# 54rt1n/shardmerge

Hardware: AMD Instinct MI355X
Metric: merged-weight GB/s per GPU + % HBM roofline, Llama-3-70B 3-way FFT merge (higher is better)
Workload: dtype f32; 1 GPU; Llama-3-70B block tensors, this rank's 1/8 slice (9 per block x 10 blocks), K=3 finetunes, bf16 in/out, resident in HBM; workload_id=llama3-70b-slice, k=3, parallelism=tensor-partition x1 (no data-path collective), streams_per_gpu=8

## Files before the change

shardmerge_amd/csrc/sm_capi.inc:

```

struct smhip_ctx {
    smhip::Pipeline<SM_BACKEND> pipe;
    explicit smhip_ctx(int device) : pipe(device) {}
};

#define SM_GUARD(ctx)                      \
    if (!(ctx)) return SMHIP_ERR_ARG;      \
    (ctx)->pipe.err.clear();
#define SM_FINISH(ctx, rc)                                                        \
    do {                                                                          \
        int rc__ = (rc);                                                          \
        if (rc__ == SMHIP_OK && !(ctx)->pipe.be.ok()) {                           \
            (ctx)->pipe.err = (ctx)->pipe.be.error();                             \
            rc__ = SMHIP_ERR_HIP;                                                 \
        }                                                                         \
        return rc__;                                                              \
    } while (0)

extern "C" {

const char* smhip_version(void) { return SM_VERSION_STRING; }

int smhip_create(int device, smhip_ctx** out) {
    if (!out) return SMHIP_ERR_ARG;
    *out = nullptr;
    smhip_ctx* c = new smhip_ctx(device);
    if (!c->pipe.be.ok()) {
        fprintf(stderr, "smhip_create: %s\n", c->pipe.be.error().c_str());
        delete c;
        return SMHIP_ERR_HIP;
    }
    *out = c;
    return SMHIP_OK;
}

void smhip_destroy(smhip_ctx* ctx) { delete ctx; }

const char* smhip_last_error(smhip_ctx* ctx) { return ctx ? ctx->pipe.err.c_str() : "null context"; }

int smhip_reserve(smhip_ctx* ctx, int rows, int cols) {
    SM_GUARD(ctx);
    if (rows < 1 || cols < 1) return ctx->pipe.fail(SMHIP_ERR_ARG, "bad shape");
    SM_FINISH(ctx, ctx->pipe.reserve(rows, cols));
}

size_t smhip_workspace_bytes(smhip_ctx* ctx) { return ctx ? ctx->pipe.workspace_bytes() : 0; }

int smhip_length_supported(int n) {
    int T;
    std::vector<int> rad;
    return smhip::plan_shape(n, T, rad) ? SMHIP_OK : SMHIP_ERR_SHAPE;
}

int smhip_shape_supported(int rows, int cols) {
    return smhip::shape_support(rows, cols) ? SMHIP_OK : SMHIP_ERR_SHAPE;
}

int smhip_fft_transform(smhip_ctx* ctx, const float* x, int rows, int cols, float* spectrum, void* stream) {
    SM_GUARD(ctx);
    if (!x || !spectrum || rows < 1 || cols < 1) return ctx->pipe.fail(SMHIP_ERR_ARG, "bad argument");
    ctx->pipe.stream = stream;
    SM_FINISH(ctx, ctx->pipe.fft_transform(x, rows, cols, spectrum));
}

int smhip_ifft_transform(smhip_ctx* ctx, const float* spectrum, int rows, int cols, float* real_out, void* stream) {
    SM_GUARD(ctx);
    if (!real_out || !spectrum || rows < 1 || cols < 1) return ctx->pipe.fail(SMHIP_ERR_ARG, "bad argument");
    ctx->pipe.stream = stream;
    SM_FINISH(ctx, ctx->pipe.ifft_transform(spectrum, rows, cols, real_out));
}

int smhip_interpolate_fft_components(smhip_ctx* ctx, const float* f0, const float* f1, int rows, int cols, double t,
                                     double t_sum, double cutoff_pct, double cull_pct, int interp_imag,
                                     float* out_spectrum, smhip_blend_info* info, void* stream) {
    SM_GUARD(ctx);
    if (!f0 || !f1 || !out_spectrum || rows < 1 || cols < 1) return ctx->pipe.fail(SMHIP_ERR_ARG, "bad argument");
    ctx->pipe.stream = stream;
    SM_FINISH(ctx, ctx->pipe.blend_full(f0, f1, rows, cols, smhip::BLEND_SLERP, t, t_sum, cutoff_pct, cull_pct, 1,
                                        interp_imag, out_spectrum, info));
}

int smhip_arithmetic_fft_components(smhip_ctx* ctx, const float* f0, const float* f1, int rows, int cols, double t,
                                    int agreement, int do_imag, float* out_spectrum, void* stream) {
    SM_GUARD(ctx);
    if (!f0 || !f1 || !out_spectrum || rows < 1 || cols < 1) return ctx->pipe.fail(SMHIP_ERR_ARG, "bad argument");
    ctx->pipe.stream = stream;
    SM_FINISH(ctx, ctx->pipe.blend_full(f0, f1, rows, cols, smhip::BLEND_ARITH, t, 1.0, 0, 0, agreement, do_imag,
                                        out_spectrum, nullptr));
}

int smhip_merge_tensors_fft2_slerp(smhip_ctx* ctx, const float* v0, const float* v1, int rows, int cols, double t,
                                   double b, double t_sum, double cutoff_pct, double cull_pct, float* out,
                                   double* norm0, double* norm1, int* branch, smhip_blend_info* info, void* stream) {
    SM_GUARD(ctx);
    if (!v0 || !v1 || !out || rows < 1 || cols < 1) return ctx->pipe.fail(SMHIP_ERR_ARG, "bad argument");
    ctx->pipe.stream = stream;
    SM_FINISH(ctx, ctx->pipe.merge_pair_slerp(v0, v1, rows, cols, t, b, t_sum, cutoff_pct, cull_pct, out, norm0, norm1,
                                              branch, info));
}

int smhip_task_arithmetic_fft2(smhip_ctx* ctx, const float* v0, const float* v1, int rows, int cols, double t,
                               int agreement, float* out, void* stream) {
    SM_GUARD(ctx);
    if (!v0 || !v1 || !out || rows < 1 || cols < 1) return ctx->pipe.fail(SMHIP_ERR_ARG, "bad argument");
    ctx->pipe.stream = stream;
    smhip::SigDesc a{v0, nullptr, smhip::DT_F32, 1.f}, bb{v1, nullptr, smhip::DT_F32, 1.f};
    smhip::PairOut po;
    po.out = out; po.out_mode = smhip::OUT_F32; po.post = 1.f;
    const int rc0 = ctx->pipe.reserve(rows, cols);
    if (rc0) SM_FINISH(ctx, rc0);
    ctx->pipe.clear_flags();
    po.ifft_policy = 0;
    SM_FINISH(ctx, ctx->pipe.pair_arith(a, bb, rows, cols, 1.f, 1.f, t, agreement, po, -1, -1));
}

int smhip_merge_layer(smhip_ctx* ctx, const smhip_layer_desc* desc, void* out_bf16, float* delta_out,
                      smhip_layer_report* report, void* stream) {
    SM_GUARD(ctx);
    if (!desc || !out_bf16) return ctx->pipe.fail(SMHIP_ERR_ARG, "bad argument");
    for (int i = 0; i < desc->k && i < SMHIP_MAX_MODELS; ++i)
        if (!desc->finetune[i] || !desc->base[i]) return ctx->pipe.fail(SMHIP_ERR_ARG, "null model tensor");
    if (!desc->base_out) return ctx->pipe.fail(SMHIP_ERR_ARG, "null base_out");
    ctx->pipe.stream = stream;
    SM_FINISH(ctx, ctx->pipe.merge_layer(*desc, out_bf16, delta_out, report));
}

int smhip_addition_merge(smhip_ctx* ctx, int k, const void* const* finetunes, const void* base, int dtype, size_t n,
                         int sign_agreement, void* out, void* stream) {
    SM_GUARD(ctx);
    if (!finetunes || !base || !out || n < 1) return ctx->pipe.fail(SMHIP_ERR_ARG, "bad argument");
    if (dtype < SMHIP_BF16 || dtype > SMHIP_F32) return ctx->pipe.fail(SMHIP_ERR_ARG, "bad dtype");
    for (int i = 0; i < k && i < SMHIP_MAX_MODELS; ++i)
        if (!finetunes[i]) return ctx->pipe.fail(SMHIP_ERR_ARG, "null model tensor");
    ctx->pipe.stream = stream;
    SM_FINISH(ctx, ctx->pipe.addition_merge(k, finetunes, base, dtype, n, sign_agreement ? 1 : 0, out));
}

int smhip_slerp(smhip_ctx* ctx, const float* v0, const float* v1, size_t rows, size_t cols, float t, float* out, void* stream) {
    SM_GUARD(ctx);
    if (rows * cols > 0 && (!v0 || !v1 || !out)) return ctx->pipe.fail(SMHIP_ERR_ARG, "bad argument");
    ctx->pipe.stream = stream;
    SM_FINISH(ctx, ctx->pipe.fn_slerp(v0, v1, rows, cols, t, out));
}

int smhip_div_scalar(smhip_ctx* ctx, const void* x, int dtype, size_t n, float s, void* out, void* stream) {
    SM_GUARD(ctx);
    if (n > 0 && (!x || !out)) return ctx->pipe.fail(SMHIP_ERR_ARG, "bad argument");
    if (dtype < SMHIP_BF16 || dtype > SMHIP_F32) return ctx->pipe.fail(SMHIP_ERR_ARG, "bad dtype");
    ctx->pipe.stream = stream;
    SM_FINISH(ctx, ctx->pipe.fn_div_scalar(x, dtype, n, s, out));
}

int smhip_lora_apply(smhip_ctx* ctx, const void* base, int dtype, int rows, int cols, const void* lora_a,
                     const void* lora_b, int factor_dtype, int rank, float scale, void* out, void* stream) {
    SM_GUARD(ctx);
    if (!base || !lora_a || !lora_b || !out || rows < 1 || cols < 1) return ctx->pipe.fail(SMHIP_ERR_ARG, "bad argument");
    if (dtype < SMHIP_BF16 || dtype > SMHIP_F32 || factor_dtype < SMHIP_BF16 || factor_dtype > SMHIP_F32)
        return ctx->pipe.fail(SMHIP_ERR_ARG, "bad dtype");
    if (rank < 1 || rank > smhip::LORA_MAX_RANK) return ctx->pipe.fail(SMHIP_ERR_ARG, "rank out of range (1..512)");
    const size_t bes = dtype == SMHIP_F32 ? 4 : 2, fes = factor_dtype == SMHIP_F32 ? 4 : 2;
    const uintptr_t o0 = (uintptr_t)out, o1 = o0 + (size_t)rows * cols * bes;
    auto overlaps = [&](const void* p, size_t bytes) { return (uintptr_t)p < o1 && o0 < (uintptr_t)p + bytes; };
    if (overlaps(base, (size_t)rows * cols * bes) || overlaps(lora_a, (size_t)rank * cols * fes) ||
        overlaps(lora_b, (size_t)rows * rank * fes))
        return ctx->pipe.fail(SMHIP_ERR_ARG, "lora_apply: out overlaps an input");
    ctx->pipe.stream = stream;
    SM_FINISH(ctx, ctx->pipe.lora_apply(base, dtype, rows, cols, lora_a, lora_b, factor_dtype, rank, scale, out));
}

int smhip_adapter_apply(smhip_ctx* ctx, const smhip_adapter_desc* d, void* stream) {
    SM_GUARD(ctx);
    if (!d || !d->base || !d->lora_a || !d->lora_b || !d->out || d->rows < 1 || d->cols < 1)
        return ctx->pipe.fail(SMHIP_ERR_ARG, "bad argument");
    if (d->dtype < SMHIP_BF16 || d->dtype > SMHIP_F32 || d->factor_dtype < SMHIP_BF16 || d->factor_dtype > SMHIP_F32 ||
        (d->magnitude && (d->magnitude_dtype < SMHIP_BF16 || d->magnitude_dtype > SMHIP_F32)))
        return ctx->pipe.fail(SMHIP_ERR_ARG, "bad dtype");
    if (d->layout != SMHIP_ADAPTER_LINEAR && d->layout != SMHIP_ADAPTER_EMBEDDING)
        return ctx->pipe.fail(SMHIP_ERR_ARG, "adapter_apply: bad layout");
    if (d->magnitude && d->layout != SMHIP_ADAPTER_LINEAR)
        return ctx->pipe.fail(SMHIP_ERR_ARG, "adapter_apply: DoRA (a magnitude) needs the LINEAR layout");
    if (d->rank < 1 || d->rank > smhip::LORA_MAX_RANK) return ctx->pipe.fail(SMHIP_ERR_ARG, "rank out of range (1..512)");
    const size_t bes = d->dtype == SMHIP_F32 ? 4 : 2, fes = d->factor_dtype == SMHIP_F32 ? 4 : 2;
    const size_t mes = d->magnitude_dtype == SMHIP_F32 ? 4 : 2;
    const bool emb = d->layout == SMHIP_ADAPTER_EMBEDDING;
    const uintptr_t o0 = (uintptr_t)d->out, o1 = o0 + (size_t)d->rows * d->cols * bes;
    auto overlaps = [&](const void* p, size_t bytes) { return (uintptr_t)p < o1 && o0 < (uintptr_t)p + bytes; };
    if (overlaps(d->base, (size_t)d->rows * d->cols * bes) ||
        overlaps(d->lora_a, (size_t)d->rank * (emb ? d->rows : d->cols) * fes) ||
        overlaps(d->lora_b, (size_t)(emb ? d->cols : d->rows) * d->rank * fes) ||
        (d->magnitude && overlaps(d->magnitude, (size_t)d->rows * mes)))
        return ctx->pipe.fail(SMHIP_ERR_ARG, "adapter_apply: out overlaps an input");
    ctx->pipe.stream = stream;
    SM_FINISH(ctx, ctx->pipe.adapter_apply(d->base, d->dtype, d->rows, d->cols, d->lora_a, d->lora_b, d->factor_dtype,
                                           d->rank, d->scale, emb ? 1 : 0, d->magnitude, d->magnitude_dtype, d->out));
}

int smhip_exact_norm(smhip_ctx* ctx, const void* x, int dtype, size_t n, double* norm_out, void* stream) {
    SM_GUARD(ctx);
    if (!norm_out || (n > 0 && !x)) return ctx->pipe.fail(SMHIP_ERR_ARG, "bad argument");
    if (dtype < SMHIP_BF16 || dtype > SMHIP_F32) return ctx->pipe.fail(SMHIP_ERR_ARG, "bad dtype");
    ctx->pipe.stream = stream;
    SM_FINISH(ctx, ctx->pipe.fn_exact_norm(x, dtype, n, norm_out));
}

int smhip_correlate_pairs(smhip_ctx* ctx, int k, const void* const* tensors, int dtype, size_t rows, size_t cols,
                          float* matrix_out, void* stream) {
    SM_GUARD(ctx);
    if (!tensors || !matrix_out || rows < 1 || cols < 1) return ctx->pipe.fail(SMHIP_ERR_ARG, "bad argument");
    if (dtype < SMHIP_BF16 || dtype > SMHIP_F32) return ctx->pipe.fail(SMHIP_ERR_ARG, "bad dtype");
    for (int i = 0; i < k && i < 8; ++i)
        if (!tensors[i]) return ctx->pipe.fail(SMHIP_ERR_ARG, "null tensor");
    ctx->pipe.stream = stream;
    SM_FINISH(ctx, ctx->pipe.correlate_pairs(k, tensors, dtype, rows, cols, matrix_out));
}

int smhip_reference_cpu_norm(smhip_ctx* ctx, const void* x, const void* base, int dtype, size_t n, float* norm_out,
                             void* stream) {
    SM_GUARD(ctx);
    if (!x || !norm_out) return ctx->pipe.fail(SMHIP_ERR_ARG, "bad argument");
    if (dtype < SMHIP_BF16 || dtype > SMHIP_F32) return ctx->pipe.fail(SMHIP_ERR_ARG, "bad dtype");
    ctx->pipe.stream = stream;
    const int rc0 = ctx->pipe.reserve(1, 1);
    if (rc0) SM_FINISH(ctx, rc0);
    smhip::SigDesc sg{x, base, dtype, 1.f};
    double out = 0;
    if (!ctx->pipe.run_serial_norms(&sg, 1, n, &out))
        return ctx->pipe.fail(SMHIP_ERR_ARG, "reference_cpu norm: inputs must be 16-byte aligned");
    *norm_out = (float)out;
    SM_FINISH(ctx, SMHIP_OK);
}

int smhip_debug_option(smhip_ctx* ctx, const char* key, long value) {
    SM_GUARD(ctx);
    if (key && std::string(key) == "aten_overlap") { ctx->pipe.aten_overlap = value != 0; return SMHIP_OK; }
    if (key && std::string(key) == "emf_max_sample") { ctx->pipe.emf_max_sample = value >= 1 && value <= 4096 ? (int)value : smhip::EMF_MAX_SAMPLE; return SMHIP_OK; }
    if (key && std::string(key) == "aten_serial") { ctx->pipe.aten_serial = value != 0; return SMHIP_OK; }
    if (key && std::string(key) == "class_norms") { ctx->pipe.class_norms_mode = value >= 0 && value <= 2 ? (int)value : 1; return SMHIP_OK; }
    if (key && std::string(key) == "cand_cap") { ctx->pipe.debug_cand_cap = value > 0 ? (uint32_t)value : 0u; return SMHIP_OK; }
    if (key && std::string(key) == "sel_chunks") { ctx->pipe.debug_sel_chunks = value > 0 ? (uint32_t)value : 0u; return SMHIP_OK; }
    if (key && std::string(key) == "sel_flush_always") { ctx->pipe.debug_flush_always = value != 0; return SMHIP_OK; }
    if (key && std::string(key) == "fuse_norms") { ctx->pipe.fuse_norms = value != 0; return SMHIP_OK; }
    if (key && std::string(key) == "noise_seed") { ctx->pipe.noise_seed_base = (uint32_t)value; return SMHIP_OK; }
    if (key && std::string(key) == "spectral_intermediates") { ctx->pipe.spectral_inter = value != 0; return SMHIP_OK; }
    if (key && std::string(key) == "fuse_spec_norm") { ctx->pipe.fuse_spec_norm = value != 0; return SMHIP_OK; }
    if (key && std::string(key) == "sel_wgs_per_cu") { ctx->pipe.sel_wgs_per_cu = value > 0 ? (int)value : 5; return SMHIP_OK; }
    if (key && std::string(key) == "pair1d") { ctx->pipe.pair1d_enabled = value != 0; return SMHIP_OK; }
    if (key && std::string(key) == "spec_cull") { ctx->pipe.spec_cull = value != 0; return SMHIP_OK; }
    if (key && std::string(key) == "spec_min_bins") { ctx->pipe.spec_min_bins = value >= 0 ? (size_t)value : (size_t)1 << 20; return SMHIP_OK; }
    if (key && std::string(key) == "dftp_pairs") { ctx->pipe.dftp_pairs_enabled = value != 0; return SMHIP_OK; }
    if (key && std::string(key) == "f2s_pair") { ctx->pipe.f2s_pair = value != 0; return SMHIP_OK; }
    if (key && std::string(key) == "f1_multi") { ctx->pipe.f1_multi = value != 0; return SMHIP_OK; }
    if (key && std::string(key) == "force_bluestein") { ctx->pipe.debug_force_bluestein = value != 0; return SMHIP_OK; }
    if (key && std::string(key) == "force_split") { ctx->pipe.debug_force_split = value > 1 && value <= smhip::DFTP_MAX_P ? (int)value : 0; return SMHIP_OK; }
    if (key && std::string(key) == "fold_columns") { ctx->pipe.fold_enabled = value != 0; return SMHIP_OK; }
    if (key && std::string(key) == "fold_min_rows") { ctx->pipe.fold_min_rows = value > 0 ? (int)value : SM_FOLD_MIN_ROWS; return SMHIP_OK; }
    return ctx->pipe.fail(SMHIP_ERR_ARG, "unknown debug option");
}

int smhip_debug_query(smhip_ctx* ctx, const char* key, long* value) {
    SM_GUARD(ctx);
    if (!key || !value) return SMHIP_ERR_ARG;
    if (std::string(key) == "spec_hit") { *value = ctx->pipe.last_spec_verdict(); SM_FINISH(ctx, SMHIP_OK); }
    if (std::string(key) == "spec_checked" || std::string(key) == "spec_hits") {
        unsigned long long c = 0, h = 0;
        ctx->pipe.spec_totals(&c, &h);
        *value = (long)(std::string(key) == "spec_hits" ? h : c);
        SM_FINISH(ctx, SMHIP_OK);
    }
    if (std::string(key) == "aten_fast" || std::string(key) == "aten_group" || std::string(key) == "aten_slow") {
        unsigned long long v3[3];
        ctx->pipe.aten_stats(1, v3);
        *value = (long)v3[std::string(key) == "aten_fast" ? 0 : std::string(key) == "aten_group" ? 1 : 2];
        SM_FINISH(ctx, SMHIP_OK);
    }
    return ctx->pipe.fail(SMHIP_ERR_ARG, "unknown debug query");
}

int smhip_profile_enable(smhip_ctx* ctx, int on) { SM_GUARD(ctx); ctx->pipe.be.profile_enable(on != 0); return SMHIP_OK; }
int smhip_profile_reset(smhip_ctx* ctx) { SM_GUARD(ctx); ctx->pipe.be.profile_reset(); return SMHIP_OK; }
int smhip_profile_count(smhip_ctx* ctx) { return ctx ? ctx->pipe.be.profile_count() : 0; }
int smhip_profile_get(smhip_ctx* ctx, int i, const char** name, uint64_t* launches, double* total_ms) {
    SM_GUARD(ctx);
    return ctx->pipe.be.profile_get(i, name, launches, total_ms) ? SMHIP_OK : SMHIP_ERR_ARG;
}

}
```

shardmerge_amd/csrc/sm_kernels.hpp:

```cpp
#pragma once
#include <cmath>
#include <cstring>

#include "fft_engine.hpp"
#include "sm_aten_core.hpp"

namespace smhip {

struct cf4 { float x, y, z, w; };
struct u32x4 { uint32_t x, y, z, w; };

enum { DT_BF16 = 0, DT_F16 = 1, DT_F32 = 2 };

struct SigDesc {
    const void* x;
    const void* base;
    int dtype;
    float prescale;
};

SM_HD uint32_t umax(uint32_t a, uint32_t b) { return a > b ? a : b; }
SM_HD float u2f(uint32_t u) { float f; memcpy(&f, &u, 4); return f; }
SM_HD uint32_t f2u(float f) { uint32_t u; memcpy(&u, &f, 4); return u; }
SM_HD float bf16_to_f(uint32_t h) { return u2f(h << 16); }
// ... 173 lines not shown

struct F1Params {
    FftPlanDev plan;
    SigDesc a, b;
    int R, C, Cb;
    int pitch4;
    int ilv;
    int nb;
    size_t row_stride;
    int vec;
    cf4* t1;
    double* partials;
    int R2;
    int rowpair;
    int Rcol;
    size_t slab_elems;
    const cf2* twR;
    F1Sigs sigs;
    AtenFuse fuse;
    int fuse_rowpair;
};

template <class P> constexpr bool f1_full_batch() {
    if constexpr (P::is_static) return P::T <= 256; else return false;
}
#ifndef SM_ROW_PACK_MAX_T
#define SM_ROW_PACK_MAX_T 256
#endif
template <class P> constexpr bool f1_opaque() {
    if constexpr (P::is_static) return P::T >= 512; else return false;
}
#ifndef SM_ROW_PACK_BIG
#define SM_ROW_PACK_BIG 0
#endif
template <class P> constexpr int f1_pack() {
    if constexpr (P::is_static) return P::T <= SM_ROW_PACK_MAX_T ? 1 : SM_ROW_PACK_BIG; else return 1;
}

template <class P, class Ex>
SM_HD void k_f1(Ex& ex, const F1Params& p) {
    typename Ex::template State<FftState> st;
    ex.init(st);
    float* lds = ex.lds() + LDS_SCRATCH_FLOATS;
    const FftPlanDev& pl = p.plan;
    const int T = plan_T<P>(pl), C = plan_N<P>(pl);
    const int LF = plan_lds<P>(pl);
    int sig_;
    const int bid = f1_pick_signal(p.sigs, ex.bid(), (p.ilv > p.nb) ? p.ilv / p.nb : 1, sig_);
    const int pbid = p.sigs.n > 1 ? bid : ex.bid();
    SigDesc sgA = p.a, sgB = p.b;
    cf4* t1_ = p.t1;
    double* partials_ = p.partials;
    if (p.sigs.n > 1) {
        sgA.x = p.sigs.x[sig_]; sgA.base = p.sigs.base[sig_];
        sgB.x = (const char*)sgA.x + p.sigs.b_off; sgB.base = sgA.base ? (const char*)sgA.base + p.sigs.b_off : nullptr;
        t1_ = p.sigs.t1[sig_]; partials_ = p.sigs.partials[sig_];
    }
    const bool vec = P::is_static ? true : (p.vec != 0);
    auto fuse_where = [&](int comp) {
        return [&, comp](int g, int& sig, long long& mrow) {
            const int row = bid * p.nb + g;
            if (row >= p.R) return false;
            if (p.fuse_rowpair) { sig = sig_; mrow = 2LL * row + comp; }
            else { sig = comp; mrow = row; if (comp == 1 && !sgB.x) return false; }
            return true;
        };
    };
    if constexpr (P::is_static) {
        if constexpr (aten_fusable(P::N, P::T)) {
            if (p.fuse.prefix) ex.each(st, [&](int tid, FftState& s) {
                s.fep[0] = aten_fused_ep<P::N, P::T>(p.fuse, tid, fuse_where(0));
                s.fep[1] = aten_fused_ep<P::N, P::T>(p.fuse, tid, fuse_where(1));
            });
        }
    }

    ex.each(st, [&](int tid, FftState& s) {
        const int g = tid / T, t = tid % T;
        const int row = bid * p.nb + g;
        const bool valid = row < p.R;
        double sa = 0.0, sb = 0.0;
        if (vec && sgA.dtype != DT_F32 && sgB.dtype != DT_F32) {
            constexpr int NQ = EMAX / 8;
            u32x4 ra[NQ], rab[NQ], rb[NQ], rbb[NQ];
            bool ok[NQ];
            size_t off[NQ];
#pragma unroll
            for (int q = 0; q < NQ; ++q) {
                const int n0 = 8 * (t + q * T);
                ok[q] = valid && n0 < C;
                off[q] = ok[q] ? ((size_t)row * p.row_stride + n0) / 8 : 0;
            }
            const bool has_ab = sgA.base != nullptr, has_b = sgB.x != nullptr, has_bb = has_b && sgB.base != nullptr;
            const u32x4* pa = (const u32x4*)sgA.x;
            const u32x4* pab = has_ab ? (const u32x4*)sgA.base : pa;
            const u32x4* pb = has_b ? (const u32x4*)sgB.x : pa;
            const u32x4* pbb = has_bb ? (const u32x4*)sgB.base : pa;
            constexpr int QB = f1_full_batch<P>() ? NQ : NQ / 2;
            bool all_ok = true;
#pragma unroll
            for (int q = 0; q < NQ; ++q) all_ok = all_ok && ok[q];
            static_for<0, NQ / QB>([&](auto h_c) {
            constexpr int Q0 = decltype(h_c)::value * QB, Q1 = Q0 + QB;
#pragma unroll
            for (int q = Q0; q < Q1; ++q) ra[q] = pa[off[q]];
#pragma unroll
            for (int q = Q0; q < Q1; ++q) rab[q] = pab[off[q]];
#pragma unroll
            for (int q = Q0; q < Q1; ++q) rb[q] = pb[off[q]];
#pragma unroll
            for (int q = Q0; q < Q1; ++q) rbb[q] = pbb[off[q]];
            auto decode = [&](auto masked_c) {
                constexpr bool MASKED = decltype(masked_c)::value;
#pragma unroll
                for (int q = Q0; q < Q1; ++q) {
                    float va[8], vb[8], ba[8], bb[8];
                    decode16x8(ra[q], sgA.dtype, va);
                    decode16x8(rab[q], sgA.dtype, ba);
                    decode16x8(rb[q], sgB.dtype, vb);
                    decode16x8(rbb[q], sgB.dtype, bb);
#pragma unroll
                    for (int c = 0; c < 8; ++c) {
                        if (!has_ab) ba[c] = 0.f;
                        if (!has_b) vb[c] = 0.f;
                        if (!has_bb) bb[c] = 0.f;
                    }
                    float pa = 0.f, pb = 0.f;
#pragma unroll
                    for (int c = 0; c < 8; ++c) {
                        float xa = (va[c] - ba[c]) * sgA.prescale;
                        float xb = (vb[c] - bb[c]) * sgB.prescale;
                        if (MASKED && !ok[q]) { xa = 0.f; xb = 0.f; }
                        s.xr[q * 8 + c] = xa; s.xi[q * 8 + c] = xb;
                        pa += xa * xa; pb += xb * xb;
                    }
                    sa += pa; sb += pb;
                }
            };
            if (all_ok) decode(std::false_type{});
            else decode(std::true_type{});
            });

        } else if (vec) {
            constexpr int NQ = EMAX / 8;
            bool ok[NQ];
            size_t off[NQ];
#pragma unroll
            for (int q = 0; q < NQ; ++q) {
                const int n0 = 8 * (t + q * T);
                ok[q] = valid && n0 < C;
                off[q] = ok[q] ? (size_t)row * p.row_stride + n0 : 0;
            }
            auto load_signal = [&](const SigDesc& sg, float* dst, double& ss) {
                if (!sg.x) {
#pragma unroll
                    for (int i = 0; i < 8 * NQ; ++i) dst[i] = 0.f;
                    return;
                }
                const bool has_base = sg.base != nullptr;
                float v[NQ][8], bv[NQ][8];
                if (sg.dtype == DT_F32) {
                    const cf4* px = (const cf4*)sg.x;
                    const cf4* pb = has_base ? (const cf4*)sg.base : px;
                    cf4 r[NQ][2], rb[NQ][2];
#pragma unroll
                    for (int q = 0; q < NQ; ++q) { r[q][0] = px[off[q] / 4]; r[q][1] = px[off[q] / 4 + 1]; }
#pragma unroll
                    for (int q = 0; q < NQ; ++q) { rb[q][0] = pb[off[q] / 4]; rb[q][1] = pb[off[q] / 4 + 1]; }
#pragma unroll
                    for (int q = 0; q < NQ; ++q) {
                        const cf4 x0 = r[q][0], x1 = r[q][1], b0 = rb[q][0], b1 = rb[q][1];
                        const float xs[8] = {x0.x, x0.y, x0.z, x0.w, x1.x, x1.y, x1.z, x1.w};
                        const float bs[8] = {b0.x, b0.y, b0.z, b0.w, b1.x, b1.y, b1.z, b1.w};
#pragma unroll
                        for (int c = 0; c < 8; ++c) { v[q][c] = xs[c]; bv[q][c] = bs[c]; }
                    }
                } else {
                    const u32x4* px = (const u32x4*)sg.x;
                    const u32x4* pb = has_base ? (const u32x4*)sg.base : px;
                    u32x4 r[NQ], rb[NQ];
#pragma unroll
                    for (int q = 0; q < NQ; ++q) r[q] = px[off[q] / 8];
#pragma unroll
                    for (int q = 0; q < NQ; ++q) rb[q] = pb[off[q] / 8];
#pragma unroll
                    for (int q = 0; q < NQ; ++q) { decode16x8(r[q], sg.dtype, v[q]); decode16x8(rb[q], sg.dtype, bv[q]); }
                }
#pragma unroll
                for (int q = 0; q < NQ; ++q) {
                    float ps = 0.f;
#pragma unroll
                    for (int c = 0; c < 8; ++c) {
                        float x = (v[q][c] - (has_base ? bv[q][c] : 0.f)) * sg.prescale;
                        if (!ok[q]) x = 0.f;
                        dst[q * 8 + c] = x;
                        ps += x * x;
                    }
                    ss += ps;
                }
            };
            load_signal(sgA, s.xr, sa);
            load_signal(sgB, s.xi, sb);
        } else {
#pragma unroll
            for (int q = 0; q < EMAX; ++q) {
                const int n = t + q * T;
                float va = 0.f, vb = 0.f;
                if (valid && n < C) {
                    const size_t off = (size_t)row * p.row_stride + n;
                    va = load_sig1(sgA, off);
                    vb = load_sig1(sgB, off);
                }
                s.xr[q] = va; s.xi[q] = vb;
                sa += (double)va * va; sb += (double)vb * vb;
            }
        }
        s.red[0] = sa; s.red[1] = sb;
    });
    ex.template block_sum<2>(st, [&](const double* tot) {
        partials_[2 * (size_t)pbid] = tot[0];
        partials_[2 * (size_t)pbid + 1] = tot[1];
    });

    wg_fft<P, f1_pack<P>(), 1>(ex, st, pl, lds,
        [&](int tid, FftState& s, auto comp_c) {
            constexpr int comp = decltype(comp_c)::value;
            const int g = tid / T, t = tid % T;
            float* l = lds + g * LF;
            const float* x = comp_of<comp>(s);
            if (vec) {
#pragma unroll
                for (int q = 0; q < EMAX / 8; ++q) {
                    const int n0 = 8 * (t + q * T);
                    if (n0 < C) {
#pragma unroll
                        for (int c = 0; c < 8; ++c) l[lpad(n0 + c)] = x[q * 8 + c];
                    }
                }
            } else {
#pragma unroll
                for (int q = 0; q < EMAX; ++q) {
                    const int n = t + q * T;
                    if (n < C) l[lpad(n)] = x[q];
                }
            }
        },
        [&](int tid, FftState& s, auto comp_c) {
            constexpr int comp = decltype(comp_c)::value;
            int tid_ = tid;
            if constexpr (f1_opaque<P>()) SM_OPAQUE(tid_);
            const int g = tid_ / T, t = tid_ % T;
            const float* l = lds + g * LF;
            float* o = comp_of<comp>(s);
#pragma unroll
            for (int u = 0; u < EMAX / 2 + 1; ++u) {
                const int k = t + u * T;
                if (k < p.Cb) {
                    const int k2 = (k == 0) ? 0 : C - k;
                    const float v1 = l[lpad(k)], v2 = l[lpad(k2)];
                    if (comp == 0) { o[2 * u] = 0.5f * (v1 + v2); o[2 * u + 1] = 0.5f * (v2 - v1); }
                    else           { o[2 * u] = 0.5f * (v1 - v2); o[2 * u + 1] = 0.5f * (v1 + v2); }
                    if (!sgB.x) o[2 * u + 1] = 0.f;
                }
            }
        },
        [&](auto comp_c) {
            constexpr int comp = decltype(comp_c)::value;
            if constexpr (P::is_static) {
                if constexpr (aten_fusable(P::N, P::T)) {
                    if (p.fuse.prefix)
                        aten_fused_rows<P::N, P::T>(ex, st, p.fuse, lds, LF, fuse_where(comp), [](FftState& s) { return s.fep[comp]; });
                }
            }
        });

    ex.each(st, [&](int tid, FftState& s) {
        int tid_ = tid;
        if constexpr (f1_opaque<P>()) SM_OPAQUE(tid_);
        const int g = tid_ / T, t = tid_ % T;
        const int row = bid * p.nb + g;
        if (row >= p.R) return;
        cf4* dst = t1_ + (size_t)(row / p.ilv) * p.pitch4 * p.ilv + (row % p.ilv);
#pragma unroll
        for (int u = 0; u < EMAX / 2 + 1; ++u) {
            const int k = t + u * T;
            if (k < p.Cb) {
                cf4 v;
                v.x = s.xr[2 * u]; v.y = s.xi[2 * u]; v.z = s.xi[2 * u + 1]; v.w = s.xr[2 * u + 1];
                dst[(size_t)k * p.ilv] = v;
            }
        }
    });
}

#ifndef SM_F1Q_QB
#define SM_F1Q_QB 1
#endif
#ifndef SM_F1Q_PREFETCH_B
#define SM_F1Q_PREFETCH_B 1
#endif
#ifndef SM_F1Q_PACK
#define SM_F1Q_PACK 1
#endif
template <class P> constexpr bool f1q_eligible() {
    if constexpr (P::is_static) return 4 * P::T <= 1024 && (P::N / P::T) % 2 == 0 && P::N % 8 == 0; else return false;
}

struct F1QState {
    float xr[EREG];
    float xi[EREG];
    double red[4];
    u32x4 rb[EMAX / 8], rbb[EMAX / 8];
};

template <class P, class Ex>
SM_HD void k_f1q(Ex& ex, const F1Params& p) {
    if constexpr (!f1q_eligible<P>()) { return; } else {
    typename Ex::template State<F1QState> st;
    ex.init(st);
    float* lds = ex.lds() + LDS_SCRATCH_FLOATS;
    const FftPlanDev& pl = p.plan;
    constexpr int T = P::T, C = P::N, LF = P::lds_floats;
    constexpr int E2 = C / T / 2;
    constexpr int NJ = (E2 + 3) / 4;
    constexpr int NQ = EMAX / 8;
    static_assert(NJ * 8 + 4 <= EREG, "register slots");
    int sig_;
    const int bid = f1_pick_signal(p.sigs, ex.bid(), p.ilv > 1 ? p.ilv : 1, sig_);
    const int pbid = p.sigs.n > 1 ? bid : ex.bid();
    SigDesc sa = p.a, sb = p.b;
    cf4* t1_ = p.t1;
    double* partials_ = p.partials;
    if (p.sigs.n > 1) {
        sa.x = p.sigs.x[sig_]; sa.base = p.sigs.base[sig_];
        sb.x = (const char*)sa.x + p.sigs.b_off; sb.base = sa.base ? (const char*)sa.base + p.sigs.b_off : nullptr;
        t1_ = p.sigs.t1[sig_]; partials_ = p.sigs.partials[sig_];
    }
    const int unit = bid;
    const bool live = unit < p.R2;
    const bool bits16 = sa.dtype != DT_F32 && sb.dtype != DT_F32;
    const bool has_ab = sa.base != nullptr, has_b = sb.x != nullptr, has_bb = has_b && sb.base != nullptr;
    const int n2A = p.rowpair ? 2 * unit : unit, n2B = p.rowpair ? 2 * unit + 1 : unit;
    cf4* const rowp = t1_ + (size_t)(unit / p.ilv) * p.pitch4 * p.ilv + (unit % p.ilv);
    const size_t slabstride = p.slab_elems;

    ex.each(st, [&](int, F1QState& s) { s.red[0] = 0.0; s.red[1] = 0.0; });

    wg_fft<P, SM_F1Q_PACK, 1>(ex, st, pl, lds,
        [&](int tid, F1QState& s, auto comp_c) {
            constexpr int comp = decltype(comp_c)::value;
            int tid_ = tid;
            SM_OPAQUE(tid_);
            const int g = tid_ / T, t = tid_ % T;
            float* l = lds + g * LF;
            const size_t rowoff = (size_t)(unit + g * p.R2) * p.row_stride;
            auto okq = [&](int q) { return live && 8 * (t + q * T) < C; };
            auto offq = [&](int q) { return okq(q) ? rowoff + 8 * (t + q * T) : (size_t)0; };
            double ss = 0.0;
            if (bits16) {
                const u32x4* pa = (const u32x4*)sa.x;
                if (comp == 0) {
                    const u32x4* pab = has_ab ? (const u32x4*)sa.base : pa;
                    u32x4 ra[NQ], rab[NQ];
#pragma unroll
                    for (int q = 0; q < NQ; ++q) ra[q] = pa[offq(q) / 8];
#pragma unroll
                    for (int q = 0; q < NQ; ++q) rab[q] = pab[offq(q) / 8];
#if SM_F1Q_PREFETCH_B
                    const u32x4* pb = has_b ? (const u32x4*)sb.x : pa;
                    const u32x4* pbb = has_bb ? (const u32x4*)sb.base : pa;
#pragma unroll
                    for (int q = 0; q < NQ; ++q) s.rb[q] = pb[offq(q) / 8];
#pragma unroll
                    for (int q = 0; q < NQ; ++q) s.rbb[q] = pbb[offq(q) / 8];
#endif
#pragma unroll
                    for (int q = 0; q < NQ; ++q) {
                        float va[8], ba[8];
                        decode16x8(ra[q], sa.dtype, va);
                        decode16x8(rab[q], sa.dtype, ba);
                        const int n0 = 8 * (t + q * T);
                        float qa = 0.f;
#pragma unroll
                        for (int c = 0; c < 8; ++c) {
                            float xa = (va[c] - (has_ab ? ba[c] : 0.f)) * sa.prescale;
                            if (!okq(q)) xa = 0.f;
                            if (n0 < C) l[lpad(n0 + c)] = xa;
                            qa += xa * xa;
                        }
                        ss += qa;
                    }
                } else {
#if !SM_F1Q_PREFETCH_B
                    const u32x4* pb = has_b ? (const u32x4*)sb.x : pa;
                    const u32x4* pbb = has_bb ? (const u32x4*)sb.base : pa;
#pragma unroll
                    for (int q = 0; q < NQ; ++q) s.rb[q] = pb[offq(q) / 8];
#pragma unroll
                    for (int q = 0; q < NQ; ++q) s.rbb[q] = pbb[offq(q) / 8];
#endif
#pragma unroll
                    for (int q = 0; q < NQ; ++q) {
                        float vb[8], bb[8];
                        decode16x8(s.rb[q], sb.dtype, vb);
                        decode16x8(s.rbb[q], sb.dtype, bb);
                        const int n0 = 8 * (t + q * T);
                        float qb = 0.f;
#pragma unroll
                        for (int c = 0; c < 8; ++c) {
                            float xb = has_b ? (vb[c] - (has_bb ? bb[c] : 0.f)) * sb.prescale : 0.f;
                            if (!okq(q)) xb = 0.f;
                            if (n0 < C) l[lpad(n0 + c)] = xb;
                            qb += xb * xb;
                        }
                        ss += qb;
                    }
                }
            } else {
                const SigDesc& sg = comp == 0 ? sa : sb;
#pragma unroll
                for (int q = 0; q < NQ; ++q) {
                    float v[8];
                    if (sg.x) load_sig8(sg, offq(q), v);
                    else { for (int c = 0; c < 8; ++c) v[c] = 0.f; }
                    const int n0 = 8 * (t + q * T);
                    float ps = 0.f;
#pragma unroll
                    for (int c = 0; c < 8; ++c) {
                        const float x = okq(q) ? v[c] : 0.f;
                        if (n0 < C) l[lpad(n0 + c)] = x;
                        ps += x * x;
                    }
                    ss += ps;
                }
            }
            s.red[comp] += ss;
        },
        [&](int tid, F1QState& s, auto comp_c) {
            constexpr int comp = decltype(comp_c)::value;
            int tid_ = tid;
            SM_OPAQUE(tid_);
            const int g = tid_ / T, t = tid_ % T;
            auto emit = [&](int k, const float* are, const float* aim, const float* bre, const float* bim) {
                SM_SCHED_FENCE();
                float ar[4], ai[4], br[4], bi[4];
#pragma unroll
                for (int q = 0; q < 4; ++q) { ar[q] = are[q]; ai[q] = aim[q]; br[q] = has_b ? bre[q] : 0.f; bi[q] = has_b ? bim[q] : 0.f; }
                Dft<4>::run(ar, ai);
                Dft<4>::run(br, bi);
#pragma unroll
                for (int k1 = 0; k1 < 4; ++k1) {
                    if (k1) {
                        const cf2 wa = p.twR[(size_t)n2A * k1], wb = p.twR[(size_t)n2B * k1];
                        cmul(ar[k1], ai[k1], wa.x, wa.y); cmul(br[k1], bi[k1], wb.x, wb.y);
                    }
                    cf4 v = {ar[k1], ai[k1], br[k1], bi[k1]};
                    if (live) rowp[(size_t)k * p.ilv + k1 * slabstride] = v;
                }
                SM_SCHED_FENCE();
            };
#pragma unroll
            for (int jj = 0; jj < NJ; ++jj) {
                const int u = 4 * jj + g;
                if (u < E2) {
                    const int k = t + u * T;
                    const int k2 = (k == 0) ? 0 : C - k;
                    float aim[4], bre[4];
#pragma unroll
                    for (int gp = 0; gp < 4; ++gp) {
                        const float* l = lds + gp * LF;
                        const float v1 = l[lpad(k)], v2 = l[lpad(k2)];
                        const int sl = (jj * 4 + gp) * 2;
                        if (comp == 0) { s.xr[sl] = 0.5f * (v1 + v2); s.xr[sl + 1] = 0.5f * (v2 - v1); }
                        else           { aim[gp] = 0.5f * (v1 - v2); bre[gp] = 0.5f * (v1 + v2); }
                    }
                    if (comp == 1) {
                        float are[4], bim[4];
#pragma unroll
                        for (int gp = 0; gp < 4; ++gp) { are[gp] = s.xr[(jj * 4 + gp) * 2]; bim[gp] = s.xr[(jj * 4 + gp) * 2 + 1]; }
                        emit(k, are, aim, bre, bim);
                    }
                }
            }
            if (tid == 0) {
                if (comp == 0) {
#pragma unroll
                    for (int gp = 0; gp < 4; ++gp) s.xr[NJ * 8 + gp] = lds[gp * LF + lpad(C / 2)];
                } else {
                    float are[4], aim[4] = {0.f, 0.f, 0.f, 0.f}, bre[4], bim[4] = {0.f, 0.f, 0.f, 0.f};
#pragma unroll
                    for (int gp = 0; gp < 4; ++gp) { are[gp] = s.xr[NJ * 8 + gp]; bre[gp] = lds[gp * LF + lpad(C / 2)]; }
                    emit(C / 2, are, aim, bre, bim);
                }
            }
        });

    ex.template block_sum<2>(st, [&](const double* tot) {
        partials_[2 * (size_t)pbid] = tot[0];
        partials_[2 * (size_t)pbid + 1] = tot[1];
    });
    }
}

struct SliceGrid { int wgs = 0; size_t t1_stride = 0, plane_stride = 0; };
template <class Ex> SM_HD int slice_of(Ex& ex, const SliceGrid& sl, int& bid) {
    bid = ex.bid();
    if (sl.wgs <= 0) return 0;
    const int s = bid / sl.wgs;
    bid -= s * sl.wgs;
    return s;
}

struct F2Params {
    FftPlanDev plan;
    const cf4* t1;
    int pitch4;
    int ilv;
    int R, C, Cb;
    int nsig;
    int swap;
    float scale[2];
    float* reA; float* imA; float* reB;
    unsigned long long* hist;
    int slab;
    int Cb_real;
    int Rfull;
    size_t slab_elems;
    SliceGrid sl;
};
SM_HD int fold_bin(int v, int slab, int Cb_real, int R2, int Rfull, size_t& off) {
    const int k1 = v / slab, k = v % slab;
    off = (size_t)k * Rfull + (size_t)k1 * R2;
    return k < Cb_real ? k : -1;
}

#ifndef SM_T1_ILV
#define SM_T1_ILV 2
#endif
#ifndef SM_T1_ILV_MIN_ROWS
#define SM_T1_ILV_MIN_ROWS 8192
#endif
#ifndef SM_F2_MAX_THREADS
#define SM_F2_MAX_THREADS 512
#endif
SM_HD constexpr int t1_interleave_rows(int R) { return R >= SM_T1_ILV_MIN_ROWS ? SM_T1_ILV : 1; }
SM_HD constexpr int f2_nsig_for(int T) { return (2 * T <= SM_F2_MAX_THREADS) ? 2 : 1; }

constexpr int FOLD_ILV = 2;
template <class P> constexpr bool fold_col_plan() {
    if constexpr (P::is_static) return f2_nsig_for(P::T) == 2 && (P::N == 2048 || P::N == 3584 || P::N == 4096 || P::N == 7168);
    else return false;
}
template <class P, int BINS, bool FOLD = false, class Ex>
SM_HD void k_f2(Ex& ex, const F2Params& p) {
    if constexpr (FOLD && !fold_col_plan<P>()) { return; } else {
    typename Ex::template State<FftState> st;
    ex.init(st);
    float* lds = ex.lds() + LDS_SCRATCH_FLOATS;
    const FftPlanDev& pl = p.plan;
    const int T = plan_T<P>(pl), R = plan_N<P>(pl);
    const int LF = plan_lds<P>(pl);
    const int ng = P::is_static ? f2_nsig_for(T) : p.nsig;
    const int ilv = FOLD ? FOLD_ILV : (P::is_static ? t1_interleave_rows(R) : p.ilv);
    int bid;
    const int slice = slice_of(ex, p.sl, bid);
    const cf4* const t1 = p.t1 + slice * p.sl.t1_stride;
    const size_t pl_off = slice * p.sl.plane_stride;
    const int lbid = (ng == 2) ? xcd_remap(bid, 8 / BINS) : xcd_remap(bid, 16);
    const int kbase = (ng == 2) ? lbid * BINS : lbid / 2;
    const int slot0 = (ng == 2) ? 0 : lbid % 2;
    if (kbase >= p.Cb) return;
    const int ngroups = (ng == 2) ? 2 * BINS : 1;
    const int nthreads = ngroups * T;
    uint32_t* lhist = (uint32_t*)(lds + ngroups * LF);

    ex.each(st, [&](int tid, FftState& s) {
        if (ng == 2) {
            const int b = tid % BINS, lane = tid / BINS;
            const int k2 = kbase + b;
            auto load_rows = [&](auto ilv_c) {
                constexpr int ILV = decltype(ilv_c)::value;
#pragma unroll
                for (int q = 0; q < EMAX / 2; ++q) {
                    const int m = lane + (q / ILV) * 2 * T;
                    const int n = m * ILV + q % ILV;
                    const bool live = n < R && k2 < p.Cb;
                    const int kc = k2 < p.Cb ? k2 : p.Cb - 1;
                    const int mcl = n < R ? m : (R - 1 - q % ILV) / ILV;
                    cf4 v;
                    if constexpr (FOLD) {
                        v = t1[(size_t)(kc / p.slab) * p.slab_elems + ((size_t)mcl * p.slab + (kc % p.slab)) * ILV + q % ILV];
                    } else {
                        v = t1[((size_t)mcl * p.pitch4 + kc) * ILV + q % ILV];
                    }
                    s.xr[2 * q] = live ? v.x : 0.f; s.xi[2 * q] = live ? v.y : 0.f; s.xr[2 * q + 1] = live ? v.z : 0.f; s.xi[2 * q + 1] = live ? v.w : 0.f;
                }
            };
            if (ilv == 2) load_rows(std::integral_constant<int, 2>{});
            else load_rows(std::integral_constant<int, 1>{});
        } else {
#pragma unroll
            for (int q = 0; q < EMAX; ++q) {
                const int n = tid + q * T;
                float re = 0.f, im = 0.f;
                if (n < R) {
                    const cf2* src = (const cf2*)(t1 + ((size_t)(n / ilv) * p.pitch4 + kbase) * ilv + n % ilv) + slot0;
                    re = src->x; im = src->y;
                }
                s.xr[q] = re; s.xi[q] = im;
            }
        }
        if (p.hist) for (int h = tid; h < HIST1_BINS; h += nthreads) lhist[h] = 0;
    });

#ifndef SM_F2_PACK
#define SM_F2_PACK 1
#endif
    wg_fft<P, SM_F2_PACK, 2>(ex, st, pl, lds,
        [&](int tid, FftState& s, auto comp_c) {
            constexpr int comp = decltype(comp_c)::value;
            const float* x = comp_of<comp>(s);
            if (ng == 2) {
                const int b = tid % BINS, lane = tid / BINS;
                float* la = lds + (2 * b) * LF;
                auto scatter_rows = [&](auto ilv_c) {
                    constexpr int ILV = decltype(ilv_c)::value;
#pragma unroll
                    for (int q = 0; q < EMAX / 2; ++q) {
                        const int n = (lane + (q / ILV) * 2 * T) * ILV + q % ILV;
                        if (n < R) { la[lpad(n)] = x[2 * q]; la[LF + lpad(n)] = x[2 * q + 1]; }
                    }
                };
                if (ilv == 2) scatter_rows(std::integral_constant<int, 2>{});
                else scatter_rows(std::integral_constant<int, 1>{});
            } else {
#pragma unroll
                for (int q = 0; q < EMAX; ++q) {
                    const int n = tid + q * T;
                    if (n < R) lds[lpad(n)] = x[q];
                }
            }
        },
        [&](int tid, FftState& s, auto comp_c) {
            constexpr int comp = decltype(comp_c)::value;
            const int g = tid / T, t = tid % T;
            const float* l = lds + g * LF;
            float* o = comp_of<comp>(s);
#pragma unroll
            for (int u = 0; u < EMAX / 4; ++u) {
#pragma unroll
                for (int c = 0; c < 4; ++c) {
                    const int k1 = 4 * (t + u * T) + c;
                    if (k1 < R) o[4 * u + c] = l[lpad(k1)];
                }
            }
        });

    ex.each(st, [&](int tid, FftState& s) {
        const int g = tid / T, t = tid % T;
        const int slot = (ng == 2) ? (g & 1) : slot0;
        const int k2 = kbase + ((ng == 2) ? (g >> 1) : 0);
        if (k2 >= p.Cb) return;
        const bool role_a = (slot ^ p.swap) == 0;
        const float sc = p.scale[slot];
        size_t poff = (size_t)k2 * R;
        int kreal = k2;
        if constexpr (FOLD) { kreal = fold_bin(k2, p.slab, p.Cb_real, R, p.Rfull, poff); if (kreal < 0) return; }
        const uint32_t w = (uint32_t)bin_weight(kreal, p.C);
        float* dre = (role_a ? p.reA : p.reB) + pl_off + poff;
        float* dim = p.imA + pl_off + poff;
#pragma unroll
        for (int u = 0; u < EMAX / 4; ++u) {
            const int k0 = 4 * (t + u * T);
            if (k0 + 3 < R && (R & 3) == 0) {
                cf4 vr = {s.xr[4 * u] * sc, s.xr[4 * u + 1] * sc, s.xr[4 * u + 2] * sc, s.xr[4 * u + 3] * sc};
                *(cf4*)(dre + k0) = vr;
                if (role_a) {
                    cf4 vi = {s.xi[4 * u] * sc, s.xi[4 * u + 1] * sc, s.xi[4 * u + 2] * sc, s.xi[4 * u + 3] * sc};
                    *(cf4*)(dim + k0) = vi;
                }
            } else {
#pragma unroll
                for (int c = 0; c < 4; ++c) {
                    if (k0 + c < R) {
                        dre[k0 + c] = s.xr[4 * u + c] * sc;
                        if (role_a) dim[k0 + c] = s.xi[4 * u + c] * sc;
                    }
                }
            }
            if (p.hist) {
#pragma unroll
                for (int c = 0; c < 4; ++c) {
                    if (k0 + c < R) {
                        const uint32_t key = f2u(s.xr[4 * u + c] * sc) & 0x7fffffffu;
                        ex.lds_atomic_add(&lhist[key >> 20], w);
                    }
                }
            }
        }
    });
    if (p.hist) {
        ex.sync();
        ex.each(st, [&](int tid, FftState&) {
            for (int h = tid; h < HIST1_BINS; h += nthreads) {
                const uint32_t v = lhist[h];
                if (v) ex.global_atomic_add(&p.hist[h], (unsigned long long)v);
            }
        });
    }
    }
}

#ifndef SM_COL_THREADS
#define SM_COL_THREADS 512
#endif
constexpr int f2_bins_for(int T, int N = 1 << 30) {
    if (T == 64 && N <= 256) return 8;
    return (SM_COL_THREADS / (2 * T)) > 1 ? (SM_COL_THREADS / (2 * T) > 8 ? 8 : SM_COL_THREADS / (2 * T)) : 1;
}
#ifndef SM_I1_THREADS
constexpr int i1_bins_for(int T) { return 2; }
#else
constexpr int i1_bins_for(int T) { return (SM_I1_THREADS / T) > 2 ? ((SM_I1_THREADS / T) > 16 ? 16 : (SM_I1_THREADS / T)) : 2; }
#endif
template <class P> constexpr int f2_bins() { if constexpr (P::is_static) return f2_bins_for(P::T, P::N); else return 1; }
template <class P> constexpr int i1_bins() { if constexpr (P::is_static) return i1_bins_for(P::T); else return 2; }

struct F2SParams {
    FftPlanDev plan;
    const cf4* t1;
    int pitch4;
    int R, C, Cb;
    int role_a;
    float scale;
    float* re; float* im;
    unsigned long long* hist;
    int slab, Cb_real, Rfull;
    size_t slab_elems;
    double* im_partials;
    SliceGrid sl;
    int two;
    const cf4* t1_2; int role_a_2; float scale_2; float* re_2;
};
template <class P> constexpr int f2s_groups() {
    if constexpr (P::is_static) return f2_nsig_for(P::T) == 2 ? 2 * f2_bins_for(P::T, P::N) : 1; else return 1;
}

#ifndef SM_F2S_ILV
#define SM_F2S_ILV 1
#endif
constexpr int F2S_ILV = SM_F2S_ILV;
#ifndef SM_F2S_DIRECT
#define SM_F2S_DIRECT 0
#endif
template <class P, int G> constexpr int f2s_direct() {
    if constexpr (!P::is_static) return 0;
    else {
        constexpr int R0 = P::radix(0);
        constexpr bool ok = F2S_ILV == 1 && (G == 1 || G == 2) && P::npass >= 2 && P::T % 2 == 0 && R0 % 2 == 0 &&
                            (P::N / R0) % 2 == 0 && (EMAX / R0) * R0 * P::T >= P::N;
        return ok ? (SM_F2S_DIRECT & 3) : 0;
    }
}
template <class P, int G, bool FOLD = false, class Ex>
SM_HD void k_f2s(Ex& ex, const F2SParams& p) {
    if constexpr (FOLD && !fold_col_plan<P>()) { return; } else {
    typename Ex::template State<FftState> st;
    ex.init(st);
    float* lds = ex.lds() + LDS_SCRATCH_FLOATS;
    const FftPlanDev& pl = p.plan;
    const int T = plan_T<P>(pl), R = plan_N<P>(pl);
    const int LF = plan_lds<P>(pl);
    constexpr int XG = G >= 8 ? 1 : 8 / G;
    int bid_in_slice;
    const int slice = slice_of(ex, p.sl, bid_in_slice);
    int sig2 = 0;
    const int lbid = p.two ? pick_signal(2, bid_in_slice, XG, sig2) : xcd_remap(bid_in_slice, XG);
    const cf4* const t1 = (sig2 ? p.t1_2 : p.t1) + slice * p.sl.t1_stride;
    const size_t pl_off = slice * p.sl.plane_stride;
    const int role_a_ = sig2 ? p.role_a_2 : p.role_a;
    const float scale_ = sig2 ? p.scale_2 : p.scale;
    float* const re_ = sig2 ? p.re_2 : p.re;
    const int kbase = lbid * G;
    if (kbase >= p.Cb) {
        if (p.im_partials) ex.each(st, [&](int tid, FftState&) { if (tid == 0) p.im_partials[ex.bid()] = 0.0; });
        return;
    }
    const int nthreads = G * T;
    const int half = R / 2;
    uint32_t* lhist = (uint32_t*)(lds + G * LF);

    constexpr int DIRECT = f2s_direct<P, G>();
    if constexpr ((DIRECT & 1) != 0) {
        constexpr int R0 = P::radix(0), MB0 = EMAX / R0, nb0 = P::N / R0;
        ex.each(st, [&](int tid, FftState& s) {
            const int g = tid / T, t = tid % T;
            const int k2 = kbase + g;
            const int kc = k2 < p.Cb ? k2 : p.Cb - 1;
            const int par = t & 1;
            static_for<0, MB0>([&](auto m_c) {
                constexpr int m = decltype(m_c)::value;
                const bool live = (t + m * T) < nb0 && k2 < p.Cb;
                static_for<0, R0 / 2>([&](auto q_c) {
                    constexpr int q = decltype(q_c)::value;
                    const int pm = live ? (t >> 1) + m * (T / 2) + q * nb0 + par * (nb0 / 2) : 0;
                    cf4 v;
#if defined(SM_DIAG_NOMEM)
                    v = cf4{(float)q, (float)t, 1.f, (float)kc};
#else
                    if constexpr (FOLD) v = t1[(size_t)(kc / p.slab) * p.slab_elems + (size_t)pm * p.slab + (kc % p.slab)];
                    else v = t1[(size_t)pm * p.pitch4 + kc];
#endif
                    s.xr[m * R0 + 2 * q] = live ? v.x : 0.f; s.xi[m * R0 + 2 * q] = live ? v.y : 0.f;
                    s.xr[m * R0 + 2 * q + 1] = live ? v.z : 0.f; s.xi[m * R0 + 2 * q + 1] = live ? v.w : 0.f;
                });
            });
            if (p.hist) for (int h = tid; h < HIST1_BINS; h += nthreads) lhist[h] = 0;
        });
        ex.template lane_pair_trade<MB0 * (R0 / 2) * 2>(st, [](FftState& s, auto k_c) {
            constexpr int k = decltype(k_c)::value;
            constexpr int idx = k / 2, m = idx / (R0 / 2), q = idx % (R0 / 2);
            float* arr = (k % 2) ? s.xi : s.xr;
            return FloatPairRef{arr[m * R0 + 2 * q], arr[m * R0 + 2 * q + 1]};
        });
    } else
    ex.each(st, [&](int tid, FftState& s) {
        const int b = tid % G, lane = tid / G;
        const int k2 = kbase + b;
#pragma unroll
        for (int q = 0; q < EMAX / 2; ++q) {
            const int m = F2S_ILV * (lane + (q / F2S_ILV) * T) + q % F2S_ILV;
            const bool live = m < half && k2 < p.Cb;
            const int mc = m < half ? m : half - 1, kc = k2 < p.Cb ? k2 : p.Cb - 1;
            cf4 v;
#if defined(SM_DIAG_NOMEM)
            v = cf4{(float)q, (float)lane, 1.f, (float)kc};
#else
            if constexpr (FOLD) {
                v = t1[(size_t)(kc / p.slab) * p.slab_elems + ((size_t)(mc / F2S_ILV) * p.slab + (kc % p.slab)) * F2S_ILV + mc % F2S_ILV];
            } else {
                v = t1[((size_t)(mc / F2S_ILV) * p.pitch4 + kc) * F2S_ILV + mc % F2S_ILV];
            }
#endif
            s.xr[2 * q] = live ? v.x : 0.f; s.xi[2 * q] = live ? v.y : 0.f; s.xr[2 * q + 1] = live ? v.z : 0.f; s.xi[2 * q + 1] = live ? v.w : 0.f;
        }
        if (p.hist) for (int h = tid; h < HIST1_BINS; h += nthreads) lhist[h] = 0;
    });

#ifndef SM_F2S_PACK
#define SM_F2S_PACK 1
#endif
    wg_fft<P, SM_F2S_PACK, 4, DIRECT>(ex, st, pl, lds,
        [&](int tid, FftState& s, auto comp_c) {
            constexpr int comp = decltype(comp_c)::value;
            const float* x = comp_of<comp>(s);
            const int b = tid % G, lane = tid / G;
            float* la = lds + b * LF;
#pragma unroll
            for (int q = 0; q < EMAX / 2; ++q) {
                const int m = F2S_ILV * (lane + (q / F2S_ILV) * T) + q % F2S_ILV;
                if (m < half) { la[lpad(2 * m)] = x[2 * q]; la[lpad(2 * m + 1)] = x[2 * q + 1]; }
            }
        },
        [&](int tid, FftState& s, auto comp_c) {
            constexpr int comp = decltype(comp_c)::value;
            const int g = tid / T, t = tid % T;
            const float* l = lds + g * LF;
            float* o = comp_of<comp>(s);
#pragma unroll
            for (int u = 0; u < EMAX / 4; ++u) {
#pragma unroll
                for (int c = 0; c < 4; ++c) {
                    const int k1 = 4 * (t + u * T) + c;
                    if (k1 < R) o[4 * u + c] = l[lpad(k1)];
                }
            }
        });

    ex.each(st, [&](int tid, FftState& s) {
        const int g = tid / T, t = tid % T;
        const int k2 = kbase + g;
        s.red[0] = 0.0;
        if (k2 >= p.Cb) return;
        const float sc = scale_;
        size_t poff = (size_t)k2 * R;
        int kreal = k2;
        if constexpr (FOLD) { kreal = fold_bin(k2, p.slab, p.Cb_real, R, p.Rfull, poff); if (kreal < 0) return; }
        const uint32_t w = (uint32_t)bin_weight(kreal, p.C);
        float* dre = re_ + pl_off + poff;
        float* dim = p.im + pl_off + poff;
        float imsq = 0.f;
        if constexpr ((DIRECT & 2) != 0) {
            constexpr int RL = P::radix(P::npass - 1), MBL = EMAX / RL, NsL = P::N / RL;
            static_for<0, MBL>([&](auto m_c) {
                constexpr int m = decltype(m_c)::value;
                const int j = t + m * T;
                if (j < NsL) {
                    static_for<0, RL>([&](auto i_c) {
                        constexpr int i = decltype(i_c)::value, e = m * RL + i;
                        const float vr = s.xr[e] * sc;
#if defined(SM_DIAG_NOMEM)
                        if (vr == 12345.678f)
#endif
                        dre[j + i * NsL] = vr;
                        if (role_a_) {
                            const float vi = s.xi[e] * sc;
#if defined(SM_DIAG_NOMEM)
                            if (vi == 12345.678f)
#endif
                            dim[j + i * NsL] = vi;
                            imsq += vi * vi;
                        }
                        if (p.hist) ex.lds_atomic_add(&lhist[(f2u(vr) & 0x7fffffffu) >> 20], w);
                    });
                }
            });
        } else
#pragma unroll
        for (int u = 0; u < EMAX / 4; ++u) {
            const int k0 = 4 * (t + u * T);
            if (k0 + 3 < R && (R & 3) == 0) {
                cf4 vr = {s.xr[4 * u] * sc, s.xr[4 * u + 1] * sc, s.xr[4 * u + 2] * sc, s.xr[4 * u + 3] * sc};
#if defined(SM_DIAG_NOMEM)
                if (vr.x == 12345.678f)
#endif
                *(cf4*)(dre + k0) = vr;
                if (role_a_) {
                    cf4 vi = {s.xi[4 * u] * sc, s.xi[4 * u + 1] * sc, s.xi[4 * u + 2] * sc, s.xi[4 * u + 3] * sc};
#if defined(SM_DIAG_NOMEM)
                    if (vi.x == 12345.678f)
#endif
                    *(cf4*)(dim + k0) = vi;
                    imsq += vi.x * vi.x + vi.y * vi.y + vi.z * vi.z + vi.w * vi.w;
                }
            } else {
#pragma unroll
                for (int c = 0; c < 4; ++c) {
                    if (k0 + c < R) {
                        dre[k0 + c] = s.xr[4 * u + c] * sc;
                        if (role_a_) { const float vi = s.xi[4 * u + c] * sc; dim[k0 + c] = vi; imsq += vi * vi; }
                    }
                }
            }
            if (p.hist) {
#pragma unroll
                for (int c = 0; c < 4; ++c) {
                    if (k0 + c < R) {
                        const uint32_t key = f2u(s.xr[4 * u + c] * sc) & 0x7fffffffu;
                        ex.lds_atomic_add(&lhist[key >> 20], w);
                    }
                }
            }
        }
        s.red[0] = (double)imsq * (double)w;
    });
    if (p.hist) {
        ex.sync();
        ex.each(st, [&](int tid, FftState&) {
            for (int h = tid; h < HIST1_BINS; h += nthreads) {
                const uint32_t v = lhist[h];
                if (v) ex.global_atomic_add(&p.hist[h], (unsigned long long)v);
            }
        });
    }
    if (p.im_partials) {
        ex.sync();
        ex.template block_sum<1>(st, [&](const double* tot) { p.im_partials[ex.bid()] = tot[0]; });
    }
    }
}

template <class Ex>
SM_HD void k_f2_r1(Ex& ex, const F2Params& p) {
    typename Ex::template State<EmptyStateF> st;
    ex.init(st);
    uint32_t* lhist = (uint32_t*)(ex.lds() + LDS_SCRATCH_FLOATS);
    const int nt = ex.nthreads();
    if (p.hist) {
        ex.each(st, [&](int tid, EmptyStateF&) { for (int h = tid; h < HIST1_BINS; h += nt) lhist[h] = 0; });
        ex.sync();
    }
    ex.each(st, [&](int tid, EmptyStateF&) {
        for (int k2 = ex.bid() * nt + tid; k2 < p.Cb; k2 += ex.nblocks() * nt) {
            const cf4 v = p.t1[k2];
            const float in[2][2] = {{v.x, v.y}, {v.z, v.w}};
            const uint32_t w = (uint32_t)bin_weight(k2, p.C);
#pragma unroll
            for (int slot = 0; slot < 2; ++slot) {
                const bool role_a = (slot ^ p.swap) == 0;
                const float re = in[slot][0] * p.scale[slot], im = in[slot][1] * p.scale[slot];
                if (role_a) { p.reA[k2] = re; p.imA[k2] = im; } else { p.reB[k2] = re; }
                if (p.hist) ex.lds_atomic_add(&lhist[(f2u(re) & 0x7fffffffu) >> 20], w);
            }
        }
    });
    if (p.hist) {
        ex.sync();
        ex.each(st, [&](int tid, EmptyStateF&) {
            for (int h = tid; h < HIST1_BINS; h += nt) {
                const uint32_t v = lhist[h];
                if (v) ex.global_atomic_add(&p.hist[h], (unsigned long long)v);
            }
        });
    }
}

struct I1Params {
    FftPlanDev plan;
    const float* reR;
    const float* imA;
    const float* cull_thr;
    float cull_val;
    int R, Cb;
    int s;
    cf2* G;
    int pitchG;
    SliceGrid sl;
};

template <class P> constexpr bool fold_full_plan() {
    if constexpr (P::is_static) return P::N == 8192 || P::N == 14336 || P::N == 16384 || P::N == 28672; else return false;
}
template <class P, int S, bool FOLD = false, class Ex>
SM_HD void k_i1(Ex& ex, const I1Params& p) {
    if constexpr (FOLD && !fold_full_plan<P>()) { return; } else {
    typename Ex::template State<FftState> st;
    ex.init(st);
    float* lds = ex.lds() + LDS_SCRATCH_FLOATS;
    const FftPlanDev& pl = p.plan;
    const int T = plan_T<P>(pl), R = plan_N<P>(pl);
    const int LF = plan_lds<P>(pl);
    int bid_in_slice;
    const int slice = slice_of(ex, p.sl, bid_in_slice);
    const size_t pl_off = slice * p.sl.plane_stride;
    cf2* const Gs = p.G + slice * p.sl.t1_stride;
    const int bid = xcd_remap(bid_in_slice, 16 / S);
    if (bid * S >= p.Cb) return;
    const float thr = p.cull_thr ? *p.cull_thr : p.cull_val;

    ex.each(st, [&](int tid, FftState& s) {
        const int g = tid / T, t = tid % T;
        const int k2 = bid * S + g;
        const bool valid = k2 < p.Cb;
        const float* sre = p.reR + pl_off + (size_t)k2 * R;
        const float* sim = p.imA + pl_off + (size_t)k2 * R;
#pragma unroll
        for (int u = 0; u < EMAX / 4; ++u) {
            const int k0 = 4 * (t + u * T);
            float re[4] = {0.f, 0.f, 0.f, 0.f}, im[4] = {0.f, 0.f, 0.f, 0.f};
            if (valid) {
                if (k0 + 3 < R && (R & 3) == 0) {
                    const cf4 a = *(const cf4*)(sre + k0), b = *(const cf4*)(sim + k0);
                    re[0] = a.x; re[1] = a.y; re[2] = a.z; re[3] = a.w;
                    im[0] = b.x; im[1] = b.y; im[2] = b.z; im[3] = b.w;
                } else {
#pragma unroll
                    for (int c = 0; c < 4; ++c)
                        if (k0 + c < R) { re[c] = sre[k0 + c]; im[c] = sim[k0 + c]; }
                }
            }
#pragma unroll
            for (int c = 0; c < 4; ++c) {
                if (fabsf(re[c]) < thr) re[c] = 0.f;
                s.xr[4 * u + c] = im[c];
                s.xi[4 * u + c] = re[c];
            }
        }
    });

#ifndef SM_I1_PACK
#define SM_I1_PACK 0
#endif
    wg_fft<P, SM_I1_PACK, 8>(ex, st, pl, lds,
        [&](int tid, FftState& s, auto comp_c) {
            constexpr int comp = decltype(comp_c)::value;
            const int g = tid / T, t = tid % T;
            float* l = lds + g * LF;
            const float* x = comp_of<comp>(s);
#pragma unroll
            for (int u = 0; u < EMAX / 4; ++u) {
#pragma unroll
                for (int c = 0; c < 4; ++c) {
                    const int k1 = 4 * (t + u * T) + c;
                    if (k1 < R) {
                        if constexpr (FOLD) {
                            const int R2 = R / 4;
                            l[lpad((k1 / R2) + 4 * (k1 % R2))] = x[4 * u + c];
                        } else {
                            l[lpad(k1)] = x[4 * u + c];
                        }
                    }
                }
            }
        },
        [&](int tid, FftState& s, auto comp_c) {
            constexpr int comp = decltype(comp_c)::value;
            float* o = comp_of<comp>(s);
#pragma unroll
            for (int j = 0; j < EMAX / (2 * S); ++j) {
                const int m = tid + j * S * T;
#pragma unroll
                for (int par = 0; par < 2; ++par) {
                    const int r = 2 * m + par;
                    if (r < R) {
#pragma unroll
                        for (int g = 0; g < S; ++g) o[(2 * j + par) * S + g] = lds[g * LF + lpad(r)];
                    }
                }
            }
        });

    ex.each(st, [&](int tid, FftState& s) {
#pragma unroll
        for (int j = 0; j < EMAX / (2 * S); ++j) {
            const int m = tid + j * S * T;
            if (2 * m < R) {
                cf4* dst = (cf4*)Gs + (size_t)m * p.pitchG + (size_t)bid * S;
                const bool odd = 2 * m + 1 < R;
#pragma unroll
                for (int g = 0; g < S; ++g) {
                    if (bid * S + g < p.pitchG) {
                        const int e0 = (2 * j) * S + g, e1 = (2 * j + 1) * S + g;
                        cf4 v = {s.xi[e0], s.xr[e0], odd ? s.xi[e1] : 0.f, odd ? s.xr[e1] : 0.f};
                        dst[g] = v;
                    }
                }
            }
        }
    });
    }
}

template <class Ex>
SM_HD void k_i1_r1(Ex& ex, const I1Params& p) {
    typename Ex::template State<EmptyStateF> st;
    ex.init(st);
    const int nt = ex.nthreads();
    const float thr = p.cull_thr ? *p.cull_thr : p.cull_val;
    ex.each(st, [&](int tid, EmptyStateF&) {
        for (int k2 = ex.bid() * nt + tid; k2 < p.Cb; k2 += ex.nblocks() * nt) {
            float re = p.reR[k2];
            if (fabsf(re) < thr) re = 0.f;
            cf4 v = {re, p.imA[k2], 0.f, 0.f};
            ((cf4*)p.G)[k2] = v;
        }
    });
}

enum { OUT_BF16 = 0, OUT_F32 = 1 };
struct I2Params {
    FftPlanDev plan;
    const cf2* G;
    int pitchG;
    int R, C, Cb;
    int nb;
    int vec;
    float inv_n;
    float post;
    int ifft_policy;
    const void* base; int base_dtype;
    void* out; int out_mode;
    uint32_t* flags;
    double* norm_partials;
};

SM_HD void i2_finish(const I2Params& p, float v, size_t off, uint32_t& nan1, uint32_t& inf1, uint32_t& nan2, uint32_t& inf2, float& outv) {
    v *= p.inv_n;
    if (p.ifft_policy) {
        if (is_nan(v)) { v = 0.f; nan1++; }
        if (is_inf(v)) inf1 = 1;
    }
    v *= p.post;
    if (p.base) {
        v += load_elem(p.base, p.base_dtype, off);
        if (is_nan(v)) { v = 0.f; nan2++; }
        if (is_inf(v)) inf2 = 1;
    }
    outv = v;
}

template <class P, class Ex>
SM_HD void k_i2(Ex& ex, const I2Params& p) {
    typename Ex::template State<FftState> st;
    ex.init(st);
    float* lds = ex.lds() + LDS_SCRATCH_FLOATS;
    const FftPlanDev& pl = p.plan;
    const int T = plan_T<P>(pl), C = plan_N<P>(pl);
    const int LF = plan_lds<P>(pl);
    const int bid = ex.bid();
    const bool vec = P::is_static ? true : (p.vec != 0);

    ex.each(st, [&](int tid, FftState& s) {
        const int g = tid / T, t = tid % T;
        const int r0 = 2 * (bid * p.nb + g), r1 = r0 + 1;
        const bool v0 = r0 < p.R, v1 = r1 < p.R;
        const cf4* GP = (const cf4*)p.G + (size_t)(v0 ? r0 / 2 : 0) * p.pitchG;
        constexpr int NU = EMAX / 2 + 1, HU = (NU + 1) / 2;
        static_for<0, 2>([&](auto half_c) {
            constexpr int u0 = decltype(half_c)::value * HU;
            constexpr int u1 = (u0 + HU < NU) ? u0 + HU : NU;
            cf4 ap[HU];
#pragma unroll
            for (int u = u0; u < u1; ++u) {
                const int k = t + u * T;
                ap[u - u0] = GP[k < p.Cb ? k : 0];
            }
#pragma unroll
            for (int u = u0; u < u1; ++u) {
                const int k = t + u * T;
                if (k < p.Cb) {
                    cf2 g0 = {ap[u - u0].x, ap[u - u0].y}, g1 = {ap[u - u0].z, ap[u - u0].w};
                    if (!v0) { g0.x = 0.f; g0.y = 0.f; }
                    if (!v1) { g1.x = 0.f; g1.y = 0.f; }
                    if (k == 0 || 2 * k == C) { g0.y = 0.f; g1.y = 0.f; }
                    const float ykr = g0.x - g1.y, yki = g0.y + g1.x;
                    const float ymr = g0.x + g1.y, ymi = g1.x - g0.y;
                    s.xr[2 * u] = yki; s.xi[2 * u] = ykr;
                    s.xr[2 * u + 1] = ymi; s.xi[2 * u + 1] = ymr;
                }
            }
        });
    });

    wg_fft<P, f1_pack<P>(), 16>(ex, st, pl, lds,
        [&](int tid, FftState& s, auto comp_c) {
            constexpr int comp = decltype(comp_c)::value;
            const int g = tid / T, t = tid % T;
            float* l = lds + g * LF;
            const float* x = comp_of<comp>(s);
#pragma unroll
            for (int u = 0; u < EMAX / 2 + 1; ++u) {
                const int k = t + u * T;
                if (k < p.Cb) {
                    l[lpad(k)] = x[2 * u];
                    if (k != 0 && 2 * k != C) l[lpad(C - k)] = x[2 * u + 1];
                }
            }
        },
        [&](int tid, FftState& s, auto comp_c) {
            constexpr int comp = decltype(comp_c)::value;
            const int g = tid / T, t = tid % T;
            const float* l = lds + g * LF;
            float* o = comp_of<comp>(s);
            if (vec) {
#pragma unroll
                for (int q = 0; q < EMAX / 8; ++q) {
                    const int n0 = 8 * (t + q * T);
                    if (n0 < C) {
#pragma unroll
                        for (int c = 0; c < 8; ++c) o[q * 8 + c] = l[lpad(n0 + c)];
// ... 2470 lines not shown
```

shardmerge_amd/csrc/sm_pipeline.hpp:

```cpp
#pragma once
#include <algorithm>
#include <cmath>
#include <cstdio>
#include <map>
#include <string>
#include <vector>

#include "../../include/shardmerge_hip.h"
#include "sm_kernels.hpp"
#include "sm_aten_norm.hpp"
#include "sm_bluestein.hpp"
#include "sm_lora.hpp"

namespace smhip {

#define SM_KERNEL_TAG(Tag, ParamsT, NAME, CALL)                                      \
    struct Tag {                                                                     \
        using Params = ParamsT;                                                      \
        static constexpr int waves = 4;                                              \
        static constexpr int max_threads = 1024;                                     \
        static const char* name() { return NAME; }                                   \
        template <class Ex> static SM_HD void run(Ex& ex, const Params& p) { CALL; } \
    };
#define SM_KERNEL_TAG_LB(Tag, ParamsT, NAME, CALL, MAXT, WAVES)                      \
    struct Tag {                                                                     \
        using Params = ParamsT;                                                      \
        static constexpr int waves = WAVES;                                          \
        static constexpr int max_threads = MAXT;                                     \
        static const char* name() { return NAME; }                                   \
        template <class Ex> static SM_HD void run(Ex& ex, const Params& p) { CALL; } \
    };
template <class P, int GROUPS> constexpr int fft_max_threads() {
    if constexpr (P::is_static) return (GROUPS * P::T < 256) ? 256 : (GROUPS * P::T > 1024 ? 1024 : GROUPS * P::T);
    else return 1024;
}
#ifndef SM_W3_MAX_THREADS
#define SM_W3_MAX_THREADS 256
#endif
#define SM_FFT_KERNEL_TAG(Tag, ParamsT, NAME, CALL, GROUPS, WAVES)                   \
    template <class P> struct Tag {                                                  \
        using Params = ParamsT;                                                      \
        static constexpr int waves = (WAVES < 4 && P::is_static && fft_max_threads<P, GROUPS>() <= SM_W3_MAX_THREADS) ? WAVES : 4; \
        static constexpr int max_threads = waves < 4 ? fft_max_threads<P, GROUPS>() : 1024; \
        static const char* name() { return NAME; }                                   \
        template <class Ex> static SM_HD void run(Ex& ex, const Params& p) { CALL; } \
    };
SM_FFT_KERNEL_TAG(KF1, F1Params, "f1_rows_fwd", k_f1<P>(ex, p), 1, 3)
SM_FFT_KERNEL_TAG(KF2, F2Params, "f2_cols_fwd", (k_f2<P, f2_bins<P>()>(ex, p)), 2 * f2_bins<P>(), 4)
SM_FFT_KERNEL_TAG(KI1x1, I1Params, "i1_cols_inv", (k_i1<P, 1>(ex, p)), 1, 4)
SM_FFT_KERNEL_TAG(KI1x2, I1Params, "i1_cols_inv", (k_i1<P, i1_bins<P>()>(ex, p)), i1_bins<P>(), 4)
SM_FFT_KERNEL_TAG(KI2, I2Params, "i2_rows_inv", k_i2<P>(ex, p), 1, 4)
SM_FFT_KERNEL_TAG(KF2S, F2SParams, "f2s_cols_fwd1", (k_f2s<P, f2s_groups<P>()>(ex, p)), f2s_groups<P>(), 4)
SM_FFT_KERNEL_TAG(KF1Q, F1Params, "f1_rows_fwd", k_f1q<P>(ex, p), 4, 4)
SM_FFT_KERNEL_TAG(KF2Q, F2Params, "f2_cols_fwd", (k_f2<P, f2_bins<P>(), true>(ex, p)), 2 * f2_bins<P>(), 4)
SM_FFT_KERNEL_TAG(KF2SQ, F2SParams, "f2s_cols_fwd1", (k_f2s<P, f2s_groups<P>(), true>(ex, p)), f2s_groups<P>(), 4)
SM_FFT_KERNEL_TAG(KI1x1Q, I1Params, "i1_cols_inv", (k_i1<P, 1, true>(ex, p)), 1, 4)
SM_FFT_KERNEL_TAG(KI1x2Q, I1Params, "i1_cols_inv", (k_i1<P, i1_bins<P>(), true>(ex, p)), i1_bins<P>(), 4)
#define SM_BLUE_KERNEL_TAG(Tag, ParamsT, NAME, CALL)                                 \
    template <class P> struct Tag {                                                  \
        using Params = ParamsT;                                                      \
        static constexpr int max_threads = fft_max_threads<P, 1>();                  \
        static constexpr int waves = max_threads > 512 ? 4 : 2;                      \
        static const char* name() { return NAME; }                                   \
        template <class Ex> static SM_HD void run(Ex& ex, const Params& p) { CALL; } \
    };
SM_BLUE_KERNEL_TAG(KF1B, F1BParams, "f1_rows_fwd", k_f1b<P>(ex, p))
SM_BLUE_KERNEL_TAG(KI2B, I2BParams, "i2_rows_inv", k_i2b<P>(ex, p))
SM_FFT_KERNEL_TAG(KPair1d, Pair1dParams, "pair_1d", k_pair1d<P>(ex, p), 1, 1)

#ifndef SM_COLS_MAX_THREADS
#define SM_COLS_MAX_THREADS 1024
#endif
#ifndef SM_F2_MAX_THREADS
#define SM_F2_MAX_THREADS 512
#endif
#ifndef SM_R14336
#define SM_R14336 16, 16, 8, 7
#endif
#ifndef SM_R7168
#define SM_R7168 32, 32, 7
#endif
#ifndef SM_T8192
#define SM_T8192 256
#define SM_W8192 4
#define SM_R8192 32, 16, 16
#endif
#define SM_STATIC_PLANS(X)                 \
    X(SPlan<1024, 64, false, 4, 32, 32>)       \
    X(SPlan<2048, 64, false, 4, 16, 16, 8>)    \
    X(SPlan<4096, 128, false, 4, 16, 16, 16>)  \
    X(SPlan<8192, SM_T8192, false, SM_W8192, SM_R8192>)  \
    X(SPlan<16384, 512, false, 4, 32, 32, 16>)\
    X(SPlan<14336, 512, false, 4, SM_R14336>) \
    X(SPlan<28672, 1024, false, 4, 16, 16, 16, 7>) \
    X(SPlan<3072, 128, false, 4, 16, 16, 4, 3>)    \
    X(SPlan<3584, 128, false, 4, 16, 32, 7>)       \
    X(SPlan<5120, 256, false, 4, 16, 16, 4, 5>)    \
    X(SPlan<6144, 256, false, 4, 16, 16, 8, 3>)    \
    X(SPlan<7168, 256, false, 4, SM_R7168>)    \
    X(SPlan<12288, 512, false, 4, 16, 16, 16, 3>)  \
    X(SPlan<13824, 512, false, 4, 32, 16, 3, 3, 3>) \
    X(SPlan<27648, 1024, false, 4, 32, 32, 3, 3, 3>) \
    X(SPlan<2304, 128, false, 4, 16, 16, 3, 3>) \
    X(SPlan<256, 64, false, 4, 8, 8, 4>)            \
    X(SPlan<512, 64, false, 4, 32, 16>)             \
    X(SPlan<64, 64, false, 4, 8, 8>)                \
    X(SPlan<128, 64, false, 4, 16, 8>)

inline bool plan_uses_cx(int N) { (void)N; return false; }

template <class PL> inline void plan_from_static(int N, int& T, std::vector<int>& radices, bool& found) {
    if (!found && PL::N == N) {
        T = PL::T; radices.clear();
        for (int i = 0; i < PL::npass; ++i) radices.push_back(PL::radix(i));
        found = true;
    }
}
inline bool plan_shape_static(int N, int& T, std::vector<int>& radices) {
    bool found = false;
#define SM_PLAN_FROM(...) plan_from_static<__VA_ARGS__>(N, T, radices, found);
    SM_STATIC_PLANS(SM_PLAN_FROM)
#undef SM_PLAN_FROM
    return found;
}

template <class PL>
inline bool plan_matches(const FftPlanDev& pl) {
    if (pl.N != PL::N || pl.T != PL::T || pl.npass != PL::npass || pl.lds_floats != PL::lds_floats || (pl.cx != 0) != PL::cx) return false;
    for (int i = 0; i < PL::npass; ++i)
        if (pl.radix[i] != PL::radix(i)) return false;
    return true;
}
SM_KERNEL_TAG(KF2R1, F2Params, "f2_cols_fwd", k_f2_r1(ex, p))
SM_KERNEL_TAG(KI1R1, I1Params, "i1_cols_inv", k_i1_r1(ex, p))
SM_KERNEL_TAG(KPublish, PublishParams, "publish", k_publish(ex, p))
SM_KERNEL_TAG(KHist, HistParams, "select_hist", k_hist(ex, p))
SM_KERNEL_TAG(KScan, ScanParams, "select_scan", k_scan(ex, p))
SM_KERNEL_TAG(KSelect2, Select2Params, "select_lvl2", k_select2<false>(ex, p))
SM_KERNEL_TAG(KSelect2Cull, Select2Params, "select_lvl2_cull", k_select2<false>(ex, p))
SM_KERNEL_TAG(KBlendSel, Select2Params, "blend", k_select2<true>(ex, p))
SM_KERNEL_TAG(KSpecCheck, SpecCheckParams, "select_spec_check", k_spec_check(ex, p))
SM_KERNEL_TAG(KSelect3, Select3Params, "select_lvl3_cand", k_select3(ex, p))
SM_KERNEL_TAG(KReduceCand, ReduceCandParams, "slerp_reduce_cand", k_reduce_cand(ex, p))
SM_KERNEL_TAG(KReduce, ReduceParams, "slerp_reduce", k_reduce(ex, p))
SM_KERNEL_TAG(KSlerpConsts, SlerpConstParams, "slerp_consts", k_slerp_consts(ex, p))
SM_KERNEL_TAG_LB(KClassEmf, ClassEmfParams, "class_norm_stats", k_class_emf(ex, p), 256, 2)
SM_KERNEL_TAG(KSumPartials, SumPartialsParams, "sum_partials", k_sum_partials(ex, p))
SM_KERNEL_TAG(KDeltaNorms, DeltaNormsParams, "delta_norms", k_delta_norms(ex, p))
SM_KERNEL_TAG(KSumPartialsN, SumNParams, "sum_partials", k_sum_partials_n(ex, p))
SM_KERNEL_TAG(KBlend, BlendParams, "blend", k_blend(ex, p))
SM_KERNEL_TAG(KCombine, CombineParams, "combine", k_combine(ex, p))
SM_KERNEL_TAG(KExpand, ExpandParams, "expand_full", k_expand(ex, p))
SM_KERNEL_TAG(KPack, PackParams, "pack_planes", k_pack(ex, p))
SM_KERNEL_TAG(KSplit, SplitParams, "split_complex", k_split(ex, p))
SM_KERNEL_TAG(KJoin, JoinParams, "join_complex", k_join(ex, p))
SM_KERNEL_TAG(KCull, CullParams, "cull_inplace", k_cull(ex, p))
SM_KERNEL_TAG(KAddition, AdditionParams, "addition_merge", k_addition(ex, p))
SM_KERNEL_TAG(KFnSums, FnSumsParams, "fn_slerp_sums", k_fn_sums(ex, p))
SM_KERNEL_TAG(KFnSlerpFin, FnSlerpFinParams, "fn_slerp_consts", k_fn_slerp_fin(ex, p))
SM_KERNEL_TAG(KFnSlerpRows0, FnSlerpRowsParams, "fn_slerp_relnorm", k_fn_slerp_rows<0>(ex, p))
SM_KERNEL_TAG(KFnSlerpRows1, FnSlerpRowsParams, "fn_slerp_out", k_fn_slerp_rows<1>(ex, p))
SM_KERNEL_TAG(KFnSlerpDen, FnSlerpDenParams, "fn_slerp_den", k_fn_slerp_den(ex, p))
SM_KERNEL_TAG(KSumsqAny, SumsqAnyParams, "fn_sumsq", k_sumsq_any(ex, p))
SM_KERNEL_TAG(KDivScalar, DivScalarParams, "fn_div_scalar", k_div_scalar(ex, p))
SM_KERNEL_TAG(KCorrPartial, CorrPartialParams, "correlate_pairs", k_corr_partial(ex, p))
SM_KERNEL_TAG(KCorrFinish, CorrFinishParams, "correlate_finish", k_corr_finish(ex, p))
SM_KERNEL_TAG(KSerialNorm, SerialNormParams, "serial_norm", k_serial_norm(ex, p))
SM_KERNEL_TAG(KSpecNorm, SpecNormParams, "spec_norm", k_spec_norm(ex, p))
SM_KERNEL_TAG(KSumsqCand, SumsqCandParams, "spec_norm_cand", k_sumsq_cand(ex, p))
SM_KERNEL_TAG(KSumSpec, SumSpecParams, "spec_norm_sum", k_sum_spec(ex, p))
SM_KERNEL_TAG(KSpecRescale, SpecRescaleParams, "spec_rescale", k_spec_rescale(ex, p))
SM_KERNEL_TAG(KDftp, DftpParams, "dft_across_slices", k_dftp(ex, p))
SM_KERNEL_TAG(KDftpPairs, DftpParams, "dft_across_slices", k_dftp_pairs(ex, p))
SM_KERNEL_TAG(KTranspose, TransposeParams, "transpose", k_transpose(ex, p))
SM_KERNEL_TAG_LB(KLoraPack, LoraPackParams, "lora_pack", k_lora_pack(ex, p), 256, 4)
SM_KERNEL_TAG_LB(KLoraBf16, LoraApplyParams, "lora_apply", k_lora_apply<DT_BF16>(ex, p), 256, 2)
SM_KERNEL_TAG_LB(KLoraF16, LoraApplyParams, "lora_apply", k_lora_apply<DT_F16>(ex, p), 256, 2)
SM_KERNEL_TAG_LB(KLoraF32, LoraApplyParams, "lora_apply", k_lora_apply<DT_F32>(ex, p), 256, 2)
SM_KERNEL_TAG_LB(KDoraNormBf16, LoraApplyParams, "dora_norm", k_dora_norm<DT_BF16>(ex, p), 256, 2)
SM_KERNEL_TAG_LB(KDoraNormF16, LoraApplyParams, "dora_norm", k_dora_norm<DT_F16>(ex, p), 256, 2)
SM_KERNEL_TAG_LB(KDoraNormF32, LoraApplyParams, "dora_norm", k_dora_norm<DT_F32>(ex, p), 256, 2)
SM_KERNEL_TAG_LB(KDoraScale, DoraScaleParams, "dora_scale", k_dora_scale(ex, p), DORA_SCALE_THREADS, 4)
SM_KERNEL_TAG_LB(KDoraApplyBf16, LoraApplyParams, "dora_apply", k_dora_apply<DT_BF16>(ex, p), 256, 2)
SM_KERNEL_TAG_LB(KDoraApplyF16, LoraApplyParams, "dora_apply", k_dora_apply<DT_F16>(ex, p), 256, 2)
SM_KERNEL_TAG_LB(KDoraApplyF32, LoraApplyParams, "dora_apply", k_dora_apply<DT_F32>(ex, p), 256, 2)
SM_KERNEL_TAG_LB(KAtenPre, AtenPreParams, "aten_norm_pre", k_aten_pre<0>(ex, p), 256, 4)
SM_KERNEL_TAG_LB(KAtenPreC, AtenPreParams, "aten_norm_pre", k_aten_pre<1>(ex, p), 256, 4)
SM_KERNEL_TAG_LB(KAtenScan, AtenScanParams, "aten_norm_scan", k_aten_scan(ex, p), 256, 4)
SM_KERNEL_TAG_LB(KAtenRec, AtenRecParams, "aten_norm_rec", k_aten_rec(ex, p), 256, 4)
#ifndef SM_ATEN_PART_WAVES
#define SM_ATEN_PART_WAVES 3
#endif
SM_KERNEL_TAG_LB(KAtenPart16, AtenPartParams, "aten_norm_part", k_aten_part<ATEN_PART_RAW16>(ex, p), 256, SM_ATEN_PART_WAVES)
SM_KERNEL_TAG_LB(KAtenPart32, AtenPartParams, "aten_norm_part", k_aten_part<ATEN_PART_RAW32>(ex, p), 256, SM_ATEN_PART_WAVES)
SM_KERNEL_TAG_LB(KAtenPart, AtenPartParams, "aten_norm_part", k_aten_part<ATEN_PART_SIGNAL>(ex, p), 256, 2)
SM_KERNEL_TAG_LB(KAtenPartC, AtenPartParams, "aten_norm_part", k_aten_part<ATEN_PART_CLASS>(ex, p), 256, 2)
SM_KERNEL_TAG_LB(KAtenWalk, AtenWalkParams, "aten_norm_walk", k_aten_walk<0>(ex, p), 256, 4)
SM_KERNEL_TAG_LB(KAtenWalkC, AtenWalkParams, "aten_norm_walk", k_aten_walk<1>(ex, p), 256, 4)
SM_KERNEL_TAG_LB(KAtenFinish, AtenFinishParams, "aten_norm_finish", k_aten_finish(ex, p), 256, 4)
#define SM_SIDE_KERNELS_0(X) X(KAtenPre) X(KAtenPreC) X(KAtenScan) X(KAtenRec) X(KAtenPart16) X(KAtenPart32) X(KAtenPart) X(KAtenPartC) X(KAtenWalk) X(KAtenWalkC) X(KAtenFinish)
#define SM_SIDE_KERNELS_1(X) X(KF2R1) X(KI1R1) X(KPublish) X(KHist) X(KScan) X(KSelect2) X(KSelect2Cull) X(KBlendSel) \
    X(KSpecCheck) X(KSelect3) X(KReduceCand) X(KReduce) X(KSlerpConsts) X(KSumPartials) X(KClassEmf)
#define SM_SIDE_KERNELS_2(X) X(KDeltaNorms) X(KSumPartialsN) X(KBlend) X(KCombine) X(KExpand) X(KPack) X(KSplit) X(KJoin) \
    X(KCull) X(KAddition) X(KFnSums) X(KFnSlerpFin) X(KFnSlerpRows0) X(KFnSlerpRows1) X(KFnSlerpDen) X(KSumsqAny) X(KDivScalar) X(KCorrPartial) X(KCorrFinish) X(KSerialNorm) X(KSpecNorm) X(KSumsqCand) X(KSumSpec)       \
    X(KSpecRescale) X(KDftp) X(KDftpPairs) X(KTranspose) X(KLoraPack) X(KLoraBf16) X(KLoraF16) X(KLoraF32) \
    X(KDoraNormBf16) X(KDoraNormF16) X(KDoraNormF32) X(KDoraScale) X(KDoraApplyBf16) X(KDoraApplyF16) X(KDoraApplyF32)
#define SM_SIDE_GROUPS 7

struct HostPlan {
    FftPlanDev dev;
    bool ok = false;
};

inline bool plan_radices(int N, int T, std::vector<int>& out) {
    out.clear();
    if (N == 1) { out.push_back(1); return true; }
    int rest = N, a = 0;
    while (rest % 2 == 0) { rest /= 2; ++a; }
    std::vector<int> odd;
    for (int p : {3, 5, 7, 11, 13})
        while (rest % p == 0) { rest /= p; odd.push_back(p); }
    if (rest != 1) return false;
    if (a > 0) {
        const int np = (a + 4) / 5;
        const int base = a / np, extra = a % np;
        for (int i = 0; i < np; ++i) out.push_back(1 << (base + (i < extra ? 1 : 0)));
    }
    for (int p : odd) out.push_back(p);
    if ((int)out.size() > MAX_PASSES) return false;
    for (int r : out) {
        const int nb = N / r;
        const int per = (nb + T - 1) / T;
        if (per * r > EMAX) return false;
    }
    return true;
}


inline bool plan_shape(int N, int& T, std::vector<int>& radices) {
    if (N < 1 || N > EMAX * 1024) return false;
    if (plan_shape_static(N, T, radices)) return true;
    int t0 = ((N + EMAX - 1) / EMAX + 63) / 64 * 64;
    if (t0 < 64) t0 = 64;
    for (T = t0; T <= 1024; T += 64)
        if (plan_radices(N, T, radices)) return true;
    return false;
}

inline bool rough_split(int N, int& p, int& M) {
    int T;
    std::vector<int> rad;
    if (plan_shape(N, T, rad)) { p = 1; M = N; return true; }
    for (p = 2; p <= DFTP_MAX_P; ++p) {
        if (N % p) continue;
        M = N / p;
        if (M % 2 == 0 && plan_shape(M, T, rad)) return true;
    }
    return false;
}
inline int bluestein_len(int C) {
    if (C < 2) return 0;
    for (int L = 256; L <= EMAX * 1024; L *= 2)
        if (L >= 2 * C - 1) return L;
    return 0;
}
inline int shape_support(int rows, int cols, bool* transposed = nullptr) {
    int T, p, M;
    std::vector<int> rad;
    if (transposed) *transposed = false;
    if (rows < 1 || cols < 1) return 0;
    if (plan_shape(cols, T, rad) && rough_split(rows, p, M)) return 1;
    if (plan_shape(rows, T, rad) && rough_split(cols, p, M)) { if (transposed) *transposed = true; return 1; }
    if (bluestein_len(cols) && rough_split(rows, p, M)) return 1;
    if (bluestein_len(rows) && rough_split(cols, p, M)) { if (transposed) *transposed = true; return 1; }
    return 0;
}

struct Buffer {
    void* p = nullptr;
    size_t cap = 0;
};

struct ProfEntry { std::string name; uint64_t launches = 0; double ms = 0; };

inline size_t round_up(size_t v, size_t m) { return (v + m - 1) / m * m; }

struct PairOut {
    void* out = nullptr; int out_mode = OUT_F32;
    const void* base = nullptr; int base_dtype = DT_BF16;
    float post = 1.f;
    int ifft_policy = 1;
};

template <class B>
class Pipeline {
  public:
    B be;
    std::string err;
    void* stream = nullptr;
    uint32_t debug_cand_cap = 0;
    uint32_t debug_sel_chunks = 0;
    bool debug_flush_always = false;
    bool spec_cull = true;
    size_t spec_min_bins = 1 << 20;
    bool dftp_pairs_enabled = true;
    int debug_force_split = 0;
    int sel_wgs_per_cu = 5;
    bool safe_select = false;
    uint32_t noise_seed_base = 0;
    bool spectral_inter = true;
    bool f2s_pair = true;
    size_t f2s_pair_max_bins = (size_t)64 << 20;
    bool f1_multi = true;
    bool fuse_spec_norm = true;
    float noise_sigma = 1.2e-7f;

    explicit Pipeline(int device) : be(device) {}
    ~Pipeline() {
        for (auto& kv : plans_) if (kv.second.dev.tw) be.free((void*)kv.second.dev.tw);
        for (Buffer* b : {&cand_, &t1_, &small_, &tmpA_, &tmpB_, &tmpC_, &fullS_, &saveR_, &saveI_, &aten_, &emf_, &lora_, &dora_}) if (b->p) be.free(b->p);
        for (Buffer& b : pool_) if (b.p) be.free(b.p);
        if (mail_) be.free_host(mail_);
        for (Buffer& b : inter_) if (b.p) be.free(b.p);
        for (Buffer& b : rowspec_) if (b.p) be.free(b.p);
        for (Buffer& b : tr_) if (b.p) be.free(b.p);
        for (auto& kv : rough_tw_) if (kv.second) be.free(kv.second);
        for (auto& kv : blue_) { if (kv.second.chirp) be.free(kv.second.chirp); if (kv.second.filt) be.free(kv.second.filt); }
    }

    int fail(int code, const std::string& msg) { err = msg; return code; }

    int get_plan(int N, FftPlanDev& out) {
        auto it = plans_.find(N);
        if (it == plans_.end()) {
            HostPlan hp;
            int T;
            std::vector<int> rad;
            if (plan_shape(N, T, rad)) {
                hp.ok = true;
                hp.dev.N = N; hp.dev.T = T; hp.dev.npass = (int)rad.size();
                for (int i = 0; i < MAX_PASSES; ++i) hp.dev.radix[i] = i < (int)rad.size() ? rad[i] : 1;
                hp.dev.cx = plan_uses_cx(N) ? 1 : 0;
                hp.dev.lds_floats = hp.dev.cx ? (int)round_up((size_t)2 * (N + (N >> 4) + 1), 32)
                                              : (int)round_up((size_t)lpad(N) + 1, 32);
                std::vector<cf2> tw(N);
                for (int j = 0; j < N; ++j) {
                    const double ang = -2.0 * M_PI * (double)j / (double)N;
                    tw[j].x = (float)cos(ang); tw[j].y = (float)sin(ang);
                }
                void* d = be.alloc(sizeof(cf2) * N);
                if (!d) return fail(SMHIP_ERR_NOMEM, "twiddle alloc failed");
                be.h2d(d, tw.data(), sizeof(cf2) * N, stream);
                hp.dev.tw = (const cf2*)d;
            } else {
                hp.dev.tw = nullptr;
            }
            it = plans_.emplace(N, hp).first;
        }
        if (!it->second.ok) {
            char buf[256];
            snprintf(buf, sizeof buf, "unsupported transform length %d (a row length needs factors in {2,3,5,7,11,13} and <= %d; the layer merge "
                                       "also takes p * M column lengths, p <= %d)", N, EMAX * 1024, DFTP_MAX_P);
            return fail(SMHIP_ERR_SHAPE, buf);
        }
        out = it->second.dev;
        return SMHIP_OK;
    }

    int ensure(Buffer& b, size_t bytes) {
        if (b.cap >= bytes) return SMHIP_OK;
        if (b.p) { be.sync(stream); be.free(b.p); b.p = nullptr; b.cap = 0; }
        b.p = be.alloc(bytes);
        if (!b.p) return fail(SMHIP_ERR_NOMEM, "workspace allocation failed");
        b.cap = bytes;
        return SMHIP_OK;
    }
    size_t workspace_bytes() const {
        size_t t = cand_.cap + t1_.cap + small_.cap + tmpA_.cap + tmpB_.cap + tmpC_.cap + fullS_.cap + saveR_.cap + saveI_.cap + aten_.cap + emf_.cap + lora_.cap + dora_.cap;
        for (const Buffer& b : inter_) t += b.cap;
        for (const Buffer& b : rowspec_) t += b.cap;
        for (const Buffer& b : pool_) t += b.cap;
        for (const Buffer& b : tr_) t += b.cap;
        return t;
    }

    struct Geo {
        int R, C, Cb, pitch4, pitchG, ilv;
        size_t plane_floats;
        bool full;
        int Cw;
        int fold;
        int batch;
        size_t t1_slice;
        int rough;
    };
#ifndef SM_FOLD_MIN_ROWS
#define SM_FOLD_MIN_ROWS 14336
#endif
    int fold_min_rows = SM_FOLD_MIN_ROWS;
    bool fold_shape(int R, int C) const {
        if (R < fold_min_rows || !(R == 8192 || R == 14336 || R == 16384 || R == 28672)) return false;
        int T; std::vector<int> rad;
        if (!plan_shape_static(C, T, rad)) return false;
        return 4 * T <= 1024 && (C / T) % 2 == 0 && C % 8 == 0;
    }
    bool fold_enabled = true;
    Geo geo(int R, int C, bool full = false, bool allow_fold = false, int batch = 1) const {
        Geo g;
        g.R = R; g.C = C; g.full = full;
        g.batch = batch < 1 ? 1 : batch;
        g.fold = (allow_fold && fold_enabled && !full && g.batch == 1 && fold_shape(R, C) && !row_bluestein(C)) ? 4 : 1;
        g.Cb = full ? C : (C / 2 + 1) * g.batch;
        g.pitch4 = (int)round_up((size_t)(C / 2 + 1), 8);
        g.t1_slice = round_up((size_t)R, 8) * (size_t)g.pitch4;
        g.pitchG = g.pitch4;
        g.ilv = t1_interleave(R);
        g.plane_floats = round_up((size_t)g.Cb * R, 64);
        g.Cw = full ? -1 : C;
        g.rough = 1;
        return g;
    }
#ifndef SM_T1_ILV
#define SM_T1_ILV 2
#endif
#ifndef SM_T1_ILV_MIN_ROWS
#define SM_T1_ILV_MIN_ROWS 8192
#endif
    static int t1_interleave(int R) { return t1_interleave_rows(R); }
    static constexpr int MAXGRID_PART = 1 << 20;
    int reserve(int R, int C, bool full = false, int batch = 1) {
        const Geo g = geo(R, C, full, false, batch);
        int rc;
        if ((rc = ensure(t1_, g.t1_slice * g.batch * sizeof(cf4)))) return rc;
        for (int i = 0; i < 4; ++i)
            if ((rc = ensure(pool_[pidx_[i]], g.plane_floats * sizeof(float)))) return rc;
        {
            const size_t ck = std::max<size_t>(1 << 16, g.plane_floats / 4), cp = std::max<size_t>(1 << 15, g.plane_floats / 16);
            if ((rc = ensure(cand_, ck * 4 + cp * 16))) return rc;
            cap_keys_ = (uint32_t)std::min<size_t>(ck, 0xffffffffu); cap_pairs_ = (uint32_t)std::min<size_t>(cp, 0xffffffffu);
        }
        if (!small_.p) {
            if ((rc = ensure(small_, SMALL_BYTES))) return rc;
            be.memset(small_.p, 0, SMALL_BYTES, stream);
            if (!mail_) mail_ = (Mailbox*)be.alloc_host(sizeof(Mailbox));
            if (!mail_) return fail(SMHIP_ERR_NOMEM, "host mailbox");
        }
        return SMHIP_OK;
    }
    static constexpr size_t OFF_HIST = 0;
    static constexpr size_t OFF_SEL = OFF_HIST + 8 * (HIST1_BINS + 2 * HIST_LO_BINS);
    static constexpr size_t OFF_CONSTS = OFF_SEL + 2 * sizeof(SelState);
    static constexpr size_t OFF_THR = OFF_CONSTS + 256;
    static constexpr size_t OFF_FLAGS = OFF_THR + 64;
    static constexpr size_t OFF_CANDCTR = OFF_FLAGS + 32;
    static constexpr size_t OFF_NORM2 = OFF_FLAGS + 64;
    static constexpr size_t OFF_PART = OFF_NORM2 + 64;
    static constexpr size_t PART_DOUBLES = 4 * 65536 + 2 * 40000;
    static constexpr size_t OFF_PART_IM = OFF_PART + PART_DOUBLES * 8;
    static constexpr size_t PART_IM_DOUBLES = 131072;
    static constexpr size_t OFF_SPEC = OFF_PART_IM + PART_IM_DOUBLES * 8;
    static constexpr size_t SMALL_BYTES = OFF_SPEC + 64;
    unsigned long long* d_hist() { return (unsigned long long*)((char*)small_.p + OFF_HIST); }
    unsigned long long* d_hist2() { return d_hist() + HIST1_BINS; }
    unsigned long long* d_hist3() { return d_hist2() + HIST_LO_BINS; }
    SelState* d_sel(int i) { return (SelState*)((char*)small_.p + OFF_SEL) + i; }
    BlendConsts* d_consts() { return (BlendConsts*)((char*)small_.p + OFF_CONSTS); }
    float* d_thr(int i) { return (float*)((char*)small_.p + OFF_THR) + i; }
    uint32_t* d_flags() { return (uint32_t*)((char*)small_.p + OFF_FLAGS); }
    uint32_t* d_candctr() { return (uint32_t*)((char*)small_.p + OFF_CANDCTR); }
    CandLists cand_lists() {
        CandLists c;
        c.keys = (uint32_t*)cand_.p; c.pairs = (cf4*)((char*)cand_.p + (size_t)cap_keys_ * 4);
        c.cap_keys = cap_keys_; c.cap_pairs = cap_pairs_; c.counters = d_candctr();
        if (debug_cand_cap) { c.cap_keys = std::min(c.cap_keys, debug_cand_cap); c.cap_pairs = std::min(c.cap_pairs, debug_cand_cap); }
        return c;
    }
    double* d_norm2() { return (double*)((char*)small_.p + OFF_NORM2); }
    double* d_part() { return (double*)((char*)small_.p + OFF_PART); }
    double* d_part_im() { return (double*)((char*)small_.p + OFF_PART_IM); }
    uint32_t* d_spec_guess(int slot) { return (uint32_t*)((char*)small_.p + OFF_SPEC) + (slot < 0 ? 0 : slot > 7 ? 7 : slot); }
    uint32_t* d_spec_flag() { return (uint32_t*)((char*)small_.p + OFF_SPEC) + 8; }
    float* plane(const Geo&, int i) { return (float*)pool_[pidx_[i]].p; }
    enum { P_REA = 0, P_IMA = 1, P_REB = 2, P_RER = 3 };
    int pool_acquire(size_t bytes) {
        int id = -1;
        for (size_t q = 0; q < pool_.size(); ++q) if (!pool_busy_[q]) { id = (int)q; break; }
        if (id < 0) { pool_.emplace_back(); pool_busy_.push_back(0); id = (int)pool_.size() - 1; }
        if (ensure(pool_[id], bytes)) return -1;
        pool_busy_[id] = 1;
        return id;
    }
    void pool_release(int id) { if (id >= 0) pool_busy_[id] = 0; }

    static bool is_static_plan(const FftPlanDev& pl) {
        bool found = false;
#define SM_IS_PLAN(...) if (plan_matches<__VA_ARGS__>(pl)) found = true;
        SM_STATIC_PLANS(SM_IS_PLAN)
#undef SM_IS_PLAN
        return found;
    }
    static int f2_bins_host(const FftPlanDev& pl) { return is_static_plan(pl) ? f2_bins_for(pl.T, pl.N) : 1; }
    static int i1_bins_host(const FftPlanDev& pl) {
        if (2 * pl.T > SM_F2_MAX_THREADS) return 1;
        return is_static_plan(pl) ? i1_bins_for(pl.T) : 2;
    }

    template <template <class> class KT, class Params>
    void launch_fft(const FftPlanDev& pl, int grid, int block, size_t lds, const Params& p, bool allow_static = true) {
        bool done = !allow_static;
#define SM_TRY_PLAN(...)                                                     \
        if (!done && plan_matches<__VA_ARGS__>(pl)) {                        \
            be.template launch<KT<__VA_ARGS__>>(grid, block, lds, p, stream);\
            done = true;                                                     \
        }
        SM_STATIC_PLANS(SM_TRY_PLAN)
#undef SM_TRY_PLAN
        if (!done || !allow_static) be.template launch<KT<DynPlan>>(grid, block, lds, p, stream);
    }

    static int pick_chunks(size_t units, int block, int min_chunks, int wgs_per_cu = 5) {
        const size_t target = (size_t)256 * wgs_per_cu;
        size_t c = (units + (size_t)block * target - 1) / ((size_t)block * target);
        if (c < (size_t)min_chunks) c = min_chunks;
        if (c > 4096) c = 4096;
        return (int)c;
    }
    static int stream_grid(size_t units, int block, int chunks) {
        const size_t per = (size_t)block * chunks;
        size_t g = (units + per - 1) / per;
        return (int)std::max<size_t>(g, 1);
    }
    static bool aligned16(const void* p) { return ((uintptr_t)p & 15) == 0; }
    static int vec4(const Geo& g) { return g.full ? (((size_t)g.R * g.C) % 4 == 0) : (g.R % 4 == 0); }

    bool debug_force_bluestein = false;
    bool row_bluestein(int C) const {
        int T; std::vector<int> rad;
        if (debug_force_bluestein) return bluestein_len(C) > 0;
        return !plan_shape(C, T, rad) && bluestein_len(C) > 0;
    }
    struct BlueHost { void* chirp = nullptr; void* filt = nullptr; int L = 0; };
    int bluestein_tables(int C, BluesteinTab& out, FftPlanDev& plan) {
        const int L = bluestein_len(C);
        if (!L) return fail(SMHIP_ERR_SHAPE, "row length too long for the chirp-z transform");
        int rc = get_plan(L, plan);
        if (rc) return rc;
        auto it = blue_.find(C);
        if (it == blue_.end()) {
            std::vector<double> wr(C), wi(C);
            for (int n = 0; n < C; ++n) {
                const unsigned long long m = ((unsigned long long)n * (unsigned long long)n) % (2ull * (unsigned long long)C);
                const double ang = -M_PI * (double)m / (double)C;
                wr[n] = cos(ang); wi[n] = sin(ang);
            }
            std::vector<double> hr(L, 0.0), hi(L, 0.0);
            for (int m = 0; m < C; ++m) {
                hr[m] = wr[m]; hi[m] = -wi[m];
                if (m) { hr[L - m] = wr[m]; hi[L - m] = -wi[m]; }
            }
            for (int i = 1, j = 0; i < L; ++i) {
                int bit = L >> 1;
                for (; j & bit; bit >>= 1) j ^= bit;
                j ^= bit;
                if (i < j) { std::swap(hr[i], hr[j]); std::swap(hi[i], hi[j]); }
            }
            for (int len = 2; len <= L; len <<= 1) {
                const int half = len / 2;
                for (int k = 0; k < half; ++k) {
                    const double ang = -2.0 * M_PI * (double)k / (double)len;
                    const double cr = cos(ang), ci = sin(ang);
                    for (int i = k; i < L; i += len) {
                        const int j = i + half;
                        const double tr = hr[j] * cr - hi[j] * ci, ti = hr[j] * ci + hi[j] * cr;
                        hr[j] = hr[i] - tr; hi[j] = hi[i] - ti;
                        hr[i] += tr; hi[i] += ti;
                    }
                }
            }
            std::vector<cf2> chirp(C), filt(L);
            for (int n = 0; n < C; ++n) { chirp[n].x = (float)wr[n]; chirp[n].y = (float)wi[n]; }
            for (int k = 0; k < L; ++k) { filt[k].x = (float)(hr[k] / L); filt[k].y = (float)(hi[k] / L); }
            BlueHost bh;
            bh.L = L;
            bh.chirp = be.alloc(sizeof(cf2) * C);
            bh.filt = be.alloc(sizeof(cf2) * L);
            if (!bh.chirp || !bh.filt) return fail(SMHIP_ERR_NOMEM, "chirp table alloc failed");
            be.h2d(bh.chirp, chirp.data(), sizeof(cf2) * C, stream);
            be.h2d(bh.filt, filt.data(), sizeof(cf2) * L, stream);
            be.sync(stream);
            it = blue_.emplace(C, bh).first;
        }
        out.chirp = (const cf2*)it->second.chirp; out.filt = (const cf2*)it->second.filt;
        return SMHIP_OK;
    }
    int get_row_plan(int C, FftPlanDev& plan, bool& blue, BluesteinTab& bt) {
        blue = row_bluestein(C);
        bt.chirp = nullptr; bt.filt = nullptr;
        return blue ? bluestein_tables(C, bt, plan) : get_plan(C, plan);
    }

    int rough_twiddles(int N, const cf2** out) {
        auto it = rough_tw_.find(N);
        if (it == rough_tw_.end()) {
            std::vector<cf2> tw(N);
            for (int j = 0; j < N; ++j) {
                const double ang = -2.0 * M_PI * (double)j / (double)N;
                tw[j].x = (float)cos(ang); tw[j].y = (float)sin(ang);
            }
            void* d = be.alloc(sizeof(cf2) * N);
            if (!d) return fail(SMHIP_ERR_NOMEM, "twiddle alloc failed");
            be.h2d(d, tw.data(), sizeof(cf2) * N, stream);
            be.sync(stream);
            it = rough_tw_.emplace(N, d).first;
        }
        *out = (const cf2*)it->second;
        return SMHIP_OK;
    }
    int run_dftp(const Geo& g, void* buf, bool rowpair, int ilv, int pitch, size_t slice_stride, bool inverse) {
        DftpParams q;
        int rc = rough_twiddles(g.R * g.rough, &q.tw);
        if (rc) return rc;
        q.buf = (cf4*)buf; q.p = g.rough; q.M = g.R; q.units = rowpair ? g.R / 2 : g.R; q.rowpair = rowpair ? 1 : 0;
        q.ilv = ilv; q.pitch = pitch; q.ncols = g.C / 2 + 1; q.slice_stride = slice_stride; q.inverse = inverse ? 1 : 0;
        q.cols = DFTP_COLS;
        if (q.p <= DFTP_PAIR_MAX_P && dftp_pairs_enabled) {
            q.cols = dftp_pairs_cols(q.p);
            const int ntp = (q.ncols + q.cols - 1) / q.cols;
            const size_t ldsp = LDS_SCRATCH_FLOATS * 4 + dftp_pairs_lds_bytes(q.p) + ((size_t)(q.p / 2 + 1) + 64) * sizeof(cf2);
            be.template launch<KDftpPairs>((q.units + DFTP_UNITS - 1) / DFTP_UNITS * ntp, 256, ldsp, q, stream);
            return SMHIP_OK;
        }
        const int ntiles = (q.ncols + DFTP_COLS - 1) / DFTP_COLS;
        const size_t lds = LDS_SCRATCH_FLOATS * 4 + (size_t)q.p * DFTP_COLS * sizeof(cf4) + (size_t)q.p * sizeof(cf2);
        be.template launch<KDftp>(q.units * ntiles, 256, lds, q, stream);
        return SMHIP_OK;
    }

    int run_f1(const Geo& g, const SigDesc& a, const SigDesc& b, int& grid_out) {
        F1Params p;
        bool blue; BluesteinTab bt;
        int rc = get_row_plan(g.C, p.plan, blue, bt);
        if (rc) return rc;
        p.a = a; p.b = b; p.R = g.R; p.C = g.C; p.Cb = g.C / 2 + 1; p.pitch4 = g.pitch4; p.ilv = g.ilv;
        p.sigs.n = 0;
        p.fuse.prefix = nullptr; p.fuse.grp = nullptr; p.fuse.nchunks = 0; p.fuse.sig0 = 0; p.fuse_rowpair = 0;
        p.nb = blue ? 1 : std::max(1, 256 / p.plan.T);
        p.row_stride = (size_t)g.C;
        p.vec = !blue && (g.C % 8 == 0) && aligned16(a.x) && aligned16(a.base) && aligned16(b.x) && aligned16(b.base);
        if (fused_.armed && p.vec && g.batch == 1 && g.rough == 1) { p.fuse = fused_.af; p.fuse_rowpair = 0; fused_.used = true; }
        p.t1 = (cf4*)t1_.p;
        p.partials = d_part();
        p.R2 = 0; p.rowpair = 0; p.Rcol = g.R; p.twR = nullptr; p.slab_elems = fold_slab_elems(g);
        if (g.fold == 4) {
            if (!p.vec) return fail(SMHIP_ERR_ARG, "internal: folded row pass on unaligned input");
            FftPlanDev colp;
            if ((rc = get_plan(g.R, colp))) return rc;
            p.R2 = g.R / 4; p.twR = colp.tw; p.ilv = FOLD_ILV; p.nb = 4;
            const int gridq = (int)round_up((size_t)p.R2, 8 * p.ilv);
            if ((size_t)gridq * 2 > PART_DOUBLES) return fail(SMHIP_ERR_SHAPE, "too many rows");
            launch_fft<KF1Q>(p.plan, gridq, 4 * p.plan.T, (LDS_SCRATCH_FLOATS + (size_t)4 * p.plan.lds_floats) * 4, p);
            grid_out = gridq;
            return SMHIP_OK;
        }
        const int xg = p.ilv > p.nb ? p.ilv / p.nb : 1;
        const bool joint = joint_rows(g);
        const int nlaunch = joint ? 1 : g.batch;
        if (joint) p.R = g.R * g.rough;
        const int grid = (int)round_up((size_t)(p.R + p.nb - 1) / p.nb, 8 * xg);
        if ((size_t)grid * 2 * nlaunch > PART_DOUBLES) return fail(SMHIP_ERR_SHAPE, "too many rows");
        const size_t lds = (LDS_SCRATCH_FLOATS + (size_t)p.nb * p.plan.lds_floats) * 4;
        for (int bi = 0; bi < nlaunch; ++bi) {
            p.a = sig_at(a, (size_t)bi * g.R * g.C); p.b = sig_at(b, (size_t)bi * g.R * g.C);
            p.t1 = (cf4*)t1_.p + (size_t)bi * g.t1_slice;
            p.partials = d_part() + (size_t)bi * 2 * grid;
            if (blue) { F1BParams q; q.f = p; q.bt = bt; launch_fft<KF1B>(p.plan, grid, p.plan.T, lds, q); }
            else launch_fft<KF1>(p.plan, grid, p.nb * p.plan.T, lds, p, p.vec != 0);
        }
        grid_out = grid * nlaunch;
        if (g.rough > 1) return run_dftp(g, t1_.p, false, p.ilv, g.pitch4, g.t1_slice, false);
        return SMHIP_OK;
    }
    static size_t dt_size(int dt) { return dt == DT_F32 ? 4 : 2; }
    static SigDesc sig_at(const SigDesc& s, size_t elems) {
        SigDesc r = s;
        if (r.x) r.x = (const char*)r.x + elems * dt_size(s.dtype);
        if (r.base) r.base = (const char*)r.base + elems * dt_size(s.dtype);
        return r;
    }
    static size_t fold_slab_elems(const Geo& g, bool rowpair = false) {
        return round_up((size_t)g.R / (rowpair ? 8 : 4), 8) * (size_t)g.pitch4;
    }
    static bool joint_rows(const Geo& g) { return g.rough > 1 && g.R % 16 == 0; }
    int run_f1_rowpairs(const Geo& g, const SigDesc& sig, void* t1buf = nullptr, double* partials = nullptr, int* grid_out = nullptr,
                        F1Sigs* multi = nullptr) {
        F1Params p;
        bool blue; BluesteinTab bt;
        int rc = get_row_plan(g.C, p.plan, blue, bt);
        if (rc) return rc;
        SigDesc a = sig, b = sig;
        b.x = (const char*)sig.x + (size_t)g.C * dt_size(sig.dtype);
        if (sig.base) b.base = (const char*)sig.base + (size_t)g.C * dt_size(sig.dtype);
        p.a = a; p.b = b; p.R = g.R / 2; p.C = g.C; p.Cb = g.C / 2 + 1; p.pitch4 = g.pitch4; p.ilv = F2S_ILV;
        p.sigs.n = 0;
        p.fuse.prefix = nullptr; p.fuse.grp = nullptr; p.fuse.nchunks = 0; p.fuse.sig0 = 0; p.fuse_rowpair = 0;
        const int nm = multi ? multi->n : 1;
        if (multi && (blue || nm < 2 || nm > F1_MAX_SIGS)) return SMHIP_ERR_ARG;
        p.nb = blue ? 1 : std::max(1, 256 / p.plan.T);
        p.row_stride = (size_t)2 * g.C;
        p.vec = !blue && (g.C % 8 == 0) && aligned16(a.x) && aligned16(a.base) && aligned16(b.x) && aligned16(b.base);
        if (fused_.armed && p.vec && g.batch == 1 && g.rough == 1) {
            p.fuse = fused_.af; p.fuse.sig0 = multi ? 0 : fused_.next_sig; p.fuse_rowpair = 1; fused_.used = true;
        }
        p.t1 = (cf4*)(t1buf ? t1buf : t1_.p);
        p.partials = partials ? partials : d_part();
        p.R2 = 0; p.rowpair = 0; p.Rcol = g.R; p.twR = nullptr; p.slab_elems = fold_slab_elems(g, true);
        if (g.fold == 4) {
            if (!p.vec) return fail(SMHIP_ERR_ARG, "internal: folded row pass on unaligned input");
            FftPlanDev colp;
            if ((rc = get_plan(g.R, colp))) return rc;
            p.R2 = g.R / 8; p.rowpair = 1; p.twR = colp.tw; p.ilv = F2S_ILV; p.nb = 4;
            const int gridq = (int)round_up((size_t)p.R2, 8 * p.ilv);
            if (multi) {
                if ((size_t)gridq * 2 * nm > PART_DOUBLES) return SMHIP_ERR_ARG;
                for (int i = 0; i < nm; ++i) multi->partials[i] = p.partials + (size_t)i * 2 * gridq;
                multi->b_off = (long long)((size_t)g.C * dt_size(sig.dtype));
                p.sigs = *multi;
            }
            launch_fft<KF1Q>(p.plan, gridq * nm, 4 * p.plan.T, (LDS_SCRATCH_FLOATS + (size_t)4 * p.plan.lds_floats) * 4, p);
            if (grid_out) *grid_out = gridq;
            return SMHIP_OK;
        }
        const int xgs = p.ilv > p.nb ? p.ilv / p.nb : 1;
        const bool joint = joint_rows(g);
        const int nlaunch = joint ? 1 : g.batch;
        if (joint) p.R = g.R * g.rough / 2;
        const int grid = (int)round_up((size_t)(p.R + p.nb - 1) / p.nb, 8 * xgs);
        if (multi && (nlaunch != 1 || g.rough > 1 || (size_t)grid * 2 * nm > PART_DOUBLES || !p.vec)) return SMHIP_ERR_ARG;
        if ((size_t)grid * 2 * nlaunch > PART_DOUBLES) return fail(SMHIP_ERR_SHAPE, "too many rows");
        const size_t lds = (LDS_SCRATCH_FLOATS + (size_t)p.nb * p.plan.lds_floats) * 4;
        cf4* const t1base = p.t1;
        double* const pbase = p.partials;
        if (multi) {
            for (int i = 0; i < nm; ++i) multi->partials[i] = pbase + (size_t)i * 2 * grid;
            multi->b_off = (long long)((size_t)g.C * dt_size(sig.dtype));
            p.sigs = *multi;
            launch_fft<KF1>(p.plan, grid * nm, p.nb * p.plan.T, lds, p, true);
            if (grid_out) *grid_out = grid;
            return SMHIP_OK;
        }
        for (int bi = 0; bi < nlaunch; ++bi) {
            p.a = sig_at(a, (size_t)bi * g.R * g.C); p.b = sig_at(b, (size_t)bi * g.R * g.C);
            p.t1 = t1base + (size_t)bi * (g.t1_slice / 2);
            p.partials = pbase + (size_t)bi * 2 * grid;
            if (blue) { F1BParams q; q.f = p; q.bt = bt; launch_fft<KF1B>(p.plan, grid, p.plan.T, lds, q); }
            else launch_fft<KF1>(p.plan, grid, p.nb * p.plan.T, lds, p, p.vec != 0);
        }
        if (grid_out) *grid_out = grid * nlaunch;
        if (g.rough > 1) return run_dftp(g, t1base, true, F2S_ILV, g.pitch4, g.t1_slice / 2, false);
        return SMHIP_OK;
    }
    struct F2SSecond { const void* t1; bool role_a; float scale; };
    int run_f2s(const Geo& g, bool role_a, float scale, bool hist, const void* t1buf = nullptr, int* im_parts = nullptr,
                const F2SSecond* second = nullptr) {
        F2SParams p;
        p.two = 0; p.t1_2 = nullptr; p.role_a_2 = 0; p.scale_2 = 0.f; p.re_2 = nullptr;
        if (second) {
            if (g.batch != 1 || second->role_a == role_a) return fail(SMHIP_ERR_ARG, "internal: paired column pass");
            p.two = 1; p.t1_2 = (const cf4*)second->t1; p.role_a_2 = second->role_a ? 1 : 0; p.scale_2 = second->scale;
            p.re_2 = plane(g, second->role_a ? P_REA : P_REB);
        }
        const int nsg = second ? 2 : 1;
        const int Rt = g.R / g.fold;
        int rc = get_plan(Rt, p.plan);
        if (rc) return rc;
        p.t1 = (const cf4*)(t1buf ? t1buf : t1_.p); p.pitch4 = g.pitch4 * g.fold; p.R = Rt; p.C = g.C;
        p.Cb = g.fold == 4 ? 4 * g.pitch4 : g.C / 2 + 1;
        p.slab = g.pitch4; p.Cb_real = g.C / 2 + 1; p.Rfull = g.R; p.slab_elems = fold_slab_elems(g, true);
        p.role_a = role_a ? 1 : 0; p.scale = scale;
        p.re = plane(g, role_a ? P_REA : P_REB); p.im = plane(g, P_IMA);
        p.hist = hist ? d_hist() : nullptr;
        const bool st = is_static_plan(p.plan);
        const int G = st ? (f2_nsig_for(p.plan.T) == 2 ? 2 * f2_bins_for(p.plan.T, p.plan.N) : 1) : 1;
        const int xg = G >= 8 ? 1 : 8 / G;
        const int grid = (int)round_up((size_t)(p.Cb + G - 1) / G, 8 * xg) * nsg;
        const size_t lds = (LDS_SCRATCH_FLOATS + (size_t)G * p.plan.lds_floats + HIST1_BINS) * 4;
        const bool any_a = role_a || (second && second->role_a);
        const bool want_im = im_parts && any_a && (size_t)grid * g.batch <= PART_IM_DOUBLES;
        if (im_parts) *im_parts = want_im ? grid * g.batch : -1;
        p.im_partials = want_im ? d_part_im() : nullptr;
        if (g.fold == 4) { launch_fft<KF2SQ>(p.plan, grid, G * p.plan.T, lds, p); return SMHIP_OK; }
        if (g.batch > 1) { p.sl.wgs = grid; p.sl.t1_stride = g.t1_slice / 2; p.sl.plane_stride = (size_t)(g.C / 2 + 1) * g.R; }
        launch_fft<KF2S>(p.plan, grid * g.batch, G * p.plan.T, lds, p);
        return SMHIP_OK;
    }
    void run_spec_norm(const Geo& g, const float* re, const float* im, const float* thr, double& sre, double& sim) {
        const size_t total = (size_t)g.Cb * g.R;
        SpecNormParams q;
        q.re = re; q.im = im; q.R = g.R; q.C = g.Cw; q.Cb = g.Cb; q.vec4 = vec4(g); q.thr = thr;
        q.chunks = pick_chunks((total + 3) / 4, 256, 8, 8);
        int grid = stream_grid((total + 3) / 4, 256, q.chunks);
        while ((size_t)grid * 2 > PART_DOUBLES) { q.chunks *= 2; grid = stream_grid((total + 3) / 4, 256, q.chunks); }
        q.partials = d_part();
        be.template launch<KSpecNorm>(grid, 256, LDS_SCRATCH_FLOATS * 4, q, stream);
        SumPartialsParams sp;
        sp.partials = d_part(); sp.nparts = grid; sp.out = mail_->norm2;
        be.template launch<KSumPartials>(1, 1024, LDS_SCRATCH_FLOATS * 4, sp, stream);
        PublishParams pp;
        pp.flags = d_flags(); pp.thr = d_thr(0); pp.consts = d_consts(); pp.mail = mail_; pp.zero_flags = nullptr;
        be.template launch<KPublish>(1, 64, LDS_SCRATCH_FLOATS * 4, pp, stream);
        be.sync(stream);
        sre = mail_->norm2[0]; sim = mail_->norm2[1];
    }
    void run_spec_rescale(const Geo& g, const float* re, const float* im, float thr, float scale, bool role_a, bool hist,
                          int* im_parts = nullptr) {
        const size_t total = (size_t)g.Cb * g.R;
        SpecRescaleParams q;
        q.re = re; q.im = role_a ? im : nullptr;
        q.dre = plane(g, role_a ? P_REA : P_REB); q.dim = plane(g, P_IMA);
        q.R = g.R; q.C = g.Cw; q.Cb = g.Cb; q.vec4 = vec4(g);
        q.thr = thr; q.scale = scale; q.sigma = noise_sigma; q.seed = ++noise_seed_;
        q.hist = hist ? d_hist() : nullptr;
        q.chunks = pick_chunks((total + 3) / 4, 256, 8, 8);
        const int grid = stream_grid((total + 3) / 4, 256, q.chunks);
        const bool want_im = im_parts && role_a && (size_t)grid <= PART_IM_DOUBLES;
        if (im_parts) *im_parts = want_im ? grid : -1;
        q.im_partials = want_im ? d_part_im() : nullptr;
        be.template launch<KSpecRescale>(grid, 256, (LDS_SCRATCH_FLOATS + HIST1_BINS) * 4, q, stream);
    }
    void run_spec_norm_fused(int sel_parts, int im_parts, double& sre, double& sim) {
        SumsqCandParams sc;
        sc.cand = cand_lists(); sc.thr = d_thr(1); sc.partials = d_part() + 4 * (size_t)sel_parts;
        be.template launch<KSumsqCand>(CAND_GRID, 256, LDS_SCRATCH_FLOATS * 4, sc, stream);
        SumSpecParams sp;
        sp.part4 = d_part(); sp.n4 = sel_parts + CAND_GRID; sp.part1 = d_part_im(); sp.n1 = im_parts; sp.out = mail_->norm2;
        sp.zero_u32 = d_candctr(); sp.zero_u32_count = 3;
        be.template launch<KSumSpec>(1, 1024, LDS_SCRATCH_FLOATS * 4, sp, stream);
        PublishParams pp;
        pp.flags = d_flags(); pp.thr = d_thr(0); pp.consts = d_consts(); pp.mail = mail_; pp.zero_flags = nullptr;
        be.template launch<KPublish>(1, 64, LDS_SCRATCH_FLOATS * 4, pp, stream);
        be.sync(stream);
        sre = mail_->norm2[0]; sim = mail_->norm2[1];
    }

    void read_norms(int grid, double& na, double& nb) {
        SumPartialsParams sp;
        sp.partials = d_part(); sp.nparts = grid; sp.out = mail_->norm2;
        be.template launch<KSumPartials>(1, 1024, LDS_SCRATCH_FLOATS * 4, sp, stream);
        be.sync(stream);
        na = std::sqrt(mail_->norm2[0]); nb = std::sqrt(mail_->norm2[1]);
    }

    int run_f2(const Geo& g, float scale0, float scale1, int swap, bool hist) {
        F2Params p;
        int rc = get_plan(g.R, p.plan);
        if (rc) return rc;
        if (g.R == 1) {
            p.slab = g.pitch4; p.Cb_real = g.C / 2 + 1; p.Rfull = 1; p.slab_elems = 0;
            p.t1 = (const cf4*)t1_.p; p.pitch4 = g.pitch4; p.ilv = 1; p.R = 1; p.C = g.C; p.Cb = g.C / 2 + 1; p.nsig = 2;
            p.swap = swap; p.scale[0] = scale0; p.scale[1] = scale1;
            p.reA = plane(g, P_REA); p.imA = plane(g, P_IMA); p.reB = plane(g, P_REB);
            p.hist = hist ? d_hist() : nullptr;
            be.template launch<KF2R1>(std::max(1, std::min(64, (p.Cb + 255) / 256)), 256, (LDS_SCRATCH_FLOATS + HIST1_BINS) * 4, p, stream);
            return SMHIP_OK;
        }
        p.slab = g.pitch4; p.Cb_real = g.C / 2 + 1; p.Rfull = g.R; p.slab_elems = fold_slab_elems(g);
        if (g.fold == 4) {
            if ((rc = get_plan(g.R / 4, p.plan))) return rc;
            p.t1 = (const cf4*)t1_.p; p.pitch4 = 4 * g.pitch4; p.ilv = FOLD_ILV; p.R = g.R / 4; p.C = g.C; p.Cb = 4 * g.pitch4;
            p.nsig = 2; p.swap = swap; p.scale[0] = scale0; p.scale[1] = scale1;
            p.reA = plane(g, P_REA); p.imA = plane(g, P_IMA); p.reB = plane(g, P_REB);
            p.hist = hist ? d_hist() : nullptr;
            const int binsq = f2_bins_host(p.plan);
            const int gridq = (int)round_up((size_t)(p.Cb + binsq - 1) / binsq, 64);
            const size_t ldsq = (LDS_SCRATCH_FLOATS + (size_t)2 * binsq * p.plan.lds_floats + HIST1_BINS) * 4;
            launch_fft<KF2Q>(p.plan, gridq, 2 * binsq * p.plan.T, ldsq, p);
            return SMHIP_OK;
        }
        p.t1 = (const cf4*)t1_.p; p.pitch4 = g.pitch4; p.ilv = g.ilv; p.R = g.R; p.C = g.C; p.Cb = g.C / 2 + 1;
        p.nsig = f2_nsig_for(p.plan.T);
        p.swap = swap; p.scale[0] = scale0; p.scale[1] = scale1;
        p.reA = plane(g, P_REA); p.imA = plane(g, P_IMA); p.reB = plane(g, P_REB);
        p.hist = hist ? d_hist() : nullptr;
        const int bins = p.nsig == 2 ? f2_bins_host(p.plan) : 1;
        const int ngroups = p.nsig == 2 ? 2 * bins : 1;
        const int grid = p.nsig == 2 ? (int)round_up((size_t)(p.Cb + bins - 1) / bins, 64) : (int)round_up((size_t)p.Cb * 2, 128);
        const size_t lds = (LDS_SCRATCH_FLOATS + (size_t)ngroups * p.plan.lds_floats + HIST1_BINS) * 4;
        if (g.batch > 1) { p.sl.wgs = grid; p.sl.t1_stride = g.t1_slice; p.sl.plane_stride = (size_t)(g.C / 2 + 1) * g.R; }
        launch_fft<KF2>(p.plan, grid * g.batch, ngroups * p.plan.T, lds, p);
        return SMHIP_OK;
    }

    static constexpr int CAND_GRID = 256;
    void run_select(const Geo& g, const float* X, const float* Y, unsigned long long rank, bool level1_done, float* thr_out,
                    bool fuse_reduce = false, int* nparts_out = nullptr, bool sumsq = false, int spec_slot = -1) {
        const size_t total = (size_t)g.Cb * g.R;
        HistParams h;
        h.X = X; h.Y = Y; h.R = g.R; h.C = g.Cw; h.Cb = g.Cb; h.vec4 = vec4(g); h.sel = d_sel(0);
        h.hist = d_hist(); h.chunks = pick_chunks((total + 3) / 4, 256, 8); h.only_if = nullptr;
        const int hgrid = stream_grid((total + 3) / 4, 256, h.chunks);
        const size_t hlds = (LDS_SCRATCH_FLOATS + HIST1_BINS) * 4;
        const size_t scan_lds = (LDS_SCRATCH_FLOATS + 2 * 256 + 32) * 4;
        ScanParams s;
        s.hist = d_hist(); s.sel = d_sel(0); s.value_out = thr_out; s.zero_also = nullptr; s.zero_count = 0;
        s.zero_u32 = nullptr; s.zero_u32_count = 0;
        if (!level1_done) { h.level = 1; be.template launch<KHist>(hgrid, 256, hlds, h, stream); }
        if (nparts_out) *nparts_out = 0;
        if (safe_select) {
            s.nbins = HIST1_BINS; s.shift = 11; s.final_level = 0; s.init = 1; s.rank_init = rank;
            be.template launch<KScan>(1, 256, scan_lds, s, stream);
            for (int level = 2; level <= 3; ++level) {
                h.level = level;
                be.template launch<KHist>(hgrid, 256, hlds, h, stream);
                s.nbins = HIST_LO_BINS; s.shift = 10; s.final_level = (level == 3); s.init = 0;
                be.template launch<KScan>(1, 256, scan_lds, s, stream);
            }
            return;
        }
        Select2Params q;
        q.X = X; q.Y = Y; q.R = g.R; q.C = g.Cw; q.Cb = g.Cb; q.vec4 = vec4(g); q.sel = d_sel(0);
        q.hist1 = d_hist(); q.rank = rank; q.hist = d_hist2();
        q.cand = cand_lists(); q.fuse_reduce = (fuse_reduce && Y) ? 1 : 0; q.partials = d_part();
        q.sumsq = (sumsq && !Y) ? 1 : 0;
        q.flush_always = debug_flush_always ? 1 : 0;
        q.chunks = debug_sel_chunks ? (int)debug_sel_chunks : pick_chunks((total + 3) / 4, 256, 8, sel_wgs_per_cu);
        int grid2 = stream_grid((total + 3) / 4, 256, q.chunks);
        while ((size_t)(grid2 + CAND_GRID) * 4 > PART_DOUBLES) { q.chunks *= 2; grid2 = stream_grid((total + 3) / 4, 256, q.chunks); }
        const size_t lds2 = (LDS_SCRATCH_FLOATS + HIST_LO_BINS + 8 + STAGE_KEYS) * 4 + (size_t)STAGE_PAIRS * sizeof(cf4);
        q.skip = nullptr; q.blendB = nullptr; q.blendR = nullptr; q.consts = nullptr; q.t_sum = 0.f; q.hist1_out = nullptr; q.guess = nullptr;
        if (spec_slot >= 0) {
            SpecCheckParams sc;
            sc.hist1 = d_hist(); sc.rank = rank; sc.guess = d_spec_guess(spec_slot); sc.flag = d_spec_flag();
            sc.sel = d_sel(0); sc.hist2 = d_hist2(); sc.counters = d_candctr();
            be.template launch<KSpecCheck>(1, 256, LDS_SCRATCH_FLOATS * 4 + (256 + 16) * 8 + 16, sc, stream);
            q.skip = d_spec_flag();
            be.template launch<KSelect2Cull>(grid2, 256, lds2, q, stream);
        } else {
            be.template launch<KSelect2>(grid2, 256, lds2, q, stream);
        }

        Select3Params t3;
        t3.cand = q.cand; t3.sel = d_sel(0); t3.hist2 = d_hist2(); t3.hist = d_hist3();
        be.template launch<KSelect3>(CAND_GRID, 256, (LDS_SCRATCH_FLOATS + HIST_LO_BINS + 8 + 2 * 256 + 32) * 4, t3, stream);

        s.hist = d_hist3(); s.sel = d_sel(1); s.nbins = HIST_LO_BINS; s.shift = 10; s.final_level = 1; s.init = 0;
        s.zero_also = d_hist(); s.zero_count = HIST1_BINS + HIST_LO_BINS;
        if (!q.fuse_reduce && !q.sumsq) { s.zero_u32 = d_candctr(); s.zero_u32_count = 3; }
        be.template launch<KScan>(1, 256, scan_lds, s, stream);

        if (q.sumsq && nparts_out) *nparts_out = grid2;
        if (q.fuse_reduce) {
            ReduceCandParams rc;
            rc.cand = q.cand; rc.thr = thr_out; rc.partials = d_part() + 4 * (size_t)grid2;
            be.template launch<KReduceCand>(CAND_GRID, 256, LDS_SCRATCH_FLOATS * 4, rc, stream);
            if (nparts_out) *nparts_out = grid2 + CAND_GRID;
        }
    }

    void run_blend(const Geo& g, int mode, int agreement, float t, float t_sum, bool hist) {
        const size_t total = (size_t)g.Cb * g.R;
        BlendParams b;
        b.reA = plane(g, P_REA); b.reB = plane(g, P_REB); b.reR = plane(g, P_RER);
        b.R = g.R; b.C = g.Cw; b.Cb = g.Cb; b.vec4 = vec4(g);
        b.mode = mode; b.agreement = agreement; b.t = t; b.t_sum = t_sum;
        b.consts = d_consts(); b.hist = hist ? d_hist() : nullptr; b.chunks = pick_chunks((total + 3) / 4, 256, 8, 8);
        be.template launch<KBlend>(stream_grid((total + 3) / 4, 256, b.chunks), 256, (LDS_SCRATCH_FLOATS + HIST1_BINS) * 4, b, stream);
    }

    void run_blend_spec(const Geo& g, float t_sum, bool sumsq, int spec_slot) {
        const size_t total = (size_t)g.Cb * g.R;
        Select2Params q;
        q.X = plane(g, P_REA); q.Y = nullptr; q.R = g.R; q.C = g.Cw; q.Cb = g.Cb; q.vec4 = vec4(g); q.sel = d_sel(0);
        q.hist1 = nullptr; q.rank = 0; q.hist = d_hist2();
        q.cand = cand_lists(); q.fuse_reduce = 0; q.partials = d_part(); q.sumsq = sumsq ? 1 : 0;
        q.flush_always = debug_flush_always ? 1 : 0;
        q.chunks = cull_select_chunks(total);
        q.skip = nullptr;
        q.blendB = plane(g, P_REB); q.blendR = plane(g, P_RER); q.consts = d_consts(); q.t_sum = t_sum;
        q.hist1_out = d_hist(); q.guess = d_spec_guess(spec_slot);
        const int grid = stream_grid((total + 3) / 4, 256, q.chunks);
        const size_t lds = (LDS_SCRATCH_FLOATS + HIST_LO_BINS + 8 + STAGE_KEYS + HIST1_BINS) * 4;
        be.template launch<KBlendSel>(grid, 256, lds, q, stream);
    }
    long last_spec_verdict() {
        if (!small_.p) return -1;
        uint32_t v = 0;
        be.d2h(&v, d_spec_flag(), sizeof v, stream);
        be.sync(stream);
        return (long)v;
    }
    void spec_totals(unsigned long long* checked, unsigned long long* hits) {
        uint32_t v[3] = {0, 0, 0};
        if (small_.p) { be.d2h(v, d_spec_flag(), sizeof v, stream); be.sync(stream); }
        *checked = v[1]; *hits = v[2];
    }
    int cull_select_chunks(size_t total) const {
        int chunks = debug_sel_chunks ? (int)debug_sel_chunks : pick_chunks((total + 3) / 4, 256, 8, sel_wgs_per_cu);
        int grid2 = stream_grid((total + 3) / 4, 256, chunks);
        while ((size_t)(grid2 + CAND_GRID) * 4 > PART_DOUBLES) { chunks *= 2; grid2 = stream_grid((total + 3) / 4, 256, chunks); }
        return chunks;
    }

    void run_slerp_consts(const Geo& g, bool have_thr, float t, int fused_parts, const float* ref_norms = nullptr,
                          const double* emf_part = nullptr, int emf_nparts = 0, int emf_elo = 0) {
        const size_t total = (size_t)g.Cb * g.R;
        SlerpConstParams c;
        c.ref_norms = ref_norms; c.emf_part = emf_part; c.emf_nparts = emf_nparts; c.emf_elo = emf_elo;
        c.fallback = nullptr; c.nfallback = 0; c.overflow = nullptr;
        c.thr = have_thr ? d_thr(0) : nullptr; c.t = t; c.out = d_consts();
        c.zero_u32 = nullptr; c.zero_u32_count = 0;
        if (fused_parts > 0) {
            c.zero_u32 = d_candctr(); c.zero_u32_count = 3;
            c.partials = d_part(); c.nparts = fused_parts;
        } else {
            ReduceParams r;
            r.reA = plane(g, P_REA); r.reB = plane(g, P_REB); r.R = g.R; r.C = g.Cw; r.Cb = g.Cb; r.vec4 = vec4(g);
            r.thr = c.thr; r.chunks = pick_chunks((total + 3) / 4, 256, 16, 8); r.only_if = nullptr;
            int grid = stream_grid((total + 3) / 4, 256, r.chunks);
            while ((size_t)grid * 4 > PART_DOUBLES) { r.chunks *= 2; grid = stream_grid((total + 3) / 4, 256, r.chunks); }
            r.partials = d_part();
            be.template launch<KReduce>(grid, 256, LDS_SCRATCH_FLOATS * 4, r, stream);
            c.partials = r.partials; c.nparts = grid;
        }
        be.template launch<KSlerpConsts>(1, 256, (2 * LDS_SCRATCH_FLOATS + 4 * EMF_VALS + 8) * 4, c, stream);
    }

    int run_inverse(const Geo& g, const float* reR, const float* imA, const float* cull_thr, const PairOut& o,
                    int* norm_grid = nullptr, float cull_val = 0.f) {
        I1Params a;
        int rc = get_plan(g.R, a.plan);
        if (rc) return rc;
        const int Cb = g.C / 2 + 1;
        a.cull_thr = cull_thr; a.cull_val = cull_val; a.R = g.R; a.Cb = Cb;
        a.G = (cf2*)t1_.p; a.pitchG = g.pitchG;
        a.s = g.R == 1 ? 1 : i1_bins_host(a.plan);
        const size_t lds1 = (LDS_SCRATCH_FLOATS + (size_t)a.s * a.plan.lds_floats) * 4;
        const int grid1 = (int)round_up((size_t)(Cb + a.s - 1) / a.s, 8 * (16 / a.s));

        I2Params b;
        bool blue; BluesteinTab bt;
        if ((rc = get_row_plan(g.C, b.plan, blue, bt))) return rc;
        b.G = (const cf2*)t1_.p; b.pitchG = g.pitchG; b.R = g.R; b.C = g.C; b.Cb = Cb;
        b.nb = blue ? 1 : std::max(1, 256 / b.plan.T);
        b.vec = !blue && (g.C % 8 == 0) && aligned16(o.out) && aligned16(o.base);
        b.inv_n = (float)(1.0 / ((double)g.R * (double)g.rough * (double)g.C));
        b.ifft_policy = o.ifft_policy;
        b.post = o.post; b.base_dtype = o.base_dtype; b.out_mode = o.out_mode;
        b.flags = d_flags();
        const bool joint = joint_rows(g);
        if (joint) b.R = g.R * g.rough;
        const int pairs = (b.R + 1) / 2;
        const int grid2 = (pairs + b.nb - 1) / b.nb;
        const int nrow_launch = joint ? 1 : g.batch;
        const bool want_norm = norm_grid && (size_t)grid2 * 2 * nrow_launch <= PART_DOUBLES;
        if (norm_grid) *norm_grid = want_norm ? grid2 * nrow_launch : -1;
        const size_t lds2 = (LDS_SCRATCH_FLOATS + (size_t)b.nb * b.plan.lds_floats) * 4;
        const size_t pslice = (size_t)Cb * g.R, eslice = (size_t)g.R * g.C;
        const int phases = g.rough > 1 ? 2 : 1;
        for (int phase = 0; phase < phases; ++phase) {
        if (phase == 1 && (rc = run_dftp(g, t1_.p, true, 1, g.pitchG, g.t1_slice / 2, true))) return rc;
        for (int bi = 0; bi < g.batch; ++bi) {
            if (g.rough > 1) { a.G = (cf2*)t1_.p + (size_t)bi * g.t1_slice; b.G = a.G; }
            a.reR = reR + bi * pslice; a.imA = imA + bi * pslice;
            if (phases == 2 && phase == 0 && g.R > 1) {
                if (bi > 0) break;
                a.G = (cf2*)t1_.p;
                a.sl.wgs = grid1; a.sl.t1_stride = g.t1_slice; a.sl.plane_stride = pslice;
                const int gridj = grid1 * g.batch;
                if (a.s >= 2) launch_fft<KI1x2>(a.plan, gridj, a.s * a.plan.T, lds1, a);
                else launch_fft<KI1x1>(a.plan, gridj, a.plan.T, lds1, a);
                continue;
            }
            if (phases == 2 && phase == 1) {
            } else
            if (g.R == 1) {
                be.template launch<KI1R1>(std::max(1, std::min(64, (Cb + 255) / 256)), 256, LDS_SCRATCH_FLOATS * 4, a, stream);
            } else if (g.fold == 4) {
                if (a.s >= 2) launch_fft<KI1x2Q>(a.plan, grid1, a.s * a.plan.T, lds1, a);
                else launch_fft<KI1x1Q>(a.plan, grid1, a.plan.T, lds1, a);
            } else if (a.s >= 2) launch_fft<KI1x2>(a.plan, grid1, a.s * a.plan.T, lds1, a);
            else launch_fft<KI1x1>(a.plan, grid1, a.plan.T, lds1, a);
            if (phases == 2 && phase == 0) continue;
            if (joint) { if (bi > 0) break; b.G = (const cf2*)t1_.p; }
            b.base = o.base ? (const char*)o.base + bi * eslice * dt_size(o.base_dtype) : nullptr;
            b.out = (char*)o.out + bi * eslice * (o.out_mode == OUT_BF16 ? 2 : 4);
            b.norm_partials = want_norm ? d_part() + (size_t)bi * 2 * grid2 : nullptr;
            if (blue) { I2BParams q; q.i = b; q.bt = bt; launch_fft<KI2B>(b.plan, grid2, b.plan.T, lds2, q); }
            else launch_fft<KI2>(b.plan, grid2, b.nb * b.plan.T, lds2, b, b.vec != 0);
        }
        }
        return SMHIP_OK;
    }

    void run_combine(const SigDesc& a, const SigDesc& b, float ca, float cb, size_t n, float* out_f32,
                     const PairOut* fin, bool want_norms, int* grid_out = nullptr) {
        CombineParams c;
        c.a = a; c.b = b; c.ca = ca; c.cb = cb; c.n = n; c.out_f32 = out_f32;
        c.base = fin ? fin->base : nullptr; c.base_dtype = fin ? fin->base_dtype : DT_BF16;
        c.out_final = fin ? fin->out : nullptr; c.out_mode = fin ? fin->out_mode : OUT_F32;
        c.flags = d_flags();
        c.vec8 = (n % 8 == 0) && aligned16(a.x) && aligned16(a.base) && aligned16(b.x) && aligned16(b.base) &&
                 aligned16(out_f32) && aligned16(c.base) && aligned16(c.out_final);
        c.chunks = pick_chunks((n + 7) / 8, 256, 4, 8);
        int grid = stream_grid((n + 7) / 8, 256, c.chunks);
        while ((size_t)grid * 2 > PART_DOUBLES) { c.chunks *= 2; grid = stream_grid((n + 7) / 8, 256, c.chunks); }
        c.partials = want_norms ? d_part() : nullptr;
        be.template launch<KCombine>(grid, 256, LDS_SCRATCH_FLOATS * 4, c, stream);
        if (grid_out) *grid_out = grid;
    }

    void publish(bool zero_flags) {
        PublishParams pp;
        pp.flags = d_flags(); pp.thr = d_thr(0); pp.consts = d_consts(); pp.mail = mail_;
        pp.zero_flags = zero_flags ? d_flags() : nullptr;
        be.template launch<KPublish>(1, 64, LDS_SCRATCH_FLOATS * 4, pp, stream);
        be.sync(stream);
        if (zero_flags) flags_clean_ = true;
    }
    void read_blend_info(smhip_blend_info* info, bool have_cut, bool have_cull, bool have_consts, bool published = false) {
        if (!info) return;
        if (!published) publish(false);
        const BlendConsts c = mail_->consts;
        float thr[4];
        for (int i = 0; i < 4; ++i) thr[i] = mail_->thr[i];
        info->cutoff_threshold = have_cut ? thr[0] : 0.0;
        info->cull_threshold = have_cull ? thr[1] : 0.0;
        info->dot = have_consts ? c.dot : 0.0;
        info->s00 = have_consts ? c.s00 : 0.0; info->s01 = have_consts ? c.s01 : 0.0; info->s11 = have_consts ? c.s11 : 0.0;
        info->n_slerp = have_consts ? c.n_slerp : 0;
        info->t = 0.0; info->cull_pct = 0.0;
    }

    static unsigned long long pct_index(unsigned long long len, double pct) {
        unsigned long long idx = (unsigned long long)((double)len * pct);
        if (idx >= len) idx = len - 1;
        return idx;
    }

    void spectral_blend(const Geo& g, int mode, double t, double t_sum, double cutoff_pct, double cull_pct,
                        int agreement, bool level1_hist_done, bool& have_cull, int* sumsq_parts = nullptr, int spec_slot = 7) {
        const unsigned long long nfull = (unsigned long long)g.R * g.C * (unsigned long long)g.batch;
        have_cull = false;
        if (mode == BLEND_SLERP) {
            const bool have_cut = cutoff_pct > 0;
            int fused = 0;
            if (have_cut)
                run_select(g, plane(g, P_REA), plane(g, P_REB), pct_index(2 * nfull, cutoff_pct), level1_hist_done, d_thr(0),
                           true, &fused);
            const float* class_norms = nullptr;
            const double* emf_part = nullptr;
            int emf_nparts = 0, emf_elo = 0;
            if (ref_mode_ && class_norms_mode == 2 && !g.full) {
                AtenSrc cs[2];
                for (int w = 0; w < 2; ++w) {
                    memset(&cs[w], 0, sizeof(AtenSrc));
                    cs[w].kind = 1; cs[w].reA = plane(g, P_REA); cs[w].reB = plane(g, P_REB);
                    cs[w].thr = have_cut ? d_thr(0) : nullptr; cs[w].which = w;
                    cs[w].R = g.R; cs[w].C = g.Cw; cs[w].Cb = g.Cb; cs[w].n = (size_t)g.Cb * g.R;
                }
                if (run_aten_norms(cs, 2, false)) class_norms = d_aten_out();
            } else if (ref_mode_ && class_norms_mode == 1) {
                ClassEmfParams q;
                q.reA = plane(g, P_REA); q.reB = plane(g, P_REB); q.thr = have_cut ? d_thr(0) : nullptr;
                q.R = g.R; q.C = g.Cw; q.Cb = g.Cb; q.n = (size_t)g.Cb * g.R;
                q.elo = (int)std::floor(std::log2(0.03 * (double)nfull + 1.0)) - 11;
                q.sample = 1;
                while (q.sample < emf_max_sample && q.n / (2 * (size_t)q.sample) >= EMF_MIN_SAMPLED) q.sample *= 2;
                const size_t rows = (q.n + 7) / 8, npieces = (rows + 8 * (size_t)q.sample - 1) / (8 * (size_t)q.sample);
                q.iters = (int)std::max<size_t>(1, std::min<size_t>(64, (npieces + (size_t)32 * 384 - 1) / ((size_t)32 * 384)));
                const int grid = (int)std::max<size_t>(1, (npieces + (size_t)32 * q.iters - 1) / ((size_t)32 * q.iters));
                if (!ensure(emf_, (size_t)grid * 2 * EMF_VALS * sizeof(double))) {
                    q.partials = (double*)emf_.p;
                    be.template launch<KClassEmf>(grid, 256, LDS_SCRATCH_FLOATS * 4 * 2, q, stream);
                    emf_part = q.partials; emf_nparts = grid; emf_elo = q.elo;
                }
            }
            run_slerp_consts(g, have_cut, (float)t, fused, class_norms, emf_part, emf_nparts, emf_elo);
            const bool spec = cull_pct > 0 && spec_cull && !safe_select && !g.full && (size_t)g.Cb * g.R >= spec_min_bins;
            if (spec) run_blend_spec(g, (float)t_sum, sumsq_parts != nullptr, spec_slot);
            else run_blend(g, BLEND_SLERP, 1, (float)t, (float)t_sum, cull_pct > 0);
            if (sumsq_parts) *sumsq_parts = 0;
            if (cull_pct > 0) {
                run_select(g, plane(g, P_RER), nullptr, pct_index(nfull, cull_pct), true, d_thr(1), false, sumsq_parts,
                           sumsq_parts != nullptr, spec ? spec_slot : -1);
                have_cull = true;
            }
        } else {
            run_blend(g, BLEND_ARITH, agreement, (float)t, 1.f, false);
        }
    }

    bool pair1d_enabled = true;
    bool pair1d_ok(const Geo& g) const {
        return pair1d_enabled && g.R == 1 && g.batch == 1 && !g.full && g.C >= 2 && g.C <= PAIR1D_MAX_C && !row_bluestein(g.C);
    }
    int run_pair1d(const Geo& g, const SigDesc& A, const SigDesc& Bs, double na, double nb, double t, double t_sum,
                   double cutoff_pct, double cull_pct, const PairOut& o, int* norm_parts) {
        Pair1dParams q;
        int rc = get_plan(g.C, q.plan);
        if (rc) return rc;
        q.a = A; q.b = Bs; q.C = g.C;
        q.sa = (float)(1.0 / na); q.sb = (float)(1.0 / nb);
        q.t = (float)t; q.t_sum = (float)t_sum;
        const unsigned long long nfull = (unsigned long long)g.C;
        q.have_cut = cutoff_pct > 0; q.rank_cut = pct_index(2 * nfull, cutoff_pct);
        q.have_cull = cull_pct > 0; q.rank_cull = pct_index(nfull, cull_pct);
        memset(&q.fin, 0, sizeof q.fin);
        q.fin.R = 1; q.fin.C = g.C; q.fin.Cb = g.C / 2 + 1;
        q.fin.inv_n = (float)(1.0 / (double)g.C);
        q.fin.ifft_policy = o.ifft_policy; q.fin.post = o.post;
        q.fin.base = o.base; q.fin.base_dtype = o.base_dtype; q.fin.out = o.out; q.fin.out_mode = o.out_mode;
        q.fin.flags = d_flags();
        q.fin.norm_partials = norm_parts ? d_part() : nullptr;
        if (norm_parts) *norm_parts = 1;
        q.thr = d_thr(0); q.consts = d_consts();
        const size_t lds = (LDS_SCRATCH_FLOATS + (size_t)q.plan.lds_floats + 2 * (size_t)g.C + HIST1_BINS + 1024 + 64 + 16) * 4;
        launch_fft<KPair1d>(q.plan, 1, q.plan.T, lds, q);
        return SMHIP_OK;
    }

    int merge_pair_slerp(const float* v0, const float* v1, int R, int C, double t, double bthr, double t_sum,
                         double cutoff_pct, double cull_pct, float* out, double* n0o, double* n1o, int* branch,
                         smhip_blend_info* info) {
        return with_select_retry([&] {
            return merge_pair_slerp_once(v0, v1, R, C, t, bthr, t_sum, cutoff_pct, cull_pct, out, n0o, n1o, branch, info);
        });
    }
    int merge_pair_slerp_once(const float* v0, const float* v1, int R, int C, double t, double bthr, double t_sum,
                              double cutoff_pct, double cull_pct, float* out, double* n0o, double* n1o, int* branch,
                              smhip_blend_info* info) {
        const Geo g = geo(R, C, false, aligned16(v0) && aligned16(v1) && aligned16(out));
        int rc = reserve(R, C);
        if (rc) return rc;
        clear_flags();
        SigDesc a{v0, nullptr, DT_F32, 1.f}, b{v1, nullptr, DT_F32, 1.f};
        int grid;
        if ((rc = run_f1(g, a, b, grid))) return rc;
        double n0, n1;
        read_norms(grid, n0, n1);
        n0 = (double)(float)n0; n1 = (double)(float)n1;
        if (n0o) *n0o = n0;
        if (n1o) *n1o = n1;
        const size_t n = (size_t)R * C;
        if (n1 < 1e-4 || n0 < 1e-4) {
            if (branch) *branch = SMHIP_BRANCH_EARLY_V0;
            SigDesc none{nullptr, nullptr, DT_F32, 1.f};
            run_combine(a, none, n0 != 0 ? (float)(1.0 / n0) : 1.f, 0.f, n, out, nullptr, false);
            read_blend_info(info, false, false, false);
            return SMHIP_OK;
        }
        const double ratio = n1 / (n0 + 1e-10);
        PairOut po;
        po.out = out; po.out_mode = OUT_F32; po.post = 1.f;
        if (ratio < bthr) {
            if (branch) *branch = SMHIP_BRANCH_LINEAR;
            if ((rc = run_f2_linear(g, (float)(1.0 / n0), (float)(1.0 / n1), (float)t))) return rc;
            if ((rc = run_inverse(g, plane(g, P_RER), plane(g, P_IMA), nullptr, po))) return rc;
            read_blend_info(info, false, false, false);
            return check_flags(true, false);
        }
        if (branch) *branch = SMHIP_BRANCH_SLERP;
        if ((rc = run_f2(g, (float)(1.0 / n0), (float)(1.0 / n1), 0, cutoff_pct > 0))) return rc;
        bool have_cull;
        spectral_blend(g, BLEND_SLERP, t, t_sum, cutoff_pct, cull_pct, 1, true, have_cull);
        if ((rc = run_inverse(g, plane(g, P_RER), plane(g, P_IMA), have_cull ? d_thr(1) : nullptr, po))) return rc;
        read_blend_info(info, cutoff_pct > 0, have_cull, true);
        if (info) { info->t = t; info->cull_pct = cull_pct; }
        return check_flags(true, false);
    }

    int run_f2_linear(const Geo& g, float s0, float s1, float t) {
        int rc = run_f2(g, s0, s1, 0, false);
        if (rc) return rc;
        const size_t total = (size_t)g.Cb * g.R;
        run_blend(g, BLEND_ARITH, 0, t, 1.f, false);
        if ((rc = ensure(tmpC_, g.plane_floats * sizeof(float)))) return rc;
        SigDesc ia{plane(g, P_IMA), nullptr, DT_F32, 1.f}, none{nullptr, nullptr, DT_F32, 1.f};
        run_combine(ia, none, 1.f, 0.f, total, (float*)tmpC_.p, nullptr, false);
        if ((rc = run_f2(g, s0, s1, 1, false))) return rc;
        SigDesc ib{plane(g, P_IMA), nullptr, DT_F32, 1.f}, ia2{tmpC_.p, nullptr, DT_F32, 1.f};
        run_combine(ia2, ib, 1.f, t, total, plane(g, P_IMA), nullptr, false);
        return SMHIP_OK;
    }

    void clear_flags() {
        if (!small_.p && reserve(1, 1)) return;
        if (!flags_clean_) be.memset(d_flags(), 0, 48, stream);
        flags_clean_ = false;
        overflow_seen_ = false;
    }
    bool select_overflowed() {
        uint32_t v = 0;
        publish(false);
        v = mail_->flags[11];
        return v != 0;
    }
    template <class F>
    int with_select_retry(F&& body) {
        int rc = body();
        if (!safe_select && overflow_seen_) {
            safe_select = true;
            rc = body();
            safe_select = false;
        }
        return rc;
    }

    int check_flags(bool ifft_stage, bool final_stage, uint32_t* nan_ifft = nullptr, uint32_t* nan_final = nullptr) {
        uint32_t f[12];
        publish(true);
        for (int i = 0; i < 12; ++i) f[i] = mail_->flags[i];
        if (f[11] && !safe_select) { overflow_seen_ = true; return SMHIP_OK; }
        if (nan_ifft) *nan_ifft = f[0];
        if (nan_final) *nan_final = f[2];
        if (ifft_stage && f[1]) return fail(SMHIP_ERR_INF_IFFT, "Inf in ifft output");
        if (final_stage && f[3]) return fail(SMHIP_ERR_INF_MERGED, "Inf in merged tensor");
        return SMHIP_OK;
    }

    int pair_arith(const SigDesc& a_in, const SigDesc& b_in, int R, int C, float sa, float sb, double t, int agreement,
                   const PairOut& po, double na_hint, double nb_hint, const Geo* layer_geo = nullptr) {
        const Geo g = layer_geo ? *layer_geo
                                : geo(R, C, false, aligned16(a_in.x) && aligned16(a_in.base) && aligned16(b_in.x) && aligned16(b_in.base) &&
                                                   aligned16(po.out) && aligned16(po.base));
        int rc = reserve(g.R, g.C, false, g.batch);
        if (rc) return rc;
        SigDesc a = a_in, b = b_in;
        int grid;
        double na = na_hint, nb = nb_hint;
        if (na < 0 || nb < 0) {
            if ((rc = run_f1(g, a, b, grid))) return rc;
            read_norms(grid, na, nb);
            na *= std::fabs(sa); nb *= std::fabs(sb);
        } else {
            na *= std::fabs(sa); nb *= std::fabs(sb);
            grid = -1;
        }
        float pre = 1.f;
        if (nb == 0) { b.x = nullptr; b.base = nullptr; }
        if (nb > 0 && na > 0 && (nb < na * 0.25 || nb > na * 4.0)) {
            int e;
            std::frexp(na / nb, &e);
            pre = std::ldexp(1.f, e - 1);
        }
        if (pre != 1.f || grid < 0 || nb == 0) {
            b.prescale = b_in.prescale * pre;
            if ((rc = run_f1(g, a, b, grid))) return rc;
        }
        if ((rc = run_f2(g, sa, sb / pre, 0, false))) return rc;
        bool have_cull;
        spectral_blend(g, BLEND_ARITH, t, 1.0, 0, 0, agreement, false, have_cull);
        return run_inverse(g, plane(g, P_RER), plane(g, P_IMA), nullptr, po);
    }

    static void correlated_pairs_least(const std::vector<float>& norms, int m, std::vector<std::pair<int, int>>& out) {
        out.clear();
        std::vector<char> used(m, 0);
        std::vector<float> corr((size_t)m * m, 0.f);
        for (int i = 0; i < m; ++i)
            for (int j = i + 1; j < m; ++j) corr[(size_t)i * m + j] = norms[i] * norms[j];
        for (;;) {
            float best = INFINITY;
            bool any = false;
            for (int i = 0; i < m; ++i)
                for (int j = i + 1; j < m; ++j)
                    if (!used[i] && !used[j]) { any = true; best = std::min(best, std::fabs(corr[(size_t)i * m + j])); }
            if (!any) break;
            int bx = -1, by = -1;
            for (int i = 0; i < m && bx < 0; ++i)
                for (int j = i + 1; j < m; ++j)
                    if (!used[i] && !used[j] && std::fabs(corr[(size_t)i * m + j]) == best) { bx = i; by = j; break; }
            if (bx < 0) break;
            out.emplace_back(bx, by);
            used[bx] = used[by] = 1;
        }
        for (int i = 0; i < m; ++i)
            if (!used[i]) out.emplace_back(i, -1);
    }

    struct Slot {
// ... 995 lines not shown
```

shardmerge_amd/csrc/smhip_device.hpp:

```cpp
#pragma once
#include <hip/hip_runtime.h>

#include "sm_pipeline.hpp"

namespace smhip {

struct DeviceExec {
    template <class S> struct State { using value_type = S; S s; };
    __device__ __forceinline__ int bid() const { return blockIdx.x; }
    __device__ __forceinline__ int nthreads() const { return blockDim.x; }
    __device__ __forceinline__ int nblocks() const { return gridDim.x; }
    __device__ __forceinline__ float* lds() {
        extern __shared__ __attribute__((aligned(16))) float sm_dyn_lds[];
        return sm_dyn_lds;
    }
    template <class S> __device__ __forceinline__ void init(State<S>&) {}
    template <class S, class F> __device__ __forceinline__ void each(State<S>& st, F&& f) { f((int)threadIdx.x, st.s); }
    __device__ __forceinline__ void sync() { __syncthreads(); }
    __device__ __forceinline__ void lds_atomic_add(uint32_t* p, uint32_t v) { atomicAdd(p, v); }
    __device__ __forceinline__ uint32_t lds_atomic_add_ret(uint32_t* p, uint32_t v) { return atomicAdd(p, v); }
    __device__ __forceinline__ uint32_t global_atomic_add_ret_u32(uint32_t* p, uint32_t v) { return atomicAdd(p, v); }
    __device__ __forceinline__ void global_atomic_add(unsigned long long* p, unsigned long long v) { atomicAdd(p, v); }
    __device__ __forceinline__ void global_atomic_add_u32(uint32_t* p, uint32_t v) { atomicAdd(p, v); }
    __device__ __forceinline__ void global_atomic_or_u32(uint32_t* p, uint32_t v) { atomicOr(p, v); }

    template <int DELTA, int N, class S, class Src, class Dst>
    __device__ __forceinline__ void wave_shift_down(State<S>& st, Src src, Dst dst) {
        const uint32_t* a = src(st.s);
        uint32_t* b = dst(st.s);
#pragma unroll
        for (int i = 0; i < N; ++i) b[i] = (uint32_t)__shfl_down((int)a[i], DELTA, 64);
    }
    template <int NP, class S, class Get>
    __device__ __forceinline__ void lane_pair_trade(State<S>& st, Get get) {
        const bool odd = (threadIdx.x & 1u) != 0;
        static_for<0, NP>([&](auto k_c) {
            auto pr = get(st.s, k_c);
            const float give = odd ? pr.a : pr.b;
            const float got = __builtin_bit_cast(float, __builtin_amdgcn_mov_dpp(__builtin_bit_cast(int, give), 0xB1, 0xF, 0xF, true));
            pr.a = odd ? got : pr.a;
            pr.b = odd ? pr.b : got;
        });
    }
    template <int NV, class S, class F>
    __device__ __forceinline__ void block_sum(State<S>& st, F&& f) {
        double v[NV];
#pragma unroll
        for (int q = 0; q < NV; ++q) v[q] = st.s.red[q];
#pragma unroll
        for (int off = 32; off > 0; off >>= 1) {
#pragma unroll
            for (int q = 0; q < NV; ++q) v[q] += __shfl_down(v[q], off, 64);
        }
        double* scratch = (double*)lds();
        const int wave = threadIdx.x >> 6, lane = threadIdx.x & 63;
        const int nw = (blockDim.x + 63) >> 6;
        if (lane == 0) {
#pragma unroll
            for (int q = 0; q < NV; ++q) scratch[wave * NV + q] = v[q];
        }
        __syncthreads();
        if (threadIdx.x == 0) {
            double tot[NV];
#pragma unroll
            for (int q = 0; q < NV; ++q) tot[q] = 0.0;
            for (int w = 0; w < nw; ++w) {
#pragma unroll
                for (int q = 0; q < NV; ++q) tot[q] += scratch[w * NV + q];
            }
            f((const double*)tot);
        }
        __syncthreads();
    }
};

template <class K>
__global__ void __launch_bounds__(K::max_threads, K::waves) sm_kernel(const typename K::Params p) {
    DeviceExec ex;
    K::run(ex, p);
}

#define SM_FFT_KERNELS_OF(X, ...)                      \
    X(KF1<__VA_ARGS__>) X(KF2<__VA_ARGS__>) X(KI1x1<__VA_ARGS__>) X(KI1x2<__VA_ARGS__>) X(KI2<__VA_ARGS__>) X(KF2S<__VA_ARGS__>) \
    X(KF1Q<__VA_ARGS__>) X(KF2Q<__VA_ARGS__>) X(KF2SQ<__VA_ARGS__>) X(KI1x1Q<__VA_ARGS__>) X(KI1x2Q<__VA_ARGS__>) \
    X(KPair1d<__VA_ARGS__>) X(KF1B<__VA_ARGS__>) X(KI2B<__VA_ARGS__>)

}
```

shardmerge_amd/csrc/smhip_side.hip:

```cpp
#include "smhip_device.hpp"

namespace smhip {
#define SM_INST(...) template __global__ void sm_kernel<__VA_ARGS__>(const typename __VA_ARGS__::Params);
#if SM_SIDE_GROUP == 0
SM_SIDE_KERNELS_0(SM_INST)
#elif SM_SIDE_GROUP == 1
SM_SIDE_KERNELS_1(SM_INST)
#elif SM_SIDE_GROUP == 2
SM_SIDE_KERNELS_2(SM_INST)
#elif SM_SIDE_GROUP == 3
SM_INST(KF1<DynPlan>) SM_INST(KF1Q<DynPlan>) SM_INST(KI2<DynPlan>) SM_INST(KPair1d<DynPlan>)
#elif SM_SIDE_GROUP == 4
SM_INST(KF2<DynPlan>) SM_INST(KF2Q<DynPlan>) SM_INST(KF2S<DynPlan>) SM_INST(KF2SQ<DynPlan>)
#elif SM_SIDE_GROUP == 5
SM_INST(KI1x1<DynPlan>) SM_INST(KI1x2<DynPlan>) SM_INST(KI1x1Q<DynPlan>) SM_INST(KI1x2Q<DynPlan>)
#elif SM_SIDE_GROUP == 6
SM_INST(KF1B<DynPlan>) SM_INST(KI2B<DynPlan>)
#else
#error "SM_SIDE_GROUP must be 0..6"
#endif
}
```

Baseline: 84.90 GB/s.

## Add fold-by-2 column FFT path for tall tensors alongside fold-by-4

Generalizes the folded 2D FFT (rows split into sub-columns whose first DFT stage is fused into the row pass) from a fixed factor of 4 to a selectable factor of 2 or 4. New kernel instantiations (F1Q2, F2Q2, F2SQ2) handle factor 2, using a gather that writes interleaved halves, and slab offsets and plan sizes are reworked to depend on the fold factor. Tensors with at least 28672 rows default to factor 2, so the column FFTs become length R/2 instead of R/4 at the cost of fewer folded rows per workgroup. It also changes fold_bin's offset formula, which risks bugs in the inverse path, and adds a debug knob to force either factor.

```diff
diff --git a/shardmerge_amd/csrc/sm_capi.inc b/shardmerge_amd/csrc/sm_capi.inc
--- a/shardmerge_amd/csrc/sm_capi.inc
+++ b/shardmerge_amd/csrc/sm_capi.inc
@@ -253,6 +253,10 @@
     if (key && std::string(key) == "force_bluestein") { ctx->pipe.debug_force_bluestein = value != 0; return SMHIP_OK; }
     if (key && std::string(key) == "force_split") { ctx->pipe.debug_force_split = value > 1 && value <= smhip::DFTP_MAX_P ? (int)value : 0; return SMHIP_OK; }
     if (key && std::string(key) == "fold_columns") { ctx->pipe.fold_enabled = value != 0; return SMHIP_OK; }
+    if (key && std::string(key) == "fold_factor") {
+        if (value != 0 && value != 2 && value != 4) return ctx->pipe.fail(SMHIP_ERR_ARG, "fold_factor: 0, 2 or 4");
+        ctx->pipe.fold_factor = (int)value; return SMHIP_OK;
+    }
     if (key && std::string(key) == "fold_min_rows") { ctx->pipe.fold_min_rows = value > 0 ? (int)value : SM_FOLD_MIN_ROWS; return SMHIP_OK; }
     return ctx->pipe.fail(SMHIP_ERR_ARG, "unknown debug option");
 }
diff --git a/shardmerge_amd/csrc/sm_kernels.hpp b/shardmerge_amd/csrc/sm_kernels.hpp
--- a/shardmerge_amd/csrc/sm_kernels.hpp
+++ b/shardmerge_amd/csrc/sm_kernels.hpp
@@ -499,8 +499,9 @@
 #ifndef SM_F1Q_PACK
 #define SM_F1Q_PACK 1
 #endif
-template <class P> constexpr bool f1q_eligible() {
-    if constexpr (P::is_static) return 4 * P::T <= 1024 && (P::N / P::T) % 2 == 0 && P::N % 8 == 0; else return false;
+template <class P, int F = 4> constexpr bool f1q_eligible() {
+    static_assert(F == 2 || F == 4, "fold factor");
+    if constexpr (P::is_static) return F * P::T <= 1024 && (P::N / P::T) % 2 == 0 && P::N % 8 == 0; else return false;
 }
 
 struct F1QState {
@@ -510,18 +511,18 @@
     u32x4 rb[EMAX / 8], rbb[EMAX / 8];
 };
 
-template <class P, class Ex>
+template <class P, int F = 4, class Ex>
 SM_HD void k_f1q(Ex& ex, const F1Params& p) {
-    if constexpr (!f1q_eligible<P>()) { return; } else {
+    if constexpr (!f1q_eligible<P, F>()) { return; } else {
     typename Ex::template State<F1QState> st;
     ex.init(st);
     float* lds = ex.lds() + LDS_SCRATCH_FLOATS;
     const FftPlanDev& pl = p.plan;
     constexpr int T = P::T, C = P::N, LF = P::lds_floats;
     constexpr int E2 = C / T / 2;
-    constexpr int NJ = (E2 + 3) / 4;
+    constexpr int NJ = (E2 + F - 1) / F;
     constexpr int NQ = EMAX / 8;
-    static_assert(NJ * 8 + 4 <= EREG, "register slots");
+    static_assert(NJ * 2 * F + F <= EREG, "register slots");
     int sig_;
     const int bid = f1_pick_signal(p.sigs, ex.bid(), p.ilv > 1 ? p.ilv : 1, sig_);
     const int pbid = p.sigs.n > 1 ? bid : ex.bid();
@@ -640,13 +641,13 @@
             const int g = tid_ / T, t = tid_ % T;
             auto emit = [&](int k, const float* are, const float* aim, const float* bre, const float* bim) {
                 SM_SCHED_FENCE();
-                float ar[4], ai[4], br[4], bi[4];
-#pragma unroll
-                for (int q = 0; q < 4; ++q) { ar[q] = are[q]; ai[q] = aim[q]; br[q] = has_b ? bre[q] : 0.f; bi[q] = has_b ? bim[q] : 0.f; }
-                Dft<4>::run(ar, ai);
-                Dft<4>::run(br, bi);
-#pragma unroll
-                for (int k1 = 0; k1 < 4; ++k1) {
+                float ar[F], ai[F], br[F], bi[F];
+#pragma unroll
+                for (int q = 0; q < F; ++q) { ar[q] = are[q]; ai[q] = aim[q]; br[q] = has_b ? bre[q] : 0.f; bi[q] = has_b ? bim[q] : 0.f; }
+                Dft<F>::run(ar, ai);
+                Dft<F>::run(br, bi);
+#pragma unroll
+                for (int k1 = 0; k1 < F; ++k1) {
                     if (k1) {
                         const cf2 wa = p.twR[(size_t)n2A * k1], wb = p.twR[(size_t)n2B * k1];
                         cmul(ar[k1], ai[k1], wa.x, wa.y); cmul(br[k1], bi[k1], wb.x, wb.y);
@@ -658,23 +659,23 @@
             };
 #pragma unroll
             for (int jj = 0; jj < NJ; ++jj) {
-                const int u = 4 * jj + g;
+                const int u = F * jj + g;
                 if (u < E2) {
                     const int k = t + u * T;
                     const int k2 = (k == 0) ? 0 : C - k;
-                    float aim[4], bre[4];
-#pragma unroll
-                    for (int gp = 0; gp < 4; ++gp) {
+                    float aim[F], bre[F];
+#pragma unroll
+                    for (int gp = 0; gp < F; ++gp) {
                         const float* l = lds + gp * LF;
                         const float v1 = l[lpad(k)], v2 = l[lpad(k2)];
-                        const int sl = (jj * 4 + gp) * 2;
+                        const int sl = (jj * F + gp) * 2;
                         if (comp == 0) { s.xr[sl] = 0.5f * (v1 + v2); s.xr[sl + 1] = 0.5f * (v2 - v1); }
                         else           { aim[gp] = 0.5f * (v1 - v2); bre[gp] = 0.5f * (v1 + v2); }
                     }
                     if (comp == 1) {
-                        float are[4], bim[4];
-#pragma unroll
-                        for (int gp = 0; gp < 4; ++gp) { are[gp] = s.xr[(jj * 4 + gp) * 2]; bim[gp] = s.xr[(jj * 4 + gp) * 2 + 1]; }
+                        float are[F], bim[F];
+#pragma unroll
+                        for (int gp = 0; gp < F; ++gp) { are[gp] = s.xr[(jj * F + gp) * 2]; bim[gp] = s.xr[(jj * F + gp) * 2 + 1]; }
                         emit(k, are, aim, bre, bim);
                     }
                 }
@@ -682,11 +683,11 @@
             if (tid == 0) {
                 if (comp == 0) {
 #pragma unroll
-                    for (int gp = 0; gp < 4; ++gp) s.xr[NJ * 8 + gp] = lds[gp * LF + lpad(C / 2)];
+                    for (int gp = 0; gp < F; ++gp) s.xr[NJ * 2 * F + gp] = lds[gp * LF + lpad(C / 2)];
                 } else {
-                    float are[4], aim[4] = {0.f, 0.f, 0.f, 0.f}, bre[4], bim[4] = {0.f, 0.f, 0.f, 0.f};
-#pragma unroll
-                    for (int gp = 0; gp < 4; ++gp) { are[gp] = s.xr[NJ * 8 + gp]; bre[gp] = lds[gp * LF + lpad(C / 2)]; }
+                    float are[F], aim[F] = {}, bre[F], bim[F] = {};
+#pragma unroll
+                    for (int gp = 0; gp < F; ++gp) { are[gp] = s.xr[NJ * 2 * F + gp]; bre[gp] = lds[gp * LF + lpad(C / 2)]; }
                     emit(C / 2, are, aim, bre, bim);
                 }
             }
@@ -727,8 +728,18 @@
 };
 SM_HD int fold_bin(int v, int slab, int Cb_real, int R2, int Rfull, size_t& off) {
     const int k1 = v / slab, k = v % slab;
-    off = (size_t)k * Rfull + (size_t)k1 * R2;
+    off = (size_t)k * Rfull + (size_t)k1 * (Rfull / 4);
     return k < Cb_real ? k : -1;
+}
+SM_HD void fold2_gather(const float* l, float* o, int t, int T, int R) {
+#pragma unroll
+    for (int u = 0; u < EMAX / 8; ++u) {
+        const int k0 = 8 * (t + u * T);
+        if (k0 < R) {
+#pragma unroll
+            for (int c = 0; c < 8; ++c) o[8 * u + (c & 1) * 4 + (c >> 1)] = l[lpad(k0 + c)];
+        }
+    }
 }
 
 #ifndef SM_T1_ILV
@@ -744,13 +755,15 @@
 SM_HD constexpr int f2_nsig_for(int T) { return (2 * T <= SM_F2_MAX_THREADS) ? 2 : 1; }
 
 constexpr int FOLD_ILV = 2;
-template <class P> constexpr bool fold_col_plan() {
-    if constexpr (P::is_static) return f2_nsig_for(P::T) == 2 && (P::N == 2048 || P::N == 3584 || P::N == 4096 || P::N == 7168);
-    else return false;
-}
-template <class P, int BINS, bool FOLD = false, class Ex>
+template <class P, int FOLD = 4> constexpr bool fold_col_plan() {
+    static_assert(FOLD == 2 || FOLD == 4, "fold factor");
+    if constexpr (!P::is_static) return false;
+    else if constexpr (FOLD == 2) return P::N == 4096 || P::N == 7168 || P::N == 8192 || P::N == 14336;
+    else return f2_nsig_for(P::T) == 2 && (P::N == 2048 || P::N == 3584 || P::N == 4096 || P::N == 7168);
+}
+template <class P, int BINS, int FOLD = 0, class Ex>
 SM_HD void k_f2(Ex& ex, const F2Params& p) {
-    if constexpr (FOLD && !fold_col_plan<P>()) { return; } else {
+    if constexpr (FOLD && !fold_col_plan<P, FOLD ? FOLD : 4>()) { return; } else {
     typename Ex::template State<FftState> st;
     ex.init(st);
     float* lds = ex.lds() + LDS_SCRATCH_FLOATS;
@@ -801,7 +814,10 @@
                 const int n = tid + q * T;
                 float re = 0.f, im = 0.f;
                 if (n < R) {
-                    const cf2* src = (const cf2*)(t1 + ((size_t)(n / ilv) * p.pitch4 + kbase) * ilv + n % ilv) + slot0;
+                    const cf4* q4;
+                    if constexpr (FOLD) q4 = t1 + (size_t)(kbase / p.slab) * p.slab_elems + ((size_t)(n / ilv) * p.slab + (kbase % p.slab)) * ilv + n % ilv;
+                    else q4 = t1 + ((size_t)(n / ilv) * p.pitch4 + kbase) * ilv + n % ilv;
+                    const cf2* src = (const cf2*)q4 + slot0;
                     re = src->x; im = src->y;
                 }
                 s.xr[q] = re; s.xi[q] = im;
@@ -843,6 +859,7 @@
             const int g = tid / T, t = tid % T;
             const float* l = lds + g * LF;
             float* o = comp_of<comp>(s);
+            if constexpr (FOLD == 2) { fold2_gather(l, o, t, T, R); return; }
 #pragma unroll
             for (int u = 0; u < EMAX / 4; ++u) {
 #pragma unroll
@@ -868,8 +885,9 @@
         float* dim = p.imA + pl_off + poff;
 #pragma unroll
         for (int u = 0; u < EMAX / 4; ++u) {
-            const int k0 = 4 * (t + u * T);
-            if (k0 + 3 < R && (R & 3) == 0) {
+            const int k0 = FOLD == 2 ? (u & 1) * R + 4 * (t + (u >> 1) * T) : 4 * (t + u * T);
+            const bool quad = FOLD == 2 ? 8 * (t + (u >> 1) * T) < R : (k0 + 3 < R && (R & 3) == 0);
+            if (quad) {
                 cf4 vr = {s.xr[4 * u] * sc, s.xr[4 * u + 1] * sc, s.xr[4 * u + 2] * sc, s.xr[4 * u + 3] * sc};
                 *(cf4*)(dre + k0) = vr;
                 if (role_a) {
@@ -879,7 +897,7 @@
             } else {
 #pragma unroll
                 for (int c = 0; c < 4; ++c) {
-                    if (k0 + c < R) {
+                    if (FOLD != 2 && k0 + c < R) {
                         dre[k0 + c] = s.xr[4 * u + c] * sc;
                         if (role_a) dim[k0 + c] = s.xi[4 * u + c] * sc;
                     }
@@ -888,7 +906,7 @@
             if (p.hist) {
 #pragma unroll
                 for (int c = 0; c < 4; ++c) {
-                    if (k0 + c < R) {
+                    if (FOLD == 2 ? quad : k0 + c < R) {
                         const uint32_t key = f2u(s.xr[4 * u + c] * sc) & 0x7fffffffu;
                         ex.lds_atomic_add(&lhist[key >> 20], w);
                     }
@@ -959,9 +977,9 @@
         return ok ? (SM_F2S_DIRECT & 3) : 0;
     }
 }
-template <class P, int G, bool FOLD = false, class Ex>
+template <class P, int G, int FOLD = 0, class Ex>
 SM_HD void k_f2s(Ex& ex, const F2SParams& p) {
-    if constexpr (FOLD && !fold_col_plan<P>()) { return; } else {
+    if constexpr (FOLD && !fold_col_plan<P, FOLD ? FOLD : 4>()) { return; } else {
     typename Ex::template State<FftState> st;
     ex.init(st);
     float* lds = ex.lds() + LDS_SCRATCH_FLOATS;
@@ -987,7 +1005,7 @@
     const int half = R / 2;
     uint32_t* lhist = (uint32_t*)(lds + G * LF);
 
-    constexpr int DIRECT = f2s_direct<P, G>();
+    constexpr int DIRECT = FOLD == 2 ? 0 : f2s_direct<P, G>();
     if constexpr ((DIRECT & 1) != 0) {
         constexpr int R0 = P::radix(0), MB0 = EMAX / R0, nb0 = P::N / R0;
         ex.each(st, [&](int tid, FftState& s) {
@@ -1064,6 +1082,7 @@
             const int g = tid / T, t = tid % T;
             const float* l = lds + g * LF;
             float* o = comp_of<comp>(s);
+            if constexpr (FOLD == 2) { fold2_gather(l, o, t, T, R); return; }
 #pragma unroll
             for (int u = 0; u < EMAX / 4; ++u) {
 #pragma unroll
@@ -1115,8 +1134,9 @@
         } else
 #pragma unroll
         for (int u = 0; u < EMAX / 4; ++u) {
-            const int k0 = 4 * (t + u * T);
-            if (k0 + 3 < R && (R & 3) == 0) {
+            const int k0 = FOLD == 2 ? (u & 1) * R + 4 * (t + (u >> 1) * T) : 4 * (t + u * T);
+            const bool quad = FOLD == 2 ? 8 * (t + (u >> 1) * T) < R : (k0 + 3 < R && (R & 3) == 0);
+            if (quad) {
                 cf4 vr = {s.xr[4 * u] * sc, s.xr[4 * u + 1] * sc, s.xr[4 * u + 2] * sc, s.xr[4 * u + 3] * sc};
 #if defined(SM_DIAG_NOMEM)
                 if (vr.x == 12345.678f)
@@ -1133,7 +1153,7 @@
             } else {
 #pragma unroll
                 for (int c = 0; c < 4; ++c) {
-                    if (k0 + c < R) {
+                    if (FOLD != 2 && k0 + c < R) {
                         dre[k0 + c] = s.xr[4 * u + c] * sc;
                         if (role_a_) { const float vi = s.xi[4 * u + c] * sc; dim[k0 + c] = vi; imsq += vi * vi; }
                     }
@@ -1142,7 +1162,7 @@
             if (p.hist) {
 #pragma unroll
                 for (int c = 0; c < 4; ++c) {
-                    if (k0 + c < R) {
+                    if (FOLD == 2 ? quad : k0 + c < R) {
                         const uint32_t key = f2u(s.xr[4 * u + c] * sc) & 0x7fffffffu;
                         ex.lds_atomic_add(&lhist[key >> 20], w);
                     }
diff --git a/shardmerge_amd/csrc/sm_pipeline.hpp b/shardmerge_amd/csrc/sm_pipeline.hpp
--- a/shardmerge_amd/csrc/sm_pipeline.hpp
+++ b/shardmerge_amd/csrc/sm_pipeline.hpp
@@ -52,8 +52,11 @@
 SM_FFT_KERNEL_TAG(KI2, I2Params, "i2_rows_inv", k_i2<P>(ex, p), 1, 4)
 SM_FFT_KERNEL_TAG(KF2S, F2SParams, "f2s_cols_fwd1", (k_f2s<P, f2s_groups<P>()>(ex, p)), f2s_groups<P>(), 4)
 SM_FFT_KERNEL_TAG(KF1Q, F1Params, "f1_rows_fwd", k_f1q<P>(ex, p), 4, 4)
-SM_FFT_KERNEL_TAG(KF2Q, F2Params, "f2_cols_fwd", (k_f2<P, f2_bins<P>(), true>(ex, p)), 2 * f2_bins<P>(), 4)
-SM_FFT_KERNEL_TAG(KF2SQ, F2SParams, "f2s_cols_fwd1", (k_f2s<P, f2s_groups<P>(), true>(ex, p)), f2s_groups<P>(), 4)
+SM_FFT_KERNEL_TAG(KF2Q, F2Params, "f2_cols_fwd", (k_f2<P, f2_bins<P>(), 4>(ex, p)), 2 * f2_bins<P>(), 4)
+SM_FFT_KERNEL_TAG(KF2SQ, F2SParams, "f2s_cols_fwd1", (k_f2s<P, f2s_groups<P>(), 4>(ex, p)), f2s_groups<P>(), 4)
+SM_FFT_KERNEL_TAG(KF1Q2, F1Params, "f1_rows_fwd", (k_f1q<P, 2>(ex, p)), 2, 4)
+SM_FFT_KERNEL_TAG(KF2Q2, F2Params, "f2_cols_fwd", (k_f2<P, f2_bins<P>(), 2>(ex, p)), 2 * f2_bins<P>(), 4)
+SM_FFT_KERNEL_TAG(KF2SQ2, F2SParams, "f2s_cols_fwd1", (k_f2s<P, f2s_groups<P>(), 2>(ex, p)), f2s_groups<P>(), 4)
 SM_FFT_KERNEL_TAG(KI1x1Q, I1Params, "i1_cols_inv", (k_i1<P, 1, true>(ex, p)), 1, 4)
 SM_FFT_KERNEL_TAG(KI1x2Q, I1Params, "i1_cols_inv", (k_i1<P, i1_bins<P>(), true>(ex, p)), i1_bins<P>(), 4)
 #define SM_BLUE_KERNEL_TAG(Tag, ParamsT, NAME, CALL)                                 \
@@ -398,18 +401,25 @@
 #define SM_FOLD_MIN_ROWS 14336
 #endif
     int fold_min_rows = SM_FOLD_MIN_ROWS;
-    bool fold_shape(int R, int C) const {
-        if (R < fold_min_rows || !(R == 8192 || R == 14336 || R == 16384 || R == 28672)) return false;
+    bool fold_shape(int R, int C) const { return fold_factor_for(R, C) != 1; }
+#ifndef SM_FOLD2_MIN_ROWS
+#define SM_FOLD2_MIN_ROWS 28672
+#endif
+    int fold_factor = 0;
+    int fold_factor_for(int R, int C) const {
+        if (R < fold_min_rows || !(R == 8192 || R == 14336 || R == 16384 || R == 28672)) return 1;
         int T; std::vector<int> rad;
-        if (!plan_shape_static(C, T, rad)) return false;
-        return 4 * T <= 1024 && (C / T) % 2 == 0 && C % 8 == 0;
+        if (!plan_shape_static(C, T, rad)) return 1;
+        if (!(4 * T <= 1024 && (C / T) % 2 == 0 && C % 8 == 0)) return 1;
+        if (fold_factor == 2 || fold_factor == 4) return fold_factor;
+        return R >= SM_FOLD2_MIN_ROWS ? 2 : 4;
     }
     bool fold_enabled = true;
     Geo geo(int R, int C, bool full = false, bool allow_fold = false, int batch = 1) const {
         Geo g;
         g.R = R; g.C = C; g.full = full;
         g.batch = batch < 1 ? 1 : batch;
-        g.fold = (allow_fold && fold_enabled && !full && g.batch == 1 && fold_shape(R, C) && !row_bluestein(C)) ? 4 : 1;
+        g.fold = (allow_fold && fold_enabled && !full && g.batch == 1 && !row_bluestein(C)) ? fold_factor_for(R, C) : 1;
         g.Cb = full ? C : (C / 2 + 1) * g.batch;
         g.pitch4 = (int)round_up((size_t)(C / 2 + 1), 8);
         g.t1_slice = round_up((size_t)R, 8) * (size_t)g.pitch4;
@@ -651,14 +661,16 @@
         p.t1 = (cf4*)t1_.p;
         p.partials = d_part();
         p.R2 = 0; p.rowpair = 0; p.Rcol = g.R; p.twR = nullptr; p.slab_elems = fold_slab_elems(g);
-        if (g.fold == 4) {
+        if (g.fold > 1) {
             if (!p.vec) return fail(SMHIP_ERR_ARG, "internal: folded row pass on unaligned input");
             FftPlanDev colp;
             if ((rc = get_plan(g.R, colp))) return rc;
-            p.R2 = g.R / 4; p.twR = colp.tw; p.ilv = FOLD_ILV; p.nb = 4;
+            p.R2 = g.R / g.fold; p.twR = colp.tw; p.ilv = FOLD_ILV; p.nb = g.fold;
             const int gridq = (int)round_up((size_t)p.R2, 8 * p.ilv);
             if ((size_t)gridq * 2 > PART_DOUBLES) return fail(SMHIP_ERR_SHAPE, "too many rows");
-            launch_fft<KF1Q>(p.plan, gridq, 4 * p.plan.T, (LDS_SCRATCH_FLOATS + (size_t)4 * p.plan.lds_floats) * 4, p);
+            const size_t ldsq = (LDS_SCRATCH_FLOATS + (size_t)g.fold * p.plan.lds_floats) * 4;
+            if (g.fold == 2) launch_fft<KF1Q2>(p.plan, gridq, 2 * p.plan.T, ldsq, p);
+            else launch_fft<KF1Q>(p.plan, gridq, 4 * p.plan.T, ldsq, p);
             grid_out = gridq;
             return SMHIP_OK;
         }
@@ -688,7 +700,8 @@
         return r;
     }
     static size_t fold_slab_elems(const Geo& g, bool rowpair = false) {
-        return round_up((size_t)g.R / (rowpair ? 8 : 4), 8) * (size_t)g.pitch4;
+        const int f = g.fold == 2 ? 2 : 4;
+        return round_up((size_t)g.R / (rowpair ? 2 * f : f), 8) * (size_t)g.pitch4;
     }
     static bool joint_rows(const Geo& g) { return g.rough > 1 && g.R % 16 == 0; }
     int run_f1_rowpairs(const Geo& g, const SigDesc& sig, void* t1buf = nullptr, double* partials = nullptr, int* grid_out = nullptr,
@@ -714,11 +727,11 @@
         p.t1 = (cf4*)(t1buf ? t1buf : t1_.p);
         p.partials = partials ? partials : d_part();
         p.R2 = 0; p.rowpair = 0; p.Rcol = g.R; p.twR = nullptr; p.slab_elems = fold_slab_elems(g, true);
-        if (g.fold == 4) {
+        if (g.fold > 1) {
             if (!p.vec) return fail(SMHIP_ERR_ARG, "internal: folded row pass on unaligned input");
             FftPlanDev colp;
             if ((rc = get_plan(g.R, colp))) return rc;
-            p.R2 = g.R / 8; p.rowpair = 1; p.twR = colp.tw; p.ilv = F2S_ILV; p.nb = 4;
+            p.R2 = g.R / (2 * g.fold); p.rowpair = 1; p.twR = colp.tw; p.ilv = F2S_ILV; p.nb = g.fold;
             const int gridq = (int)round_up((size_t)p.R2, 8 * p.ilv);
             if (multi) {
                 if ((size_t)gridq * 2 * nm > PART_DOUBLES) return SMHIP_ERR_ARG;
@@ -726,7 +739,9 @@
                 multi->b_off = (long long)((size_t)g.C * dt_size(sig.dtype));
                 p.sigs = *multi;
             }
-            launch_fft<KF1Q>(p.plan, gridq * nm, 4 * p.plan.T, (LDS_SCRATCH_FLOATS + (size_t)4 * p.plan.lds_floats) * 4, p);
+            const size_t ldsq = (LDS_SCRATCH_FLOATS + (size_t)g.fold * p.plan.lds_floats) * 4;
+            if (g.fold == 2) launch_fft<KF1Q2>(p.plan, gridq * nm, 2 * p.plan.T, ldsq, p);
+            else launch_fft<KF1Q>(p.plan, gridq * nm, 4 * p.plan.T, ldsq, p);
             if (grid_out) *grid_out = gridq;
             return SMHIP_OK;
         }
@@ -774,7 +789,7 @@
         int rc = get_plan(Rt, p.plan);
         if (rc) return rc;
         p.t1 = (const cf4*)(t1buf ? t1buf : t1_.p); p.pitch4 = g.pitch4 * g.fold; p.R = Rt; p.C = g.C;
-        p.Cb = g.fold == 4 ? 4 * g.pitch4 : g.C / 2 + 1;
+        p.Cb = g.fold > 1 ? g.fold * g.pitch4 : g.C / 2 + 1;
         p.slab = g.pitch4; p.Cb_real = g.C / 2 + 1; p.Rfull = g.R; p.slab_elems = fold_slab_elems(g, true);
         p.role_a = role_a ? 1 : 0; p.scale = scale;
         p.re = plane(g, role_a ? P_REA : P_REB); p.im = plane(g, P_IMA);
@@ -789,6 +804,7 @@
         if (im_parts) *im_parts = want_im ? grid * g.batch : -1;
         p.im_partials = want_im ? d_part_im() : nullptr;
         if (g.fold == 4) { launch_fft<KF2SQ>(p.plan, grid, G * p.plan.T, lds, p); return SMHIP_OK; }
+        if (g.fold == 2) { launch_fft<KF2SQ2>(p.plan, grid, G * p.plan.T, lds, p); return SMHIP_OK; }
         if (g.batch > 1) { p.sl.wgs = grid; p.sl.t1_stride = g.t1_slice / 2; p.sl.plane_stride = (size_t)(g.C / 2 + 1) * g.R; }
         launch_fft<KF2S>(p.plan, grid * g.batch, G * p.plan.T, lds, p);
         return SMHIP_OK;
@@ -864,16 +880,18 @@
             return SMHIP_OK;
         }
         p.slab = g.pitch4; p.Cb_real = g.C / 2 + 1; p.Rfull = g.R; p.slab_elems = fold_slab_elems(g);
-        if (g.fold == 4) {
-            if ((rc = get_plan(g.R / 4, p.plan))) return rc;
-            p.t1 = (const cf4*)t1_.p; p.pitch4 = 4 * g.pitch4; p.ilv = FOLD_ILV; p.R = g.R / 4; p.C = g.C; p.Cb = 4 * g.pitch4;
-            p.nsig = 2; p.swap = swap; p.scale[0] = scale0; p.scale[1] = scale1;
+        if (g.fold > 1) {
+            if ((rc = get_plan(g.R / g.fold, p.plan))) return rc;
+            p.t1 = (const cf4*)t1_.p; p.pitch4 = g.fold * g.pitch4; p.ilv = FOLD_ILV; p.R = g.R / g.fold; p.C = g.C; p.Cb = g.fold * g.pitch4;
+            p.nsig = f2_nsig_for(p.plan.T); p.swap = swap; p.scale[0] = scale0; p.scale[1] = scale1;
             p.reA = plane(g, P_REA); p.imA = plane(g, P_IMA); p.reB = plane(g, P_REB);
             p.hist = hist ? d_hist() : nullptr;
-            const int binsq = f2_bins_host(p.plan);
-            const int gridq = (int)round_up((size_t)(p.Cb + binsq - 1) / binsq, 64);
-            const size_t ldsq = (LDS_SCRATCH_FLOATS + (size_t)2 * binsq * p.plan.lds_floats + HIST1_BINS) * 4;
-            launch_fft<KF2Q>(p.plan, gridq, 2 * binsq * p.plan.T, ldsq, p);
+            const int binsq = p.nsig == 2 ? f2_bins_host(p.plan) : 1;
+            const int ngq = p.nsig == 2 ? 2 * binsq : 1;
+            const int gridq = p.nsig == 2 ? (int)round_up((size_t)(p.Cb + binsq - 1) / binsq, 64) : (int)round_up((size_t)p.Cb * 2, 128);
+            const size_t ldsq = (LDS_SCRATCH_FLOATS + (size_t)ngq * p.plan.lds_floats + HIST1_BINS) * 4;
+            if (g.fold == 2) launch_fft<KF2Q2>(p.plan, gridq, ngq * p.plan.T, ldsq, p);
+            else launch_fft<KF2Q>(p.plan, gridq, ngq * p.plan.T, ldsq, p);
             return SMHIP_OK;
         }
         p.t1 = (const cf4*)t1_.p; p.pitch4 = g.pitch4; p.ilv = g.ilv; p.R = g.R; p.C = g.C; p.Cb = g.C / 2 + 1;
@@ -1074,7 +1092,7 @@
             } else
             if (g.R == 1) {
                 be.template launch<KI1R1>(std::max(1, std::min(64, (Cb + 255) / 256)), 256, LDS_SCRATCH_FLOATS * 4, a, stream);
-            } else if (g.fold == 4) {
+            } else if (g.fold > 1) {
                 if (a.s >= 2) launch_fft<KI1x2Q>(a.plan, grid1, a.s * a.plan.T, lds1, a);
                 else launch_fft<KI1x1Q>(a.plan, grid1, a.plan.T, lds1, a);
             } else if (a.s >= 2) launch_fft<KI1x2>(a.plan, grid1, a.s * a.plan.T, lds1, a);
diff --git a/shardmerge_amd/csrc/smhip_device.hpp b/shardmerge_amd/csrc/smhip_device.hpp
--- a/shardmerge_amd/csrc/smhip_device.hpp
+++ b/shardmerge_amd/csrc/smhip_device.hpp
@@ -83,6 +83,7 @@
 #define SM_FFT_KERNELS_OF(X, ...)                      \
     X(KF1<__VA_ARGS__>) X(KF2<__VA_ARGS__>) X(KI1x1<__VA_ARGS__>) X(KI1x2<__VA_ARGS__>) X(KI2<__VA_ARGS__>) X(KF2S<__VA_ARGS__>) \
     X(KF1Q<__VA_ARGS__>) X(KF2Q<__VA_ARGS__>) X(KF2SQ<__VA_ARGS__>) X(KI1x1Q<__VA_ARGS__>) X(KI1x2Q<__VA_ARGS__>) \
+    X(KF1Q2<__VA_ARGS__>) X(KF2Q2<__VA_ARGS__>) X(KF2SQ2<__VA_ARGS__>) \
     X(KPair1d<__VA_ARGS__>) X(KF1B<__VA_ARGS__>) X(KI2B<__VA_ARGS__>)
 
 }
diff --git a/shardmerge_amd/csrc/smhip_side.hip b/shardmerge_amd/csrc/smhip_side.hip
--- a/shardmerge_amd/csrc/smhip_side.hip
+++ b/shardmerge_amd/csrc/smhip_side.hip
@@ -9,9 +9,9 @@
 #elif SM_SIDE_GROUP == 2
 SM_SIDE_KERNELS_2(SM_INST)
 #elif SM_SIDE_GROUP == 3
-SM_INST(KF1<DynPlan>) SM_INST(KF1Q<DynPlan>) SM_INST(KI2<DynPlan>) SM_INST(KPair1d<DynPlan>)
+SM_INST(KF1<DynPlan>) SM_INST(KF1Q<DynPlan>) SM_INST(KF1Q2<DynPlan>) SM_INST(KI2<DynPlan>) SM_INST(KPair1d<DynPlan>)
 #elif SM_SIDE_GROUP == 4
-SM_INST(KF2<DynPlan>) SM_INST(KF2Q<DynPlan>) SM_INST(KF2S<DynPlan>) SM_INST(KF2SQ<DynPlan>)
+SM_INST(KF2<DynPlan>) SM_INST(KF2Q<DynPlan>) SM_INST(KF2S<DynPlan>) SM_INST(KF2SQ<DynPlan>) SM_INST(KF2Q2<DynPlan>) SM_INST(KF2SQ2<DynPlan>)
 #elif SM_SIDE_GROUP == 5
 SM_INST(KI1x1<DynPlan>) SM_INST(KI1x2<DynPlan>) SM_INST(KI1x1Q<DynPlan>) SM_INST(KI1x2Q<DynPlan>)
 #elif SM_SIDE_GROUP == 6
```

Measured after the change: 63.16 GB/s, median of 2. -25.6%, worse.
